# hyperplane-lab/ACL-GAN

Hardware: AMD Instinct MI355X
Metric: training images/sec at 256x256 (gen+dis step) (higher is better)
Workload: dtype fp32

## Files before the change

### acl-gan_amd/csrc/common.h

```cpp
#pragma once
#include <hip/hip_runtime.h>
#include <stdint.h>
#include <stddef.h>
#include <string>
#include <atomic>
#include "../../include/aclgan_hip.h"
#include "switches.h"

namespace aclgan {

void set_error(const char* fmt, ...);
int hip_fail(hipError_t e, const char* what);

extern std::atomic<long long> g_launches;
extern std::atomic<long long> g_enc_reuse_hits;

#define ACL_CHECK_LAUNCH(what)                                           \
    do {                                                                 \
        ++::aclgan::g_launches;                                          \
        hipError_t e__ = hipGetLastError();                              \
        if (e__ != hipSuccess) return ::aclgan::hip_fail(e__, what);     \
    } while (0)

#define ACL_REQUIRE(cond, ...)                                           \
    do {                                                                 \
        if (!(cond)) { ::aclgan::set_error(__VA_ARGS__); return ACLGAN_EINVAL; } \
    } while (0)

int reduce_slices_ordered(const float* part, int64_t n, int nslices, float* out, hipStream_t st);
size_t colsum_ordered_bytes(int64_t M, int C);
int colsum_ordered(const float* dy, float* db, int64_t M, int C, void* part, hipStream_t st);

static inline int cdiv(int a, int b) { return (a + b - 1) / b; }
static inline int64_t cdiv64(int64_t a, int64_t b) { return (a + b - 1) / b; }

struct ConvGeom {
    int B, Hi, Wi, Ci, Co, k, s, p, up, act;
    int Hu, Wu;
    int Hp, Wp;
    int Ho, Wo;
    int M;
    int K;
};
int make_geom(const aclgan_conv_desc* d, ConvGeom* g);

int conv_fold(const ConvGeom& g, const float* dxp, float* dx, int accumulate, hipStream_t st);
double conv_exec_flops(const ConvGeom& g, int which, bool f16);
bool conv_wgrad_fast_supported(const ConvGeom& g);
int conv_fwd(const ConvGeom& g, const float* x, const float* w, const float* bias, float* y, hipStream_t st, void* scratch = nullptr, float* stats = nullptr,
             float* keepV = nullptr);
size_t conv_fwd_keep_bytes(const ConvGeom& g);
int conv_fwd_stats_chunk(const ConvGeom& g);
size_t conv_fwd_scratch_bytes(const ConvGeom& g);
size_t conv_up5_scratch_bytes(const ConvGeom& g);
int conv_up5_fwd(const ConvGeom& g, const float* x, const float* w, const float* bias, float* y, void* scratch, hipStream_t st, float* keepV = nullptr);
int conv_fwd_naive(const ConvGeom& g, const float* x, const float* w, const float* bias, float* y, hipStream_t st);
size_t conv_dgrad_scratch_bytes(const ConvGeom& g);
int conv_dgrad(const ConvGeom& g, const float* dy, const float* w, float* dx, void* scratch, int accumulate, hipStream_t st);
int conv_wgrad(const ConvGeom& g, const float* x, const float* dy, float* dw, float* db, hipStream_t st, void* scratch = nullptr, const float* haveV = nullptr);
size_t conv_wgrad_scratch_bytes(const ConvGeom& g);
int conv_up5_dgrad(const ConvGeom& g, const float* dy, const float* w, float* dx, int accumulate, void* scratch, hipStream_t st);
int conv_up5_wgrad(const ConvGeom& g, const float* x, const float* dy, float* dw, float* db, void* scratch, hipStream_t st, const float* haveV = nullptr);

int conv_fwd_fast(const ConvGeom& g, const float* x, const float* w, const float* bias, float* y, hipStream_t st, void* scratch = nullptr, float* stats = nullptr,
                  float* keepV = nullptr);
size_t conv_fwd_fast_scratch_bytes(const ConvGeom& g);
int conv_dgrad_fast(const ConvGeom& g, const float* dy, const float* w, float* dxp, float* dx, int accumulate, bool* direct, hipStream_t st);
int conv_dgrad_ring(const ConvGeom& g, const float* dy, const float* w, float* dx, int band, hipStream_t st);
double conv_dgrad_ring_flops(const ConvGeom& g, int band);
int conv_wgrad_fast(const ConvGeom& g, const float* x, const float* dy, float* dw, float* db, hipStream_t st, void* scratch = nullptr, const float* haveV = nullptr);
size_t conv_wgrad_fast_scratch_bytes(const ConvGeom& g);

struct WinoUCache { void* user; float* (*lookup)(void* user, const float* w, int variant, size_t bytes, bool* fresh); };
void set_wino_ucache(const WinoUCache* c);
const WinoUCache* wino_ucache();
size_t conv_wino_u_bytes(const ConvGeom& g);
int conv_wino_u_variant(const ConvGeom& g, int dgrad, bool keepV);
int conv_up5_wino_u_variant(const ConvGeom& g, int dgrad, bool keepV);
int conv_wino_prefill(const ConvGeom& g, int uv, const float* w0, int64_t w_stride, float* U0, int64_t u_stride, int count, hipStream_t st);
int wino_fused_filter_batch(const float* w0, int64_t w_stride, float* Uf0, int64_t u_stride, int count, int Co, int Ci, int flip, hipStream_t st);

bool conv_wino_ok(const ConvGeom& g);
size_t conv_wino_scratch_bytes(const ConvGeom& g);
int conv_fwd_wino(const ConvGeom& g, const float* x, const float* w, const float* bias, float* y, void* scratch, hipStream_t st, float* stats = nullptr,
                  float* keepV = nullptr);
size_t conv_wino_keep_bytes(const ConvGeom& g);
size_t conv_up5_wino_keep_bytes(const ConvGeom& g);
int conv_dgrad_wino_interior(const ConvGeom& g, const float* dy, const float* w, float* dx, int accumulate, void* scratch, hipStream_t st);
size_t conv_wgrad_wino_scratch_bytes(const ConvGeom& g);
bool conv_up5_wino_ok(const ConvGeom& g);
size_t conv_up5_wino_fwd_scratch_bytes(const ConvGeom& g);
size_t conv_up5_wino_dgrad_scratch_bytes(const ConvGeom& g);
size_t conv_up5_wino_wgrad_scratch_bytes(const ConvGeom& g);
int conv_up5_wino_fwd_phases(const ConvGeom& g, const float* x, const float* wp, const float* bias, float* y, void* scratch, hipStream_t st, float* keepV = nullptr,
                             const float* wkey = nullptr);
int conv_up5_wino_dgrad_phases(const ConvGeom& g, const float* dy, const float* wp, float* dx, int accumulate, void* scratch, hipStream_t st,
                               const float* wkey = nullptr);
bool wino_u_cached(const float* wkey, int variant);
int conv_up5_wino_wgrad_phases(const ConvGeom& g, const float* x, const float* dy, float* dwp, float* db, void* scratch, hipStream_t st, const float* haveV = nullptr);
size_t conv_up5_dgrad_scratch_bytes(const ConvGeom& g);
int conv_wgrad_wino(const ConvGeom& g, const float* x, const float* dy, float* dw, float* db, void* scratch, hipStream_t st, const float* haveV = nullptr);

bool conv16_eligible(const ConvGeom& g, int which);
size_t conv_fwd16_scratch_bytes(const ConvGeom& g);
size_t conv_dgrad16_scratch_bytes(const ConvGeom& g);
size_t conv_wgrad16_scratch_bytes(const ConvGeom& g);
int conv_fwd16(const ConvGeom& g, int dtype, const float* x, const float* w, const void* w16, const float* bias, float* y, void* scratch, hipStream_t st,
               const void* x16 = nullptr, int y_storage = 0);
int conv_dgrad16(const ConvGeom& g, int dtype, const float* dy, const float* w, const void* w16t, float* dx, int accumulate, void* scratch, hipStream_t st);
int conv_wgrad16(const ConvGeom& g, int dtype, const float* x, const float* dy, float* dw, float* db, void* scratch, hipStream_t st, int x_storage = 0,
                 int dy_storage = 0);

bool conv16s_ok(const ConvGeom& g, int which);
int conv_fwd16s_stats_chunk(const ConvGeom& g);
int wino_fused_force(int on);
bool wino_fused_ok(int B, int H, int W, int Cin_, int Cout_, int act = ACLGAN_ACT_NONE, int gph = 1, int kph = 1);
int wino_fused_filter(const float* w, float* Uf, int Co, int Ci, int flip, hipStream_t st, int nph = 1);
int wino_fused_launch(int B, int H, int W, int Cin_, int Cout_, const float* in, const float* Uf, const float* bias, float* out, int act, int accumulate,
                      int reflect, float2* stats, hipStream_t st);
int wino_fused_up5_fwd(int B, int Hi, int Wi, int Cin_, int Cout_, const float* x, const float* Uf, const float* bias, float* y, int Hf, int Wf, int act,
                       hipStream_t st);
bool wino_wgrad_fused_ok(const ConvGeom& g);
size_t wino_wgrad_fused_scratch_bytes(const ConvGeom& g);
int wino_wgrad_fused(const ConvGeom& g, const float* x, const float* dy, float* dw, float* db, void* scratch, hipStream_t st);
int wino_fused_up5_dgrad(int B, int Hi, int Wi, int Cin_, int Cout_, const float* dy, const float* Uf, float* dx, int Hf, int Wf, int accumulate, hipStream_t st);
bool wino_fused_s2k4_ok(int B, int Hi, int Wi, int Ci, int Co, int act, int dgrad);
size_t wino_fused_s2k4_u_bytes(int Ci, int Co);
int wino_fused_filter_s2k4(const float* w, float* Uf, int Co, int Ci, int dgrad, hipStream_t st);
int wino_fused_s2k4_fwd(int B, int Hi, int Wi, int Ci, int Co, const float* x, const float* Uf, const float* bias, float* y, int act, float2* stats, hipStream_t st);
int wino_fused_s2k4_dgrad(int B, int Hi, int Wi, int Ci, int Co, const float* dy, const float* Uf, float* dx, int accumulate, hipStream_t st);
bool conv_s2k4_wino_ok(const ConvGeom& g, int which);
size_t conv_s2k4_wino_scratch_bytes(const ConvGeom& g);
int conv_fwd_s2k4_wino(const ConvGeom& g, const float* x, const float* w, const float* bias, float* y, void* scratch, hipStream_t st, float* stats = nullptr);
int conv_dgrad_s2k4_wino_interior(const ConvGeom& g, const float* dy, const float* w, float* dx, int accumulate, void* scratch, hipStream_t st);
bool gemm_x3_shape_ok(int T, int K, int N);
int gemm_slices_x3(const void* A3, size_t a_plane, const void* B3, size_t b_plane, float* C, int T, int K, int N, int nslices, int a_mod, hipStream_t st);
int split3_planes(const float* x, void* out, int64_t n, int64_t plane_elems, hipStream_t st);
int conv_fwd16s(const ConvGeom& g, int dtype, const void* x16, const void* w16, const float* bias, void* y, int yst, hipStream_t st, float* stats = nullptr);
size_t conv_dgrad16s_scratch_bytes(const ConvGeom& g);
bool conv_wgrad16s_ok(const ConvGeom& g);
size_t conv_wgrad16s_scratch_bytes(const ConvGeom& g);
int conv_wgrad16s(const ConvGeom& g, int dtype, const void* x16, const void* dy16, float* dw, float* db, void* scratch, hipStream_t st);
int conv_dgrad16s(const ConvGeom& g, int dtype, const void* dy16, const void* w16t, void* dx, int dxst, int accumulate, void* scratch, hipStream_t st);
int cast_flat16(const float* src, void* dst, int64_t n, int dtype, hipStream_t st);
int transpose_flat16(const float* base, void* base_t, const int64_t* offs, const int* co, const int* taps, const int* ci, int n, int dtype, hipStream_t st);

int conv_fwd_small(const ConvGeom& g, const float* x, const float* w, const float* bias, float* y, hipStream_t st);
int conv_wgrad_small(const ConvGeom& g, const float* x, const float* dy, float* dw, float* db, hipStream_t st, void* scratch = nullptr);
size_t conv_wgrad_small_scratch_bytes(const ConvGeom& g);
int conv_dgrad_small(const ConvGeom& g, const float* dy, const float* w, float* dxp, hipStream_t st);
bool conv_s2k4_thin_dgrad_ok(const ConvGeom& g);

size_t norm_scratch_bytes(int B, int HW, int C);
struct NormST { int x = 0, y = 0, res = 0, dy = 0, dx = 0, dres = 0; };
int norm_fwd(int kind, int act, int B, int HW, int C, const void* x, const float* w, const float* b, int w_stride,
             const void* residual, void* y, float* mean, float* rstd, void* scratch, hipStream_t st, const float* stats = nullptr,
             int stats_chunk = 0, const NormST* sto = nullptr, float* ss_out = nullptr);
int norm_bwd(int kind, int act, int B, int HW, int C, const void* x, const void* y, const void* dy,
             const float* w, int w_stride, const float* mean, const float* rstd, void* dx, float* dw, float* db,
             void* dres, int dres_accumulate, void* scratch, hipStream_t st, const NormST* sto = nullptr, float* sbc_out = nullptr,
             const float* ss = nullptr);
int norm_bwd_ln_params(const float* sbc, int B, int C, float* dgamma, float* dbeta, hipStream_t st);

int act_bwd_inplace(int act, const void* y, void* dy, int64_t n, hipStream_t st, int yst = 0, int gst = 0);
int cast_storage(const void* src, int src_st, void* dst, int dst_st, int64_t n, hipStream_t st);
int positive_mask(const void* y, int yst, unsigned char* dst, int64_t n, hipStream_t st);
int positive_mask_diff(const float* a, int ca, const float* b, int cb, unsigned char* dst, int64_t npix, hipStream_t st);
int avgpool3s2_fwd(int B, int H, int W, int C, const float* x, float* y, hipStream_t st);
int avgpool3s2_bwd(int B, int H, int W, int C, const float* dy, float* dx, int accumulate, hipStream_t st);
size_t diffaugment_scratch_bytes(int N, int H, int W, int C);
int diffaugment_fwd(int N, int H, int W, int C, int policy, const float* x, const float* params, float* y, void* scratch, hipStream_t st);
int diffaugment_bwd(int N, int H, int W, int C, int policy, const float* dy, const float* params, float* dx, int accumulate, void* scratch, hipStream_t st);
struct DisView {
    int cin = 0, dim = 0, n_layer = 0, num_scales = 0;
    const float* lscale = nullptr;
    const float* w[64]; const float* b[64]; float* dw[64];
};
const int DIS_VIEW_MAX = 64;
int dis_view(const aclgan_ctx* ctx, int net, DisView* v);
int adam_flat(float* p, const float* g, float* m, float* v, int64_t n, const aclgan_adam* o, int step, hipStream_t st);
int adam_flat_ema(float* p, const float* g, float* m, float* v, float* ema, int64_t n, const aclgan_adam* o, int step, float decay, int mode, hipStream_t st);
int nchw_to_nhwc(const float* src, float* dst, int B, int C, int H, int W, hipStream_t st);
int nhwc_to_nchw(const float* src, float* dst, int B, int C, int H, int W, hipStream_t st);
int fill_zero(float* p, int64_t n, hipStream_t st);
int zero_async(void* p, size_t bytes, hipStream_t st);

int linear_fwd(int B, int I, int O, const float* x, const float* w, const float* bias, int act, float* y, hipStream_t st);
bool mlp3_fwd_ok(int S, int M);
int mlp3_fwd(int B, int S, int M, int O, const float* s, const float* W0, const float* b0, const float* W1, const float* b1, const float* W2,
             const float* b2, float* m0, float* m1, float* ap, hipStream_t st);
int linear_bwd(int B, int I, int O, const float* x, const float* y, float* dy, const float* w, int act,
               float* dx, float* dw, float* db, hipStream_t st);
int linear_bwd_params(int B, int I, int O, const float* x, const float* dy, float* dw, float* db, hipStream_t st);
int gap_fwd(int B, int HW, int C, const void* x, float* y, hipStream_t st, int xst = 0);
int gap_bwd(int B, int HW, int C, const float* dy, void* dx, int accumulate, hipStream_t st, int xst = 0);

int focus_blend_fwd(int B, int HW, const float* dec4, const float* bg, float* out, const float* pair_first, float* pair, hipStream_t st);
int focus_blend_bwd(int B, int HW, const float* dec4, const float* bg, const float* d_out, const float* d_pair,
                    float* d_dec4, float* d_bg, int bg_accumulate, hipStream_t st);
int plain_pair_fwd(int B, int HW, const float* dec3, float* out, const float* pair_first, float* pair, hipStream_t st);
int plain_pair_bwd(int B, int HW, const float* d_out, const float* d_pair, float* d_dec3, hipStream_t st);
int focus_translation_nchw(const float* fg, int64_t fg_bstride, const float* bg, int64_t bg_bstride, const float* focus, int64_t focus_bstride,
                           float* out, int B, int HW, hipStream_t st);
int lsgan_loss(const float* o, int n, float target, float weight, float* loss_slot, float* d_o, float gscale, hipStream_t st, const float* lscale = nullptr);
struct LsganTerm { const float* o; float* d_o; float* slot; int n; float target, weight, gscale; };
const int LSGAN_MAX_TERMS = 12;
int lsgan_loss_batch(const LsganTerm* terms, int nterms, hipStream_t st, const float* lscale = nullptr);
struct LecamTerm { LsganTerm ls; const float* anchor; float* lecam; float* stats; };
int lsgan_lecam_batch(const LecamTerm* terms, int nterms, float lambda, int start, const int* count, hipStream_t st, const float* lscale = nullptr);
static inline size_t lecam_state_floats(int S) { return (size_t)18 * S + 4; }
int lecam_fold(float* state, int num_scales, float decay, bool whole, hipStream_t st);
struct AdaSignTerm { const float* o; int n; float weight; };
const int ADA_SIGN_MAX_TERMS = 12;
static inline size_t ada_state_floats() { return 12; }
int augment_gate(const float* rows, const float* u, const float* state, int n, int H, int W, int policy, float* rows_eff, hipStream_t st);
int ada_sign(const AdaSignTerm* terms, int nterms, float* acc, hipStream_t st);
int ada_fold(float* state, float target, int interval, float step, hipStream_t st);
const int L1_PART_FLOATS = 1024;
int l1_loss(const float* a, int a_stride, const float* b, int64_t npix, float* loss_slot, float* d_a, float gscale, int d_accumulate, hipStream_t st,
            const float* lscale = nullptr, float* part = nullptr);
int focus_sums_blocks(int64_t npix);
int focus_sums(const float* dec4, int64_t npix, float eps, float upper, float* part, hipStream_t st);
int focus_loss_finish(const float* dec4, int64_t npix, const float* part, float delta, float upper, float lower, float eps,
                      float scale, float* size_slot, float* digit_slot, float* d_dec4, hipStream_t st, const float* lscale = nullptr,
                      const float* totals = nullptr, int64_t npix_total = 0);
int focus_totals(const float* part, int64_t npix, int nmask, float* totals, hipStream_t st);
int adam_flat_scaled(float* p, const float* g, float* m, float* v, int64_t n, const aclgan_adam* o, int step, float* state, int group, hipStream_t st);
int adam_flat_scaled_ema(float* p, const float* g, float* m, float* v, float* ema, int64_t n, const aclgan_adam* o, int step, float decay, int mode,
                         float* state, int group, hipStream_t st);
size_t grad_clip_state_floats();
int gradnorm_launch(const float* g, int64_t n, float max_norm, float* clip, float* lscale, hipStream_t st);
int modeseek_chunks(int64_t n);
size_t modeseek_scratch_floats(int B, int64_t n);
int modeseek_part(const void* a, const void* b, int st, int B, int64_t n, float* part, hipStream_t s);
int modeseek_grad(const void* a, const void* b, int st, int B, int64_t n, const float* part, const float* u, const float* u2, int sd, float u_scale,
                  float weight, const float* lscale, float* out4, float* da, float* db, int accumulate, hipStream_t s);
int adam_flat_clipped(float* p, const float* g, float* m, float* v, float* ema, int64_t n, const aclgan_adam* o, int step, float decay, int mode,
                      float* state, int group, float max_norm, float* clip, hipStream_t st);

const int SN_MAX_LAYERS = 16;
struct SnLayerPtrs { const float* w; float* u; float* v; float* wn; float* uf; float* vf; float* G; int co, k; };
size_t sn_scratch_bytes(int n, const int* co, const int* k);
int sn_power_iteration(int n, const SnLayerPtrs* L, float* sigma, void* scratch, hipStream_t st);
struct SnFoldPtrs { const float* w; const float* G; const float* u; const float* v; float* grad; int co, k; };
size_t sn_fold_scratch_bytes(int n, const int* co, const int* k);
int sn_fold(int n, const SnFoldPtrs* L, const float* sigma, void* scratch, hipStream_t st);

}
```

### acl-gan_amd/csrc/engine.h

```cpp
#pragma once
#include "common.h"
#include <dlfcn.h>

#include <functional>
#include <map>
#include <vector>
#include <tuple>
#include <mutex>
#include <algorithm>
#include <cmath>
#include <cstring>
#include <cstdio>

namespace aclgan {

struct TensorInfo {
    std::string name;
    int64_t offset;
    int64_t numel;
    int shape[4];
    int ndim;
};

struct Group {
    std::vector<TensorInfo> tensors;
    std::map<std::string, int> index;
    int64_t numel = 0;
    float *param = nullptr, *grad = nullptr, *m = nullptr, *v = nullptr;
};

struct Act {
    float* d = nullptr;
    float* g = nullptr;
    int dt = 0, gdt = 0;
    int B = 0, H = 0, W = 0, C = 0;
    bool need_grad = false;
    bool gw = false;
    Act* parent = nullptr;
    struct Stamp { int lane, ck; };
    Stamp dst[4]; int ndst = 0;
    Stamp gst = {-1, 0};
    Act* root() { return parent ? parent : this; }
    int64_t numel() const { return (int64_t)B * H * W * C; }
    bool written() const { return gw || (parent && parent->gw); }
};

struct PW {
    const float* w = nullptr; const float* b = nullptr;
    float* dw = nullptr; float* db = nullptr;
    int64_t nw = 0, nb = 0;
    const unsigned short* w16 = nullptr;
    const unsigned short* w16t = nullptr;
};

struct TapeOp {
    std::function<int(aclgan_ctx&)> fn;
    int64_t goff[4] = {0, 0, 0, 0}, gnum[4] = {0, 0, 0, 0};
    int ng = 0;
    int lane = 0;
    int pass = -1;
};

struct Roctx {
    int (*push)(const char*) = nullptr;
    int (*pop)() = nullptr;
    bool on = false;
    Roctx() {
        if (!sw(SW_ROCTX)) return;
        for (const char* name : {"librocprofiler-sdk-roctx.so", "librocprofiler-sdk-roctx.so.1", "libroctx64.so", "libroctx64.so.4"}) {
            void* h = dlopen(name, RTLD_NOW | RTLD_GLOBAL);
            if (!h) continue;
            push = (int (*)(const char*))dlsym(h, "roctxRangePushA");
            pop = (int (*)())dlsym(h, "roctxRangePop");
            if (push && pop) { on = true; return; }
        }
    }
    static Roctx& get() { static Roctx r; return r; }
    void end_range() { pop(); push(("~end@" + std::to_string((long long)g_launches)).c_str()); pop(); }
};

struct StreamPool {
    static const int N = 4;
    hipStream_t s[N] = {nullptr, nullptr, nullptr, nullptr};
    static StreamPool& of_device() {
        static StreamPool pools[16];
        int dev = 0;
        (void)hipGetDevice(&dev);
        return pools[(dev >= 0 && dev < 16) ? dev : 0];
    }
    int get(int i, hipStream_t* out) {
        static std::mutex mu;
        std::lock_guard<std::mutex> lock(mu);
        if (!s[i]) {
            const hipError_t e = hipStreamCreateWithFlags(&s[i], hipStreamNonBlocking);
            if (e != hipSuccess) { s[i] = nullptr; return hip_fail(e, "stream pool"); }
        }
        *out = s[i];
        return ACLGAN_OK;
    }
};

inline const char* const NET_NAMES[5] = {"gen_AB", "gen_BA", "dis_A", "dis_B", "dis_2"};

}

using namespace aclgan;

struct aclgan_ctx {
    aclgan_arch arch;
    int dis_norm = ACLGAN_NORM_NONE;
    struct SnLayer { int co, k; std::string key; int64_t u_off, v_off; };
    std::vector<SnLayer> sn_layers[5];
    Group sn;
    std::vector<std::string> pass_names;
    std::vector<int> tape_pass;
    std::map<std::string, int> pass_count;
    int cur_pass = -1;
    int pass_begin(const char* net, const char* what);
    void pass_end(int prev);
    Group groups[2];
    char* ws = nullptr;
    size_t ws_bytes = 0;
    hipStream_t st = nullptr;
    bool dry = false;
    size_t top = 0, peak = 0;
    std::vector<Act*> acts;
    std::vector<TapeOp> tape;
    int dtype = ACLGAN_DTYPE_FP32;
    unsigned short* w16[2] = {nullptr, nullptr};
    unsigned short* w16t[2] = {nullptr, nullptr};
    float* lscale = nullptr;
    float* clip[2] = {nullptr, nullptr};
    float clip_max[2] = {0.f, 0.f};
    float* ema = nullptr;
    int fwd_weights = ACLGAN_WEIGHTS_LIVE;
    bool read_ema = false;
    const float* weights(int group) const { return group == ACLGAN_GROUP_GEN && read_ema ? ema : groups[group].param; }
    std::vector<int64_t> cv_off[2];
    std::vector<int> cv_co[2], cv_taps[2], cv_ci[2];
    int trained = -1;
    bool fire_dry = false;
    aclgan_sync_fn sync_fn = nullptr;
    void* sync_user = nullptr;
    int sync_world = 1;
    int64_t bucket_elems = 0;
    aclgan_bucket_fn bucket_fn = nullptr;
    void* bucket_user = nullptr;
    std::vector<int> bucket_order;
    struct NeedKey {
        int which, B, H, W, dtype; long long epoch; int determ, buckets;
        bool operator<(const NeedKey& o) const {
            return std::tie(which, B, H, W, dtype, epoch, determ, buckets) < std::tie(o.which, o.B, o.H, o.W, o.dtype, o.epoch, o.determ, o.buckets);
        }
    };
    std::map<NeedKey, size_t> need_cache;
    struct CarryBlock { float *in32, *co, *out, *mean, *rstd, *ss; int B, H, W, C, co_st, out_st; };
    struct CarryRec {
        bool valid = false;
        int B = 0, H = 0, W = 0, dtype = 0, determ = 0;
        const float* x_a = nullptr;
        long long gen_epoch = 0, tune_epoch = 0;
        char* ws = nullptr; size_t ws_bytes = 0, bytes = 0;
        std::vector<CarryBlock> blocks[2];
    };
    CarryRec carry;
    long long gen_epoch = 0;
    int aug_policy = 0;
    const float* aug_params = nullptr;
    int aug_rows = 0;
    float* lecam_state = nullptr;
    float lecam_lambda = 0.f, lecam_decay = 0.f;
    int lecam_start = 0;
    bool in_dis_update = false;
    float* ada_state = nullptr;
    float ada_target = 0.f, ada_step = 0.f;
    int ada_interval = 1;
    float ms_lambda = 0.f;
    const float* ms_z = nullptr;
    int ms_rows = 0;
    float* ms_out = nullptr;
    bool ms_on() const { return ms_lambda > 0.f && ms_z; }
    int carry_arm = ACLGAN_CARRY_OFF;
    int carry_call = ACLGAN_CARRY_OFF;
    int carry_mode = ACLGAN_CARRY_OFF;
    int carry_pass = 0; size_t carry_blk = 0;
    bool carry_fail = false;
    size_t carry_res = 0;
    int last_mode[2] = {ACLGAN_CARRY_OFF, ACLGAN_CARRY_OFF};
    void carry_drop() { carry.valid = false; ++gen_epoch; }
    size_t lim() const { return carry_res ? ((ws_bytes - carry_res) & ~(size_t)255) : ws_bytes; }
    void* alloc_carry(size_t bytes);
    void carry_pass_begin(int pass) { carry_mode = carry_call; carry_pass = pass; carry_blk = 0; }
    void carry_pass_end() { carry_mode = ACLGAN_CARRY_OFF; }
    double alg_bytes = 0.0;
    void count(double bytes) { alg_bytes += bytes; }
    double exec_flops = 0.0;
    size_t keep_total = 0;
    struct MaskEnt { int B, H, W, C, act; long long off; };
    unsigned char* mask_dst = nullptr; size_t mask_cap = 0, mask_top = 0;
    std::vector<MaskEnt> mask_log;
    int mask_push(int B, int H, int W, int C, int act, size_t n, unsigned char** dst) {
        if (mask_top + n > mask_cap) { set_error("aclgan_debug_capture_masks: buffer too small (%zu bytes)", mask_cap); return ACLGAN_ENOMEM; }
        *dst = mask_dst + mask_top;
        mask_log.push_back(MaskEnt{B, H, W, C, act, (long long)mask_top});
        mask_top += n;
        return ACLGAN_OK;
    }
    struct UEnt { float* u; bool filled; int layout; int lane, ck; };
    std::map<std::pair<const float*, int>, UEnt> ucache;
    WinoUCache ucache_hook;
    static float* ucache_lookup(void* user, const float* w, int variant, size_t bytes, bool* fresh);
    int ucache_reserve(const float* w, int variant, size_t bytes);
    bool act16() const { return dtype != ACLGAN_DTYPE_FP32 && sw(SW_ACT16); }

    hipStream_t st2 = nullptr;
    hipEvent_t ev_fork = nullptr, ev_join = nullptr;
    bool side_pending = false;
    size_t top2 = 0, peak2 = 0;
    void* alloc2(size_t bytes);
    int side_fork();
    int side_join();

    static const int MAXL = 4;
    hipStream_t st0 = nullptr;
    hipStream_t lane_st[MAXL] = {nullptr, nullptr, nullptr, nullptr};
    int nlanes = 1, cur_lane = 0;
    std::vector<hipEvent_t> ev_pool; size_t ev_next = 0;
    std::vector<hipEvent_t> lane_evs[MAXL];
    int seen[MAXL][MAXL] = {};
    size_t hw[MAXL] = {0, 0, 0, 0};
    bool lane_dirty[MAXL] = {false, false, false, false};
    int pass_seq = 0, cur_pass_id = -1;
    hipStream_t lane_stream(int l) const { return l == 0 ? st0 : lane_st[l]; }
    int nck(int l) const { return (int)lane_evs[l].size(); }
    hipStream_t st2_pool = nullptr;
    void lanes_clear();
    int lanes_begin(int want);
    int checkpoint(int l);
    int mark() { return nlanes > 1 ? checkpoint(cur_lane) : ACLGAN_OK; }
    int set_lane(int l);
    int wait_ck(int d, int s, int k);
    int need(Act* a);
    void wrote(Act* a);
    int acq(Act* a);
    int lanes_join();
    int lanes_barrier();
    void lanes_quiesce();
    ~aclgan_ctx();
    void reset_step();
    void* alloc(size_t bytes);
    float* allocf(int64_t n) { return (float*)alloc((size_t)n * sizeof(float)); }
    Act* new_act(int B, int H, int W, int C, bool need_grad, int st = 0, float* const* at = nullptr);
    Act* new_view(Act* joint, int b0, int nb);
    void push(std::function<int(aclgan_ctx&)> fn, std::initializer_list<std::pair<const float*, int64_t>> grads = {});
    PW pw(int group, int net, const std::string& key, bool with_bias = true) const;
    int64_t numel_of(int group, int net, const std::string& key) const;
    const float* param(int group, int net, const std::string& key) const;
    float* gradp(int group, int net, const std::string& key) const;
};

namespace aclgan {

#define RUN(expr)                                  \
    do {                                           \
        if (!c.dry) { int rc__ = (expr); if (rc__) return rc__; } \
    } while (0)
#define CHK(expr)                                  \
    do { int rc__ = (expr); if (rc__) return rc__; } while (0)
#define NEED(ptr)                                  \
    do { if (!(ptr)) { set_error("workspace too small (need > %zu bytes, bound %zu)", c.top, c.ws_bytes); return ACLGAN_ENOMEM; } } while (0)
#define NEED_ACT(a)                                \
    do { NEED((a)->d); if ((a)->need_grad) NEED((a)->g); } while (0)

struct PassScope {
    aclgan_ctx& c; int prev, prev_id;
    PassScope(aclgan_ctx& c_, int net, const char* what) : c(c_), prev(c_.pass_begin(NET_NAMES[net], what)), prev_id(c_.cur_pass_id) { c.cur_pass_id = c.pass_seq++; }
    ~PassScope() { c.pass_end(prev); c.cur_pass_id = prev_id; }
};

struct NormSpec {
    int kind = ACLGAN_NORM_NONE;
    const float* w = nullptr; const float* b = nullptr;
    float* dw = nullptr; float* db = nullptr;
    int w_stride = 0;
};

static inline void mark_written(Act* a) { a->gw = true; }

struct LsSeg { float target, weight, gscale; float* slot; };

int stream_capturing(hipStream_t s);
int run_tape(aclgan_ctx& c);
int prefill_on_side_lane(aclgan_ctx& c, int B, int H, int W, bool train);
int content_encode(aclgan_ctx& c, int net, bool train, Act* x, Act** out);
int style_encode(aclgan_ctx& c, int net, bool train, Act* x, Act** out);
int decode(aclgan_ctx& c, int net, bool train, Act* content, Act* style, Act** out);
int dis_forward(aclgan_ctx& c, int net, bool train, Act* x, std::vector<Act*>* outs, int lane_a = -1, int lane_b = -1);
int dis_lsgan(aclgan_ctx& c, int net, bool train, Act* x, int nb, int row0, const std::vector<LsSeg>& segs, int lane_a = -1, int lane_b = -1);
int blend(aclgan_ctx& c, Act* dec4, Act* bg, Act* pair_first, Act** out_p, Act** pair_p, Act* out_dst = nullptr, Act* pair_dst = nullptr);
int zero_grad_of(aclgan_ctx& c, Act* a);
int pack_params(aclgan_ctx& c);
int input_act(aclgan_ctx& c, const float* nchw, int B, int C, int H, int W, Act** out);
int wrap_vec(aclgan_ctx& c, const float* dev, int B, int n, float scale, Act** out);

}
```

### acl-gan_amd/csrc/engine.hip

```cpp
#include "engine.h"

int aclgan_ctx::pass_begin(const char* net, const char* what) {
    if (!Roctx::get().on || dry) return -1;
    const std::string base = std::string(net) + "." + what;
    const int n = ++pass_count[base];
    pass_names.push_back(base + "#" + std::to_string(n));
    const int prev = cur_pass;
    cur_pass = (int)pass_names.size() - 1;
    Roctx::get().push((pass_names.back() + "@" + std::to_string((long long)g_launches)).c_str());
    return prev;
}
void aclgan_ctx::pass_end(int prev) {
    if (!Roctx::get().on || dry) return;
    Roctx::get().end_range();
    cur_pass = prev;
}

void* aclgan_ctx::alloc2(size_t bytes) {
    const size_t need = top2 + ((bytes + 255) & ~(size_t)255);
    top2 = need;
    if (need > peak2) peak2 = need;
    if (dry) return (void*)(uintptr_t)4096;
    if (peak + need + 256 > lim()) return nullptr;
    return ws + ((lim() - need) & ~(size_t)255);
}
int aclgan_ctx::side_fork() {
    if (dry) return ACLGAN_OK;
    if (!st2) {
        CHK(aclgan::StreamPool::of_device().get(0, &st2_pool));
        st2 = st2_pool;
    }
    if (st2 == st) return ACLGAN_OK;
    if (!ev_fork) {
        hipError_t e = hipEventCreateWithFlags(&ev_fork, hipEventDisableTiming);
        if (e == hipSuccess) e = hipEventCreateWithFlags(&ev_join, hipEventDisableTiming);
        if (e != hipSuccess) return aclgan::hip_fail(e, "side stream events");
    }
    hipError_t e = hipEventRecord(ev_fork, st);
    if (e == hipSuccess) e = hipStreamWaitEvent(st2, ev_fork, 0);
    if (e != hipSuccess) return aclgan::hip_fail(e, "side stream fork");
    side_pending = true;
    return ACLGAN_OK;
}
int aclgan_ctx::side_join() {
    if (dry || !side_pending) return ACLGAN_OK;
    hipError_t e = hipEventRecord(ev_join, st2);
    if (e == hipSuccess) e = hipStreamWaitEvent(st0 ? st0 : st, ev_join, 0);
    if (e != hipSuccess) return aclgan::hip_fail(e, "side stream join");
    side_pending = false;
    return ACLGAN_OK;
}


int aclgan::stream_capturing(hipStream_t s) {
    hipStreamCaptureStatus cs = hipStreamCaptureStatusNone;
    if (hipStreamIsCapturing(s, &cs) != hipSuccess) { (void)hipGetLastError(); return -1; }
    return cs != hipStreamCaptureStatusNone;
}
void aclgan_ctx::lanes_clear() {
    for (int l = 0; l < MAXL; ++l) { lane_evs[l].clear(); hw[l] = 0; lane_dirty[l] = false; for (int m = 0; m < MAXL; ++m) seen[l][m] = 0; }
    ev_next = 0; cur_lane = 0;
}
int aclgan_ctx::lanes_begin(int want) {
    nlanes = std::max(1, std::min(want, (int)MAXL));
    if (!sw(SW_SIDE_STREAM)) nlanes = 1;
    const bool capturing = !dry && stream_capturing(st) > 0;
    if (!dry && !capturing) (void)hipGetLastError();
    if (capturing) nlanes = 1;
    st0 = st;
    lanes_clear();
    if (dry) return ACLGAN_OK;
    if (sw(SW_SIDE_STREAM) && !st2_pool) { int rc = aclgan::StreamPool::of_device().get(0, &st2_pool); if (rc) return rc; }
    st2 = capturing ? st : st2_pool;
    for (int l = 1; l < nlanes; ++l)
        if (!lane_st[l]) { int rc = aclgan::StreamPool::of_device().get(l, &lane_st[l]); if (rc) return rc; }
    return ACLGAN_OK;
}
int aclgan_ctx::checkpoint(int l) {
    hipEvent_t ev = nullptr;
    if (!dry) {
        if (ev_next == ev_pool.size()) {
            hipEvent_t e = nullptr;
            hipError_t rc = hipEventCreateWithFlags(&e, hipEventDisableTiming);
            if (rc != hipSuccess) return aclgan::hip_fail(rc, "lane event");
            ev_pool.push_back(e);
        }
        ev = ev_pool[ev_next++];
        hipError_t rc = hipEventRecord(ev, lane_stream(l));
        if (rc != hipSuccess) return aclgan::hip_fail(rc, "lane checkpoint");
    }
    lane_evs[l].push_back(ev);
    lane_dirty[l] = false;
    return ACLGAN_OK;
}
int aclgan_ctx::set_lane(int l) {
    if (nlanes <= 1) return ACLGAN_OK;
    l %= nlanes;
    if (l == cur_lane) return ACLGAN_OK;
    CHK(checkpoint(cur_lane));
    cur_lane = l;
    lane_dirty[l] = true;
    if (!dry) st = lane_stream(l);
    return ACLGAN_OK;
}
int aclgan_ctx::wait_ck(int d, int s, int k) {
    if (d == s || k < seen[d][s]) return ACLGAN_OK;
    if (k >= nck(s)) {
        CHK(checkpoint(s));
        k = nck(s) - 1;
    }
    if (!dry) {
        hipError_t e = hipStreamWaitEvent(lane_stream(d), lane_evs[s][k], 0);
        if (e != hipSuccess) return aclgan::hip_fail(e, "lane wait");
    }
    lane_dirty[d] = true;
    seen[d][s] = k + 1;
    return ACLGAN_OK;
}
int aclgan_ctx::need(Act* a) {
    if (nlanes <= 1 || !a) return ACLGAN_OK;
    Act* r = a->root();
    for (int i = 0; i < r->ndst; ++i)
        if (r->dst[i].lane != cur_lane) { int rc = wait_ck(cur_lane, r->dst[i].lane, r->dst[i].ck); if (rc) return rc; }
    return ACLGAN_OK;
}
void aclgan_ctx::wrote(Act* a) {
    if (!a) return;
    Act* r = a->root();
    for (int i = 0; i < r->ndst; ++i)
        if (r->dst[i].lane == cur_lane) { r->dst[i].ck = nck(cur_lane); return; }
    if (r->ndst < 4) r->dst[r->ndst++] = Act::Stamp{cur_lane, nck(cur_lane)};
}
int aclgan_ctx::acq(Act* a) {
    if (nlanes <= 1 || !a) return ACLGAN_OK;
    Act* r = a->root();
    if (r->gst.lane >= 0 && r->gst.lane != cur_lane) { int rc = wait_ck(cur_lane, r->gst.lane, r->gst.ck); if (rc) return rc; }
    r->gst = Act::Stamp{cur_lane, nck(cur_lane)};
    return ACLGAN_OK;
}
int aclgan_ctx::lanes_join() {
    if (nlanes > 1) {
        CHK(set_lane(0));
        for (int l = 1; l < nlanes; ++l) {
            if (lane_dirty[l]) CHK(checkpoint(l));
            if (nck(l) > 0) CHK(wait_ck(0, l, nck(l) - 1));
        }
    }
    return side_join();
}
int aclgan_ctx::lanes_barrier() {
    int rc = lanes_join();
    if (rc || nlanes <= 1) return rc;
    CHK(checkpoint(0));
    for (int l = 1; l < nlanes; ++l) CHK(wait_ck(l, 0, nck(0) - 1));
    for (int l = 0; l < MAXL; ++l) hw[l] = 0;
    return ACLGAN_OK;
}
void aclgan_ctx::lanes_quiesce() {
    if (dry) return;
    for (int l = 1; l < nlanes; ++l) if (lane_st[l]) (void)hipStreamSynchronize(lane_st[l]);
    if (st2) (void)hipStreamSynchronize(st2);
    side_pending = false;
    cur_lane = 0; if (st0) st = st0;
}
aclgan_ctx::~aclgan_ctx() {
    reset_step();
    if (ev_fork) (void)hipEventDestroy(ev_fork);
    if (ev_join) (void)hipEventDestroy(ev_join);
    for (hipEvent_t e : ev_pool) (void)hipEventDestroy(e);
}
void aclgan_ctx::reset_step() {
    for (Act* a : acts) delete a;
    acts.clear();
    tape.clear();
    tape_pass.clear(); pass_names.clear(); pass_count.clear(); cur_pass = -1;
    top = 0;
    top2 = 0;
    keep_total = 0;
    ucache.clear();
    read_ema = false;
    lanes_clear();
    nlanes = 1; pass_seq = 0; cur_pass_id = -1;
    if (st0) { st = st0; st0 = nullptr; }
}
void* aclgan_ctx::alloc(size_t bytes) {
    size_t a = (top + 255) & ~(size_t)255;
    if (nlanes > 1) for (int l = 0; l < nlanes; ++l) if (l != cur_lane && hw[l] > a) a = hw[l];
    top = a + bytes;
    if (nlanes > 1) { const size_t e = (top + 255) & ~(size_t)255; if (e > hw[cur_lane]) hw[cur_lane] = e; }
    if (top > peak) peak = top;
    if (dry) return (void*)(uintptr_t)(a + 4096);
    if (top + peak2 + 256 > lim()) return nullptr;
    return ws + a;
}
Act* aclgan_ctx::new_act(int B, int H, int W, int C, bool need_grad, int st, float* const* at) {
    Act* a = new Act();
    a->B = B; a->H = H; a->W = W; a->C = C; a->need_grad = need_grad; a->dt = st; a->gdt = st;
    a->d = at ? *at : (float*)alloc((size_t)a->numel() * (st ? 2 : 4));
    if (need_grad) a->g = allocf(a->numel());
    acts.push_back(a);
    wrote(a);
    return a;
}
Act* aclgan_ctx::new_view(Act* joint, int b0, int nb) {
    Act* a = new Act();
    a->B = nb; a->H = joint->H; a->W = joint->W; a->C = joint->C; a->need_grad = joint->need_grad;
    const int64_t off = (int64_t)b0 * joint->H * joint->W * joint->C;
    a->d = joint->d + off;
    a->g = joint->g ? joint->g + off : nullptr;
    a->parent = joint;
    acts.push_back(a);
    return a;
}
void aclgan_ctx::push(std::function<int(aclgan_ctx&)> fn, std::initializer_list<std::pair<const float*, int64_t>> grads) {
    TapeOp op;
    op.fn = std::move(fn);
    if (trained >= 0 && groups[trained].grad)
        for (const auto& g : grads)
            if (g.first && g.second > 0 && op.ng < 4 && g.first >= groups[trained].grad && g.first < groups[trained].grad + groups[trained].numel) {
                op.goff[op.ng] = g.first - groups[trained].grad; op.gnum[op.ng] = g.second; ++op.ng;
            }
    op.lane = cur_lane; op.pass = cur_pass_id;
    tape.push_back(std::move(op));
    tape_pass.push_back(cur_pass);
}
void* aclgan_ctx::alloc_carry(size_t bytes) {
    const size_t need = carry_res + ((bytes + 255) & ~(size_t)255);
    if (dry) { carry_res = need; return (void*)(uintptr_t)4096; }
    if (peak + peak2 + need + 512 > ws_bytes) return nullptr;
    carry_res = need;
    return ws + ((ws_bytes - need) & ~(size_t)255);
}
float* aclgan_ctx::ucache_lookup(void* user, const float* w, int variant, size_t bytes, bool* fresh) {
    aclgan_ctx* c = (aclgan_ctx*)user;
    const int layout = variant >> 4;
    auto it = c->ucache.find(std::make_pair(w, variant & 15));
    if (it == c->ucache.end()) return nullptr;
    UEnt& e = it->second;
    if (!e.filled) {
        *fresh = true;
        if (bytes) { e.filled = true; e.layout = layout; e.lane = c->cur_lane; e.ck = c->nck(c->cur_lane); }
        return e.u;
    }
    if (e.layout != layout) return nullptr;
    *fresh = false;
    if (bytes && c->nlanes > 1 && e.lane != c->cur_lane && c->wait_ck(c->cur_lane, e.lane, e.ck) != ACLGAN_OK) return nullptr;
    return e.u;
}
int aclgan_ctx::ucache_reserve(const float* w, int variant, size_t bytes) {
    if (sw(SW_NOUCACHE) || !bytes || ucache.count(std::make_pair(w, variant))) return ACLGAN_OK;
    float* u = (float*)alloc(bytes);
    if (!u) return ACLGAN_ENOMEM;
    ucache[std::make_pair(w, variant)] = UEnt{u, false, 0, 0, 0};
    return ACLGAN_OK;
}

static const TensorInfo* find_tensor(const Group& g, int net, const std::string& key) {
    auto it = g.index.find(std::string(NET_NAMES[net]) + "/" + key);
    return it == g.index.end() ? nullptr : &g.tensors[it->second];
}
const float* aclgan_ctx::param(int group, int net, const std::string& key) const {
    const TensorInfo* t = find_tensor(groups[group], net, key);
    return t && groups[group].param ? weights(group) + t->offset : nullptr;
}
float* aclgan_ctx::gradp(int group, int net, const std::string& key) const {
    const TensorInfo* t = find_tensor(groups[group], net, key);
    return t && groups[group].grad ? groups[group].grad + t->offset : nullptr;
}
int64_t aclgan_ctx::numel_of(int group, int net, const std::string& key) const {
    const TensorInfo* t = find_tensor(groups[group], net, key);
    return t ? t->numel : 0;
}
PW aclgan_ctx::pw(int group, int net, const std::string& key, bool with_bias) const {
    PW p;
    p.w = param(group, net, key + ".weight"); p.dw = gradp(group, net, key + ".weight"); p.nw = numel_of(group, net, key + ".weight");
    if (with_bias) { p.b = param(group, net, key + ".bias"); p.db = gradp(group, net, key + ".bias"); p.nb = numel_of(group, net, key + ".bias"); }
    if (dtype != ACLGAN_DTYPE_FP32 && p.w && w16[group] && w16t[group]) {
        const int64_t off = p.w - weights(group);
        p.w16 = w16[group] + off; p.w16t = w16t[group] + off;
    }
    return p;
}

namespace aclgan {

static void add_tensor(Group& g, const std::string& name, int ndim, int d0, int d1 = 1, int d2 = 1, int d3 = 1) {
    TensorInfo t;
    t.name = name; t.offset = g.numel; t.ndim = ndim;
    t.shape[0] = d0; t.shape[1] = d1; t.shape[2] = d2; t.shape[3] = d3;
    t.numel = (int64_t)d0 * d1 * d2 * d3;
    g.index[name] = (int)g.tensors.size();
    g.tensors.push_back(t);
    g.numel += (t.numel + 3) / 4 * 4;
}
static void add_conv(Group& g, const std::string& prefix, int co, int ci, int k) {
    add_tensor(g, prefix + ".weight", 4, co, ci, k, k);
    add_tensor(g, prefix + ".bias", 1, co);
}

static void build_gen(Group& g, const std::string& net, const aclgan_arch& a) {
    char buf[160];
    const int nd = a.gen_n_downsample, nr = a.gen_n_res, sd = a.gen_style_dim;
    int d = a.gen_dim;
    add_conv(g, net + "/enc_style.model.0.conv", d, a.input_dim_a, 7);
    for (int i = 0; i < 2; ++i) { snprintf(buf, sizeof buf, "/enc_style.model.%d.conv", 1 + i); add_conv(g, net + buf, 2 * d, d, 4); d *= 2; }
    for (int i = 0; i < 2; ++i) { snprintf(buf, sizeof buf, "/enc_style.model.%d.conv", 3 + i); add_conv(g, net + buf, d, d, 4); }
    add_conv(g, net + "/enc_style.model.6", sd, d, 1);
    d = a.gen_dim;
    add_conv(g, net + "/enc_content.model.0.conv", d, a.input_dim_a, 7);
    for (int i = 0; i < nd; ++i) { snprintf(buf, sizeof buf, "/enc_content.model.%d.conv", 1 + i); add_conv(g, net + buf, 2 * d, d, 4); d *= 2; }
    for (int r = 0; r < nr; ++r)
        for (int j = 0; j < 2; ++j) { snprintf(buf, sizeof buf, "/enc_content.model.%d.model.%d.model.%d.conv", 1 + nd, r, j); add_conv(g, net + buf, d, d, 3); }
    for (int r = 0; r < nr; ++r)
        for (int j = 0; j < 2; ++j) { snprintf(buf, sizeof buf, "/dec.model.0.model.%d.model.%d.conv", r, j); add_conv(g, net + buf, d, d, 3); }
    int idx = 2;
    for (int i = 0; i < nd; ++i) {
        snprintf(buf, sizeof buf, "/dec.model.%d.norm.gamma", idx); add_tensor(g, net + buf, 1, d / 2);
        snprintf(buf, sizeof buf, "/dec.model.%d.norm.beta", idx); add_tensor(g, net + buf, 1, d / 2);
        snprintf(buf, sizeof buf, "/dec.model.%d.conv", idx); add_conv(g, net + buf, d / 2, d, 5);
        d /= 2; idx += 2;
    }
    snprintf(buf, sizeof buf, "/dec.model.%d.conv", idx - 1); add_conv(g, net + buf, a.gen_output_dim, d, 7);
    const int C = a.gen_dim << nd, nad = 2 * C * 2 * nr, md = a.gen_mlp_dim;
    add_tensor(g, net + "/mlp.model.0.fc.weight", 2, md, sd); add_tensor(g, net + "/mlp.model.0.fc.bias", 1, md);
    add_tensor(g, net + "/mlp.model.1.fc.weight", 2, md, md); add_tensor(g, net + "/mlp.model.1.fc.bias", 1, md);
    add_tensor(g, net + "/mlp.model.2.fc.weight", 2, nad, md); add_tensor(g, net + "/mlp.model.2.fc.bias", 1, nad);
}

static void build_dis(Group& g, const std::string& net, int input_dim, const aclgan_arch& a, std::vector<aclgan_ctx::SnLayer>* sn = nullptr,
                      Group* st = nullptr) {
    char buf[160];
    for (int s = 0; s < a.dis_num_scales; ++s) {
        int d = a.dis_dim;
        snprintf(buf, sizeof buf, "/cnns.%d.0.conv", s); add_conv(g, net + buf, d, input_dim, 4);
        for (int i = 0; i < a.dis_n_layer - 1; ++i) {
            snprintf(buf, sizeof buf, "/cnns.%d.%d.conv", s, i + 1);
            if (sn) {
                const std::string pre = net + buf + ".module.";
                add_tensor(g, pre + "bias", 1, 2 * d);
                add_tensor(g, pre + "weight_bar", 4, 2 * d, d, 4, 4);
                aclgan_ctx::SnLayer L;
                L.co = 2 * d; L.k = 16 * d; L.key = std::string(buf + 1) + ".module.";
                L.u_off = st->numel; add_tensor(*st, pre + "weight_u", 1, L.co);
                L.v_off = st->numel; add_tensor(*st, pre + "weight_v", 1, L.k);
                sn->push_back(L);
            } else {
                add_conv(g, net + buf, 2 * d, d, 4);
            }
            d *= 2;
        }
        snprintf(buf, sizeof buf, "/cnns.%d.%d", s, a.dis_n_layer); add_conv(g, net + buf, 1, d, 1);
    }
}

static void fire_bucket(aclgan_ctx& c, int b) {
    c.bucket_order.push_back(b);
    if (!c.bucket_fn || (c.dry && !c.fire_dry)) return;
    const int64_t off = (int64_t)b * c.bucket_elems;
    const int64_t n = std::min<int64_t>(c.bucket_elems, c.groups[c.trained].numel - off);
    c.bucket_fn(c.bucket_user, c.trained, b, off, n);
}
static int run_tape_impl(aclgan_ctx& c) {
    const size_t n = c.tape.size();
    const bool buckets = c.trained >= 0 && c.bucket_elems > 0;
    std::vector<std::vector<int>> done_at;
    if (buckets) {
        const int nb = (int)cdiv64(c.groups[c.trained].numel, c.bucket_elems);
        std::vector<size_t> first(nb, n);
        for (size_t i = 0; i < n; ++i)
            for (int r = 0; r < c.tape[i].ng; ++r) {
                const int64_t b0 = c.tape[i].goff[r] / c.bucket_elems, b1 = (c.tape[i].goff[r] + c.tape[i].gnum[r] - 1) / c.bucket_elems;
                for (int64_t b = b0; b <= b1 && b < nb; ++b) first[b] = std::min(first[b], i);
            }
        done_at.resize(n);
        c.bucket_order.clear();
        for (int b = 0; b < nb; ++b) {
            if (first[b] == n) fire_bucket(c, b);
            else done_at[first[b]].push_back(b);
        }
    }
    CHK(c.lanes_barrier());
    const bool marks = Roctx::get().on && !c.dry && c.tape_pass.size() == n;
    int open = -1, last_pass = -2;
    for (size_t i = n; i-- > 0;) {
        if (marks && c.tape_pass[i] != open) {
            if (open >= 0) Roctx::get().end_range();
            open = c.tape_pass[i];
            if (open >= 0) Roctx::get().push(("bwd:" + c.pass_names[open] + "@" + std::to_string((long long)g_launches)).c_str());
        }
        if (c.tape[i].pass != last_pass) { if (last_pass != -2) CHK(c.mark()); last_pass = c.tape[i].pass; }
        CHK(c.set_lane(c.tape[i].lane));
        int rc_i = c.tape[i].fn(c);
        if (!rc_i && !c.dry && sw(SW_FAULT_AT) >= 0 && (int)(n - 1 - i) == sw(SW_FAULT_AT)) { set_error("injected fault after backward closure %d (tuning key fault_at)", sw(SW_FAULT_AT)); rc_i = ACLGAN_EHIP; }
        if (rc_i) { if (marks && open >= 0) Roctx::get().pop(); return rc_i; }
        if (buckets && !done_at[i].empty()) {
            const int lane = c.cur_lane;
            CHK(c.lanes_join());
            for (int b : done_at[i]) fire_bucket(c, b);
            CHK(c.set_lane(lane));
        }
    }
    if (marks && open >= 0) Roctx::get().end_range();
    return c.lanes_join();
}
int run_tape(aclgan_ctx& c) {
    const int rc = run_tape_impl(c);
    if (rc) c.lanes_quiesce();
    return rc;
}

}

extern "C" {

int aclgan_ctx_create(const aclgan_arch* arch, aclgan_ctx** out) {
    return aclgan_ctx_create_dis_norm(arch, ACLGAN_NORM_NONE, out);
}

int aclgan_ctx_create_dis_norm(const aclgan_arch* arch, int dis_norm, aclgan_ctx** out) {
    ACL_REQUIRE(arch && out, "null argument");
    ACL_REQUIRE(dis_norm == ACLGAN_NORM_NONE || dis_norm == ACLGAN_NORM_SN, "dis_norm %d: only none (%d) and sn (%d) are implemented", dis_norm,
                ACLGAN_NORM_NONE, ACLGAN_NORM_SN);
    ACL_REQUIRE(arch->input_dim_a == 3 && arch->input_dim_b == 6, "input_dim_a must be 3 and input_dim_b 6 (trainer.py:19-23,132-133)");
    ACL_REQUIRE(arch->gen_output_dim == 4 || arch->gen_output_dim == 3, "gen.output_dim must be 4 (image + focus mask, trainer.py:108) or 3 (non-focus configuration, trainer.py:117-121)");
    ACL_REQUIRE(arch->gen_dim >= 4 && (arch->gen_dim & (arch->gen_dim - 1)) == 0, "gen.dim must be a power of two >= 4");
    ACL_REQUIRE(arch->dis_dim >= 4 && arch->dis_dim % 4 == 0, "dis.dim must be a multiple of 4");
    ACL_REQUIRE(arch->gen_n_downsample >= 1 && arch->gen_n_res >= 1 && arch->dis_n_layer >= 1 && arch->dis_num_scales >= 1, "bad layer counts");
    ACL_REQUIRE(arch->gen_mlp_dim >= 1 && arch->gen_style_dim >= 1, "bad mlp/style dims");
    ACL_REQUIRE(dis_norm != ACLGAN_NORM_SN || arch->dis_num_scales * (arch->dis_n_layer - 1) <= SN_MAX_LAYERS,
                "spectral norm: at most %d normalised layers per discriminator", SN_MAX_LAYERS);
    aclgan_ctx* c = new aclgan_ctx();
    c->arch = *arch;
    const bool sn = dis_norm == ACLGAN_NORM_SN && arch->dis_n_layer > 1;
    c->dis_norm = sn ? ACLGAN_NORM_SN : ACLGAN_NORM_NONE;
    build_gen(c->groups[0], "gen_AB", *arch);
    build_gen(c->groups[0], "gen_BA", *arch);
    build_dis(c->groups[1], "dis_A", arch->input_dim_a, *arch, sn ? &c->sn_layers[ACLGAN_NET_DIS_A] : nullptr, &c->sn);
    build_dis(c->groups[1], "dis_B", arch->input_dim_a, *arch, sn ? &c->sn_layers[ACLGAN_NET_DIS_B] : nullptr, &c->sn);
    build_dis(c->groups[1], "dis_2", arch->input_dim_b, *arch, sn ? &c->sn_layers[ACLGAN_NET_DIS_2] : nullptr, &c->sn);
    for (int g = 0; g < 2; ++g)
        for (const TensorInfo& t : c->groups[g].tensors)
            if (t.ndim == 4) {
                c->cv_off[g].push_back(t.offset); c->cv_co[g].push_back(t.shape[0]);
                c->cv_taps[g].push_back(t.shape[2] * t.shape[3]); c->cv_ci[g].push_back(t.shape[1]);
            }
    *out = c;
    return ACLGAN_OK;
}

void aclgan_ctx_destroy(aclgan_ctx* ctx) { delete ctx; }

int aclgan_ctx_enable_capture(aclgan_ctx* ctx) {
    ACL_REQUIRE(ctx, "null ctx");
    return ACLGAN_OK;
}

int aclgan_warm_streams(int lanes) {
    int n = 0;
    if (hipGetDeviceCount(&n) != hipSuccess || n <= 0) { (void)hipGetLastError(); return ACLGAN_OK; }
    if (!sw(SW_SIDE_STREAM)) return ACLGAN_OK;
    lanes = std::max(1, std::min(lanes <= 0 ? sw(SW_LANES) : lanes, 3));
    hipStream_t s = nullptr;
    int rc = aclgan::StreamPool::of_device().get(0, &s);
    for (int l = 1; l < lanes && rc == ACLGAN_OK; ++l) rc = aclgan::StreamPool::of_device().get(l, &s);
    return rc;
}

int aclgan_debug_capture_masks(aclgan_ctx* ctx, unsigned char* dst, size_t cap_bytes) {
    ACL_REQUIRE(ctx, "null ctx");
    ctx->mask_dst = dst; ctx->mask_cap = dst ? cap_bytes : 0; ctx->mask_top = 0; ctx->mask_log.clear();
    return ACLGAN_OK;
}
int aclgan_debug_mask_count(const aclgan_ctx* ctx) { return ctx ? (int)ctx->mask_log.size() : 0; }
int aclgan_debug_mask_info(const aclgan_ctx* ctx, int index, int* dims4, long long* offset, int* act) {
    ACL_REQUIRE(ctx && index >= 0 && index < (int)ctx->mask_log.size(), "mask index out of range");
    const aclgan_ctx::MaskEnt& e = ctx->mask_log[index];
    if (dims4) { dims4[0] = e.B; dims4[1] = e.H; dims4[2] = e.W; dims4[3] = e.C; }
    if (offset) *offset = e.off;
    if (act) *act = e.act;
    return ACLGAN_OK;
}

int aclgan_set_compute_dtype(aclgan_ctx* ctx, int dtype) {
    ACL_REQUIRE(ctx && dtype >= ACLGAN_DTYPE_FP32 && dtype <= ACLGAN_DTYPE_FP16, "bad ctx / dtype %d", dtype);
    ctx->dtype = dtype;
    ctx->carry_drop();
    return ACLGAN_OK;
}
int aclgan_bind_params16(aclgan_ctx* ctx, int group, void* w16, void* w16t) {
    ACL_REQUIRE(ctx && group >= 0 && group <= 1, "bad ctx/group");
    ctx->w16[group] = (unsigned short*)w16; ctx->w16t[group] = (unsigned short*)w16t;
    ctx->carry_drop();
    return ACLGAN_OK;
}
int aclgan_bind_loss_scale(aclgan_ctx* ctx, float* state) {
    ACL_REQUIRE(ctx, "null ctx");
    ctx->lscale = state;
    return ACLGAN_OK;
}

int64_t aclgan_group_numel(const aclgan_ctx* ctx, int group) {
    if (!ctx || group < 0 || group > ACLGAN_GROUP_SN_STATE) return -1;
    return group == ACLGAN_GROUP_SN_STATE ? ctx->sn.numel : ctx->groups[group].numel;
}
int aclgan_tensor_count(const aclgan_ctx* ctx, int group) {
// ... 182 lines not shown
```

### acl-gan_amd/csrc/engine_graph.hip

```cpp
#include "engine.h"

namespace aclgan {

static int conv_block(aclgan_ctx& c, const PW& W, bool train_w, Act* in, int Co, int k, int stride, int pad, int up, int act,
                      const NormSpec& ns, Act* residual, Act** out_p, int out16 = 1) {
    aclgan_conv_desc d;
    d.B = in->B; d.Hi = in->H; d.Wi = in->W; d.Ci = in->C; d.Co = Co; d.k = k; d.stride = stride; d.pad = pad; d.upsample = up;
    d.act = ns.kind == ACLGAN_NORM_NONE ? act : ACLGAN_ACT_NONE;
    ConvGeom g;
    CHK(make_geom(&d, &g));
    if (!W.w) { set_error("conv_block: parameters not bound"); return ACLGAN_EINVAL; }
    CHK(c.need(in)); CHK(c.need(residual));
    Act* const gin = in;
    const bool want_grad = train_w || in->need_grad || ns.dw != nullptr;
    const bool has_norm = ns.kind != ACLGAN_NORM_NONE;
    const int dt = c.dtype;
    const bool h16 = dt != ACLGAN_DTYPE_FP32 && W.w16 != nullptr;
    const bool f16 = h16 && conv16_eligible(g, 0), d16 = h16 && conv16_eligible(g, 1), w16 = h16 && conv16_eligible(g, 2);
    const bool a16 = h16 && c.act16();
    const bool s_bwd = a16 && f16 && d16 && w16 && conv16s_ok(g, 1);
    const bool s_fwd = a16 && f16 && conv16s_ok(g, 0) && in->dt != 0;
    const bool keep = c.carry_mode == ACLGAN_CARRY_KEEP, adopt = c.carry_mode == ACLGAN_CARRY_ADOPT, carried = keep || adopt;
    const bool tw = train_w || keep;
    aclgan_ctx::CarryBlock cb_dry = {};
    aclgan_ctx::CarryBlock* cb = &cb_dry;
    if (carried && !c.dry) {
        std::vector<aclgan_ctx::CarryBlock>& blocks = c.carry.blocks[c.carry_pass];
        if (keep) { blocks.push_back(cb_dry); cb = &blocks.back(); }
        else {
            if (c.carry_blk >= blocks.size()) { set_error("conv_block: the kept encodings hold no block %zu", c.carry_blk); return ACLGAN_EINVAL; }
            cb = &blocks[c.carry_blk++];
        }
    }
    auto buf = [&](float* aclgan_ctx::CarryBlock::*slot, size_t bytes) -> float* {
        if (!carried) return (float*)c.alloc(bytes);
        if (adopt && !c.dry) return cb->*slot;
        float* p = (float*)c.alloc_carry(bytes);
        cb->*slot = p;
        return p;
    };
    auto act_in = [&](float* aclgan_ctx::CarryBlock::*slot, int B_, int H_, int W_, int C_, bool grad, int st) -> Act* {
        float* at = carried ? buf(slot, (size_t)B_ * H_ * W_ * C_ * (st ? 2 : 4)) : nullptr;
        return c.new_act(B_, H_, W_, C_, grad, st, carried ? &at : nullptr);
    };
    if (in->dt != 0 && !(f16 && (w16 || !tw))) {
        Act* in32 = act_in(&aclgan_ctx::CarryBlock::in32, in->B, in->H, in->W, in->C, false, 0);
        NEED_ACT(in32);
        if (!adopt) RUN(cast_storage(in->d, in->dt, in32->d, 0, in->numel(), c.st));
        in = in32;
    }
    const int out_st = (a16 && Co % 64 == 0 && out16) ? dt : 0;
    const int co_st = has_norm ? ((s_bwd && sw(SW_CO16)) ? dt : 0) : ((f16 || !out_st) ? out_st : 0);
    if (adopt && !c.dry && (cb->B != g.B || cb->H != g.Ho || cb->W != g.Wo || cb->C != Co || cb->co_st != co_st || cb->out_st != out_st)) {
        set_error("conv_block: the kept encodings do not match this layer (%d x %d x %d x %d)", g.B, g.Ho, g.Wo, Co);
        return ACLGAN_EINVAL;
    }
    if (keep) { cb->B = g.B; cb->H = g.Ho; cb->W = g.Wo; cb->C = Co; cb->co_st = co_st; cb->out_st = out_st; }
    Act* co = act_in(&aclgan_ctx::CarryBlock::co, g.B, g.Ho, g.Wo, Co, want_grad, co_st);
    NEED_ACT(co);
    Act* out = co;
    float *mean = nullptr, *rstd = nullptr, *ss = nullptr;
    const int HW = g.Ho * g.Wo;
    if (has_norm) {
        out = act_in(&aclgan_ctx::CarryBlock::out, g.B, g.Ho, g.Wo, Co, want_grad, out_st);
        NEED_ACT(out);
        const int nstat = ns.kind == ACLGAN_NORM_LN ? g.B : g.B * Co;
        mean = buf(&aclgan_ctx::CarryBlock::mean, (size_t)nstat * 4); rstd = buf(&aclgan_ctx::CarryBlock::rstd, (size_t)nstat * 4);
        NEED(mean); NEED(rstd);
        if ((want_grad || keep) && (act == ACLGAN_ACT_RELU || act == ACLGAN_ACT_LRELU) && sw(SW_NORM_MASK)) {
            ss = buf(&aclgan_ctx::CarryBlock::ss, (size_t)2 * g.B * Co * 4);
            NEED(ss);
        }
        co->gdt = s_bwd ? dt : 0;
    } else if (out_st && !co_st) {
        out = act_in(&aclgan_ctx::CarryBlock::out, g.B, g.Ho, g.Wo, Co, want_grad, out_st);
        NEED_ACT(out);
        out->gdt = 0;
    } else {
        out->gdt = s_bwd ? co_st : 0;
    }
    if (gin->need_grad && !s_bwd) gin->gdt = 0;
    float* keepV = nullptr;
    if (train_w && !adopt && !f16 && !w16) {
        const size_t kb = conv_fwd_keep_bytes(g);
        if (kb && c.keep_total + kb <= (size_t)(sw_real(SW_KEEPV_BUDGET_GB) * 1073741824.0) + 1) { keepV = (float*)c.alloc(kb); NEED(keepV); c.keep_total += kb; }
    }
    const size_t ubytes = f16 ? 0 : conv_wino_u_bytes(g);
    if (ubytes && !adopt && c.ucache_reserve(W.w, g.up ? 2 : 0, ubytes)) { set_error("workspace too small (filter-transform cache)"); return ACLGAN_ENOMEM; }
    const double es_in = in->dt ? 2.0 : 4.0, es_co = co->dt ? 2.0 : 4.0, es_out = out->dt ? 2.0 : 4.0, es_w = f16 ? 2.0 : 4.0;
    if (!adopt) c.count(es_in * (double)in->numel() + es_w * (double)Co * g.K + 4.0 * Co + es_co * (double)co->numel());
    if (!adopt) c.exec_flops += conv_exec_flops(g, 0, f16);
    if (out != co && !adopt) c.count((es_co + es_out) * (double)co->numel() + ((has_norm && residual) ? (residual->dt ? 2.0 : 4.0) * (double)co->numel() : 0.0));
    const size_t mark = c.top;
    if (!adopt) {
    const int schunk = !has_norm ? 0 : (s_fwd ? conv_fwd16s_stats_chunk(g) : (!f16 ? conv_fwd_stats_chunk(g) : 0));
    float* stats = nullptr;
    if (schunk) { stats = c.allocf((size_t)2 * g.B * (HW / schunk) * Co); NEED(stats); }
    {
        const size_t fmark = c.top;
        void* fscr = nullptr;
        const size_t fb = s_fwd ? 0 : (f16 ? conv_fwd16_scratch_bytes(g) : conv_fwd_scratch_bytes(g));
        if (fb) { fscr = c.alloc(fb); NEED(fscr); }
        if (s_fwd) RUN(conv_fwd16s(g, dt, in->d, W.w16, W.b, co->d, co->dt, c.st, stats));
        else if (f16) RUN(conv_fwd16(g, dt, in->dt ? nullptr : in->d, W.w, W.w16, W.b, co->d, fscr, c.st, in->dt ? in->d : nullptr, co->dt));
        else RUN(conv_fwd(g, in->d, W.w, W.b, co->d, c.st, fscr, stats, keepV));
        c.top = fmark;
    }
    NormST nst;
    nst.x = co->dt; nst.y = out->dt; nst.res = residual ? residual->dt : 0;
    if (has_norm) {
        void* scr = c.alloc(norm_scratch_bytes(g.B, HW, Co));
        NEED(scr);
        RUN(norm_fwd(ns.kind, act, g.B, HW, Co, co->d, ns.w, ns.b, ns.w_stride, residual ? residual->d : nullptr, out->d, mean, rstd, scr, c.st, stats, schunk, &nst, ss));
    } else if (out != co) {
        RUN(cast_storage(co->d, co->dt, out->d, out->dt, co->numel(), c.st));
    }
    }
    c.top = mark;
    *out_p = out;
    if (c.mask_dst && !c.dry && want_grad && (act == ACLGAN_ACT_RELU || act == ACLGAN_ACT_LRELU)) {
        unsigned char* dst = nullptr;
        CHK(c.mask_push(out->B, out->H, out->W, out->C, act, (size_t)out->numel(), &dst));
        RUN(positive_mask(out->d, out->dt, dst, out->numel(), c.st));
    }
    c.wrote(out); c.wrote(co);
    if (!want_grad) return ACLGAN_OK;
    const bool ln_train = ns.kind == ACLGAN_NORM_LN && ns.dw != nullptr;
    c.push([=](aclgan_ctx& c) -> int {
        if (!out->gw) return ACLGAN_OK;
        CHK(c.acq(out));
        if (residual && residual->need_grad) CHK(c.acq(residual));
        if (gin->need_grad) CHK(c.acq(gin));
        const double eg_out = out->gdt ? 2.0 : 4.0, eg_co = (has_norm ? co->gdt : (s_bwd ? dt : out->gdt)) ? 2.0 : 4.0, eg_in = gin->gdt ? 2.0 : 4.0;
        c.count((es_co + eg_out + eg_co) * (double)co->numel() + ((residual && residual->need_grad) ? (residual->gdt ? 2.0 : 4.0) * (double)co->numel() : 0.0));
        if (train_w) { c.count(es_in * (double)in->numel() + eg_co * (double)co->numel() + 4.0 * ((double)Co * g.K + Co)); c.exec_flops += conv_exec_flops(g, 2, w16); }
        if (gin->need_grad) { c.count(eg_co * (double)co->numel() + es_w * (double)Co * g.K + eg_in * (double)in->numel()); c.exec_flops += conv_exec_flops(g, 1, d16); }
        const bool side = train_w && sw(SW_SIDE_STREAM);
        if (ubytes && gin->need_grad && !d16 && c.ucache_reserve(W.w, g.up ? 3 : 1, ubytes)) { set_error("workspace too small (filter-transform cache)"); return ACLGAN_ENOMEM; }
        float* g16 = nullptr;
        const size_t mark_pre = c.top;
        if (!has_norm && s_bwd && out->gdt == 0) {
            g16 = (float*)c.alloc((size_t)out->numel() * 2);
            NEED(g16);
        }
        float* sbc = nullptr;
        if (ln_train && side) { sbc = c.allocf((int64_t)2 * g.B * Co); NEED(sbc); }
        const size_t mark0 = side ? c.top : mark_pre;
        const float* dyp = nullptr;
        int dy_st = 0;
        if (has_norm) {
            const size_t mark = c.top;
            void* scr = c.alloc(norm_scratch_bytes(g.B, HW, Co));
            NEED(scr);
            float* dres = nullptr; int dacc = 0;
            if (residual && residual->need_grad) { dres = residual->g; dacc = residual->gw ? 1 : 0; mark_written(residual); }
            NormST bst;
            bst.x = co->dt; bst.y = out->dt; bst.dy = out->gdt; bst.dx = co->gdt; bst.dres = residual ? residual->gdt : 0;
            RUN(norm_bwd(ns.kind, act, g.B, HW, Co, co->d, out->d, out->g, ns.w, ns.w_stride, mean, rstd, co->g, ns.dw, ns.db, dres, dacc, scr, c.st, &bst, sbc, ss));
            c.top = mark;
            dyp = co->g; dy_st = co->gdt;
        } else if (s_bwd && out->gdt == 0) {
            RUN(cast_storage(out->g, 0, g16, dt, out->numel(), c.st));
            RUN(act_bwd_inplace(act, out->d, g16, out->numel(), c.st, out->dt, dt));
            dyp = g16; dy_st = dt;
        } else {
            RUN(act_bwd_inplace(act, co->d, out->g, out->numel(), c.st, co->dt, out->gdt));
            dyp = out->g; dy_st = out->gdt;
        }
        if (train_w) {
            const size_t mark = c.top;
            void* wscr = nullptr;
            const size_t wb = w16 ? conv_wgrad16_scratch_bytes(g) : conv_wgrad_scratch_bytes(g);
            hipStream_t wst = c.st;
            if (side) {
                CHK(c.side_fork());
                if (!c.dry) wst = c.st2;
                c.top2 = 0;
                if (wb) { wscr = c.alloc2(wb); if (!wscr) { set_error("workspace too small for the side-stream scratch"); return ACLGAN_ENOMEM; } }
                if (sbc) RUN(norm_bwd_ln_params(sbc, g.B, Co, ns.dw, ns.db, wst));
            } else if (wb) { wscr = c.alloc(wb); NEED(wscr); }
            if (w16) RUN(conv_wgrad16(g, dt, in->d, dyp, W.dw, W.db, wscr, wst, in->dt, dy_st));
            else {
                if (in->dt || dy_st) { set_error("conv_block: fp32 weight-gradient kernel on 16-bit operands"); return ACLGAN_EINVAL; }
                RUN(conv_wgrad(g, in->d, dyp, W.dw, W.db, wst, wscr, keepV));
            }
            c.top = mark;
        }
        if (gin->need_grad) {
            const size_t mark = c.top;
            if (s_bwd) {
                if (!dy_st) { set_error("conv_block: 16-bit-storage dgrad on an fp32 gradient"); return ACLGAN_EINVAL; }
                void* scr = c.alloc(conv_dgrad16s_scratch_bytes(g));
                NEED(scr);
                RUN(conv_dgrad16s(g, dt, dyp, W.w16t, gin->g, gin->gdt, gin->gw ? 1 : 0, scr, c.st));
            } else {
                if (dy_st || gin->gdt) { set_error("conv_block: fp32-output dgrad kernel on 16-bit gradients"); return ACLGAN_EINVAL; }
                void* scr = c.alloc(d16 ? conv_dgrad16_scratch_bytes(g) + 256 : conv_dgrad_scratch_bytes(g));
                NEED(scr);
                if (d16) RUN(conv_dgrad16(g, dt, dyp, W.w, W.w16t, gin->g, gin->gw ? 1 : 0, scr, c.st));
                else RUN(conv_dgrad(g, dyp, W.w, gin->g, scr, gin->gw ? 1 : 0, c.st));
            }
            mark_written(gin);
            c.top = mark;
        }
        c.top = mark0;
        return ACLGAN_OK;
    }, {{train_w ? W.dw : nullptr, W.nw}, {train_w ? W.db : nullptr, W.nb}, {ln_train ? ns.dw : nullptr, Co}, {ln_train ? ns.db : nullptr, Co}});
    return ACLGAN_OK;
}

static int prefill_wino_u(aclgan_ctx& c, int net, int B, int H, int W, bool train) {
    if (sw(SW_NOUCACHE) || !sw(SW_U_BATCH)) return ACLGAN_OK;
    const aclgan_arch& a = c.arch;
    const int nd = a.gen_n_downsample, count = 2 * a.gen_n_res, C = a.gen_dim << nd;
    if (count < 2) return ACLGAN_OK;
    aclgan_conv_desc d;
    d.B = B; d.Hi = H >> nd; d.Wi = W >> nd; d.Ci = C; d.Co = C; d.k = 3; d.stride = 1; d.pad = 1; d.upsample = 0; d.act = ACLGAN_ACT_NONE;
    ConvGeom g;
    if (make_geom(&d, &g)) return ACLGAN_OK;
    const size_t ubytes = conv_wino_u_bytes(g);
    if (!ubytes) return ACLGAN_OK;
    if (c.dtype != ACLGAN_DTYPE_FP32 && c.w16[0] && conv16_eligible(g, 0)) return ACLGAN_OK;
    char buf[160];
    for (int part = 0; part < 2; ++part) {
        std::vector<const float*> ws;
        for (int r = 0; r < a.gen_n_res; ++r)
            for (int j = 0; j < 2; ++j) {
                if (part == 0) snprintf(buf, sizeof buf, "enc_content.model.%d.model.%d.model.%d.conv.weight", 1 + nd, r, j);
                else snprintf(buf, sizeof buf, "dec.model.0.model.%d.model.%d.conv.weight", r, j);
                ws.push_back(c.param(0, net, buf));
            }
        if (!ws[0]) continue;
        const int64_t wstride = ws[1] - ws[0];
        bool even = wstride > 0;
        for (int i = 1; i < count && even; ++i) even = ws[i] && ws[i] - ws[i - 1] == wstride;
        if (!even) continue;
        for (int dgrad = 0; dgrad <= (train ? 1 : 0); ++dgrad) {
            const bool keepV = train && !dgrad && conv_fwd_keep_bytes(g) > 0;
            const int uv = conv_wino_u_variant(g, dgrad, keepV);
            if (uv < 0 || c.ucache.count(std::make_pair(ws[0], uv & 15))) continue;
            float* u0 = nullptr;
            bool contiguous = true;
            const size_t ustride = (ubytes + 255) & ~(size_t)255;
            for (int i = 0; i < count; ++i) {
                float* u = (float*)c.alloc(ubytes);
                NEED(u);
                if (i == 0) u0 = u;
                else if ((char*)u != (char*)u0 + (size_t)i * ustride) contiguous = false;
                c.ucache[std::make_pair(ws[i], uv & 15)] = aclgan_ctx::UEnt{u, contiguous, uv >> 4, c.cur_lane, c.nck(c.cur_lane)};
            }
            if (!contiguous) {
                for (int i = 0; i < count; ++i) c.ucache[std::make_pair(ws[i], uv & 15)].filled = false;
                continue;
            }
            RUN(conv_wino_prefill(g, uv, ws[0], wstride, u0, (int64_t)(ustride / sizeof(float)), count, c.st));
        }
    }
    return ACLGAN_OK;
}

int prefill_on_side_lane(aclgan_ctx& c, int B, int H, int W, bool train) {
    const int AB = ACLGAN_NET_GEN_AB, BA = ACLGAN_NET_GEN_BA;
    if (c.nlanes <= 1) { CHK(prefill_wino_u(c, AB, B, H, W, train)); return prefill_wino_u(c, BA, B, H, W, train); }
    const int LP = c.nlanes - 1;
    CHK(c.mark());
    const int k0 = c.nck(0) - 1;
    CHK(c.set_lane(LP));
    CHK(c.wait_ck(LP, 0, k0));
    CHK(prefill_wino_u(c, AB, B, H, W, train)); CHK(prefill_wino_u(c, BA, B, H, W, train));
    CHK(c.mark());
    return c.set_lane(0);
}

int content_encode(aclgan_ctx& c, int net, bool train, Act* x, Act** out) {
    PassScope pass(c, net, c.carry_mode == ACLGAN_CARRY_ADOPT ? "encode(adopted)" : "encode");
    const aclgan_arch& a = c.arch;
    char buf[160];
    NormSpec in_; in_.kind = ACLGAN_NORM_IN;
    Act* h = nullptr;
    int d = a.gen_dim;
    CHK(conv_block(c, c.pw(0, net, "enc_content.model.0.conv"), train, x, d, 7, 1, 3, 0, ACLGAN_ACT_RELU, in_, nullptr, &h));
    for (int i = 0; i < a.gen_n_downsample; ++i) {
        snprintf(buf, sizeof buf, "enc_content.model.%d.conv", 1 + i);
        CHK(conv_block(c, c.pw(0, net, buf), train, h, 2 * d, 4, 2, 1, 0, ACLGAN_ACT_RELU, in_, nullptr, &h));
        d *= 2;
    }
    for (int r = 0; r < a.gen_n_res; ++r) {
        Act *t = nullptr, *o = nullptr;
        snprintf(buf, sizeof buf, "enc_content.model.%d.model.%d.model.0.conv", 1 + a.gen_n_downsample, r);
        CHK(conv_block(c, c.pw(0, net, buf), train, h, d, 3, 1, 1, 0, ACLGAN_ACT_RELU, in_, nullptr, &t));
        snprintf(buf, sizeof buf, "enc_content.model.%d.model.%d.model.1.conv", 1 + a.gen_n_downsample, r);
        CHK(conv_block(c, c.pw(0, net, buf), train, t, d, 3, 1, 1, 0, ACLGAN_ACT_NONE, in_, h, &o));
        h = o;
    }
    *out = h;
    return ACLGAN_OK;
}

static int dense(aclgan_ctx& c, const PW& W, bool train_w, Act* in, int O, int act, Act** out_p, bool launch = true) {
    const int B = in->B, I = in->H * in->W * in->C;
    const bool want = train_w || in->need_grad;
    CHK(c.need(in));
    Act* out = c.new_act(B, 1, 1, O, want);
    NEED_ACT(out);
    if (!W.w) { set_error("dense: parameters not bound"); return ACLGAN_EINVAL; }
    if (launch) RUN(linear_fwd(B, I, O, in->d, W.w, W.b, act, out->d, c.st));
    c.count(4.0 * ((double)B * I + (double)O * I + O + (double)B * O) * (want ? 3.0 : 1.0));
    c.wrote(out);
    *out_p = out;
    if (!want) return ACLGAN_OK;
    c.push([=](aclgan_ctx& c) -> int {
        if (!out->gw) return ACLGAN_OK;
        CHK(c.acq(out));
        if (in->need_grad) CHK(c.acq(in));
        float* dx = nullptr;
        float* tmp = nullptr;
        const size_t mark = c.top;
        if (in->need_grad) {
            if (in->gw) { tmp = c.allocf((int64_t)B * I); NEED(tmp); dx = tmp; } else dx = in->g;
        }
        const bool side = train_w && sw(SW_SIDE_STREAM);
        RUN(linear_bwd(B, I, O, in->d, out->d, out->g, W.w, act, dx, (train_w && !side) ? W.dw : nullptr, (train_w && !side) ? W.db : nullptr, c.st));
        if (side) {
            CHK(c.side_fork());
            RUN(linear_bwd_params(B, I, O, in->d, out->g, W.dw, W.db, c.st2));
        }
        if (in->need_grad) {
            if (tmp) {
                RUN(gap_bwd(B, 1, I, tmp, in->g, 1, c.st));
            }
            mark_written(in);
        }
        c.top = mark;
        return ACLGAN_OK;
    }, {{train_w ? W.dw : nullptr, W.nw}, {train_w ? W.db : nullptr, W.nb}});
    return ACLGAN_OK;
}

int style_encode(aclgan_ctx& c, int net, bool train, Act* x, Act** out) {
    PassScope pass(c, net, "style");
    const aclgan_arch& a = c.arch;
    char buf[160];
    NormSpec none;
    Act* h = nullptr;
    int d = a.gen_dim;
    CHK(conv_block(c, c.pw(0, net, "enc_style.model.0.conv"), train, x, d, 7, 1, 3, 0, ACLGAN_ACT_RELU, none, nullptr, &h));
    for (int i = 0; i < 2; ++i) {
        snprintf(buf, sizeof buf, "enc_style.model.%d.conv", 1 + i);
        CHK(conv_block(c, c.pw(0, net, buf), train, h, 2 * d, 4, 2, 1, 0, ACLGAN_ACT_RELU, none, nullptr, &h));
        d *= 2;
    }
    for (int i = 0; i < 2; ++i) {
        snprintf(buf, sizeof buf, "enc_style.model.%d.conv", 3 + i);
        CHK(conv_block(c, c.pw(0, net, buf), train, h, d, 4, 2, 1, 0, ACLGAN_ACT_RELU, none, nullptr, &h));
    }
    const bool want = h->need_grad;
    Act* p = c.new_act(h->B, 1, 1, d, want);
    NEED_ACT(p);
    RUN(gap_fwd(h->B, h->H * h->W, d, h->d, p->d, c.st, h->dt));
    c.wrote(p);
    c.count((h->dt ? 2.0 : 4.0) * (double)h->numel() * (want ? 2.0 : 1.0));
    if (want) {
        Act* hh = h;
        c.push([=](aclgan_ctx& c) -> int {
            if (!p->gw) return ACLGAN_OK;
            CHK(c.acq(p)); CHK(c.acq(hh));
            RUN(gap_bwd(hh->B, hh->H * hh->W, hh->C, p->g, hh->g, hh->gw ? 1 : 0, c.st, hh->gdt));
            mark_written(hh);
            return ACLGAN_OK;
        });
    }
    CHK(dense(c, c.pw(0, net, "enc_style.model.6"), train, p, a.gen_style_dim, ACLGAN_ACT_NONE, out));
    return ACLGAN_OK;
}

int decode(aclgan_ctx& c, int net, bool train, Act* content, Act* style, Act** out) {
    PassScope pass(c, net, "decode");
    const aclgan_arch& a = c.arch;
    char buf[160];
    const int C = content->C, nr = a.gen_n_res, nad = 2 * C * 2 * nr;
    Act *m0 = nullptr, *m1 = nullptr, *ap = nullptr;
    const int sdim = style->H * style->W * style->C;
    const bool fused = sw(SW_MLP_FUSED) && mlp3_fwd_ok(sdim, a.gen_mlp_dim);
    const PW W0 = c.pw(0, net, "mlp.model.0.fc"), W1 = c.pw(0, net, "mlp.model.1.fc"), W2 = c.pw(0, net, "mlp.model.2.fc");
    CHK(dense(c, W0, train, style, a.gen_mlp_dim, ACLGAN_ACT_RELU, &m0, !fused));
    CHK(dense(c, W1, train, m0, a.gen_mlp_dim, ACLGAN_ACT_RELU, &m1, !fused));
    CHK(dense(c, W2, train, m1, nad, ACLGAN_ACT_NONE, &ap, !fused));
    if (fused) RUN(mlp3_fwd(style->B, sdim, a.gen_mlp_dim, nad, style->d, W0.w, W0.b, W1.w, W1.b, W2.w, W2.b, m0->d, m1->d, ap->d, c.st));
    if (ap->need_grad) {
        RUN(fill_zero(ap->g, ap->numel(), c.st));
        mark_written(ap);
    }
    Act* h = content;
    int j = 0;
    for (int r = 0; r < nr; ++r) {
        Act *t = nullptr, *o = nullptr;
        for (int half = 0; half < 2; ++half) {
            NormSpec ns; ns.kind = ACLGAN_NORM_ADAIN; ns.w_stride = nad;
            ns.b = ap->d + 2 * C * j; ns.w = ap->d + 2 * C * j + C;
            if (ap->need_grad) { ns.db = ap->g + 2 * C * j; ns.dw = ap->g + 2 * C * j + C; }
            ++j;
            snprintf(buf, sizeof buf, "dec.model.0.model.%d.model.%d.conv", r, half);
            if (half == 0) CHK(conv_block(c, c.pw(0, net, buf), train, h, C, 3, 1, 1, 0, ACLGAN_ACT_RELU, ns, nullptr, &t));
            else CHK(conv_block(c, c.pw(0, net, buf), train, t, C, 3, 1, 1, 0, ACLGAN_ACT_NONE, ns, h, &o));
        }
        h = o;
    }
    int d = C, idx = 2;
    for (int i = 0; i < a.gen_n_downsample; ++i) {
        NormSpec ns; ns.kind = ACLGAN_NORM_LN;
        snprintf(buf, sizeof buf, "dec.model.%d.norm.gamma", idx); ns.w = c.param(0, net, buf); ns.dw = train ? c.gradp(0, net, buf) : nullptr;
        snprintf(buf, sizeof buf, "dec.model.%d.norm.beta", idx); ns.b = c.param(0, net, buf); ns.db = train ? c.gradp(0, net, buf) : nullptr;
        snprintf(buf, sizeof buf, "dec.model.%d.conv", idx);
        CHK(conv_block(c, c.pw(0, net, buf), train, h, d / 2, 5, 1, 2, 1, ACLGAN_ACT_RELU, ns, nullptr, &h, i + 1 < a.gen_n_downsample ? 1 : 0));
        d /= 2; idx += 2;
    }
    NormSpec none;
    snprintf(buf, sizeof buf, "dec.model.%d.conv", idx - 1);
    CHK(conv_block(c, c.pw(0, net, buf), train, h, a.gen_output_dim, 7, 1, 3, 0, ACLGAN_ACT_TANH, none, nullptr, out));
    return ACLGAN_OK;
}

struct SnCall {
    int n = 0;
    float *slot = nullptr, *G = nullptr, *sigma = nullptr;
    void* fscr = nullptr;
    unsigned short *s16 = nullptr, *s16t = nullptr;
    int64_t soff[SN_MAX_LAYERS] = {};
};

static int sn_begin_call(aclgan_ctx& c, int net, bool train, SnCall* sc) {
    const std::vector<aclgan_ctx::SnLayer>& Ls = c.sn_layers[net];
    const int n = (int)Ls.size();
    if (!c.dry && !c.sn.param) { set_error("spectral norm: aclgan_bind_sn_state was not called"); return ACLGAN_EINVAL; }
    int co[SN_MAX_LAYERS], kk[SN_MAX_LAYERS], taps[SN_MAX_LAYERS], ci[SN_MAX_LAYERS];
    int64_t tot = 0, tu = 0, tv = 0;
    sc->n = n;
    for (int l = 0; l < n; ++l) {
        co[l] = Ls[l].co; kk[l] = Ls[l].k; taps[l] = 16; ci[l] = Ls[l].k / 16;
        sc->soff[l] = tot;
        tot += (int64_t)co[l] * kk[l]; tu += co[l]; tv += kk[l];
    }
    const bool h16 = c.dtype != ACLGAN_DTYPE_FP32;
    sc->slot = c.allocf(tot); NEED(sc->slot);
    if (h16) {
        sc->s16 = (unsigned short*)c.alloc((size_t)tot * 2); NEED(sc->s16);
        sc->s16t = (unsigned short*)c.alloc((size_t)tot * 2); NEED(sc->s16t);
    }
    sc->sigma = c.allocf(n); NEED(sc->sigma);
    if (train) {
        sc->G = c.allocf(tot); NEED(sc->G);
        sc->fscr = c.alloc(sn_fold_scratch_bytes(n, co, kk)); NEED(sc->fscr);
    }
    const size_t mark = c.top;
    void* scr = c.alloc(sn_scratch_bytes(n, co, kk));
    NEED(scr);
    SnLayerPtrs P[SN_MAX_LAYERS];
    for (int l = 0; l < n; ++l) {
        float* st = c.sn.param;
        P[l] = SnLayerPtrs{c.param(1, net, Ls[l].key + "weight_bar"), st ? st + Ls[l].u_off : nullptr, st ? st + Ls[l].v_off : nullptr,
                           sc->slot + sc->soff[l], nullptr, nullptr, train ? sc->G + sc->soff[l] : nullptr, co[l], kk[l]};
    }
    RUN(sn_power_iteration(n, P, sc->sigma, scr, c.st));
    if (h16) {
        RUN(cast_flat16(sc->slot, sc->s16, tot, c.dtype, c.st));
        RUN(transpose_flat16(sc->slot, sc->s16t, sc->soff, co, taps, ci, n, c.dtype, c.st));
    }
    c.top = mark;
    c.count(4.0 * tot * (2.0 + 0.25 + 1.0 + (train ? 1.0 : 0.0)) + (h16 ? (8.0 + 4.0) * tot : 0.0) + 4.0 * 3.0 * (tu + tv));
    c.exec_flops += 4.0 * tot;
    if (!train) return ACLGAN_OK;
    const float* lo = nullptr; const float* hi = nullptr;
    for (int l = 0; l < n; ++l) {
        const float* g = c.gradp(1, net, Ls[l].key + "weight_bar");
        if (!g) continue;
        if (!lo || g < lo) lo = g;
        if (!hi || g + (int64_t)co[l] * kk[l] > hi) hi = g + (int64_t)co[l] * kk[l];
    }
    const SnCall s = *sc;
    c.push([=](aclgan_ctx& c) -> int {
        hipStream_t fst = c.st;
        if (sw(SW_SIDE_STREAM)) {
            CHK(c.side_fork());
            if (!c.dry) fst = c.st2;
        }
        SnFoldPtrs F[SN_MAX_LAYERS];
        const float* st = c.sn.param;
        for (int l = 0; l < s.n; ++l)
            F[l] = SnFoldPtrs{c.param(1, net, Ls[l].key + "weight_bar"), s.G + s.soff[l], st ? st + Ls[l].u_off : nullptr,
                              st ? st + Ls[l].v_off : nullptr, c.gradp(1, net, Ls[l].key + "weight_bar"), co[l], kk[l]};
        c.count(4.0 * tot * 5.0);
        c.exec_flops += 6.0 * tot;
        RUN(sn_fold(s.n, F, s.sigma, s.fscr, fst));
        return ACLGAN_OK;
    }, {{lo, (int64_t)(hi - lo)}});
    return ACLGAN_OK;
}

static PW sn_pw(aclgan_ctx& c, int net, const SnCall& sc, int l) {
    const aclgan_ctx::SnLayer& L = c.sn_layers[net][l];
    PW p;
    p.w = sc.slot + sc.soff[l];
    p.dw = sc.G ? sc.G + sc.soff[l] : nullptr;
    p.nw = (int64_t)L.co * L.k;
    p.b = c.param(1, net, L.key + "bias"); p.db = c.gradp(1, net, L.key + "bias"); p.nb = L.co;
    if (sc.s16) { p.w16 = sc.s16 + sc.soff[l]; p.w16t = sc.s16t + sc.soff[l]; }
    return p;
}

int dis_forward(aclgan_ctx& c, int net, bool train, Act* x, std::vector<Act*>* outs, int lane_a, int lane_b) {
    PassScope pass(c, net, "forward");
    const aclgan_arch& a = c.arch;
    char buf[160];
    NormSpec none;
    Act* xin = x;
    if (lane_a < 0) lane_a = lane_b = c.cur_lane;
    SnCall sc;
    const bool sn = !c.sn_layers[net].empty();
    int pi_lane = 0, pi_ck = 0;
    if (sn) {
        CHK(c.set_lane(lane_a));
        CHK(c.need(x));
        CHK(sn_begin_call(c, net, train, &sc));
        pi_lane = c.cur_lane; pi_ck = c.nck(pi_lane);
    }
    for (int s = 0; s < a.dis_num_scales; ++s) {
        CHK(c.set_lane(s == 0 ? lane_a : lane_b));
        if (sn) CHK(c.wait_ck(c.cur_lane, pi_lane, pi_ck));
        Act* h = xin;
        int d = a.dis_dim;
        for (int i = 0; i < a.dis_n_layer; ++i) {
            snprintf(buf, sizeof buf, "cnns.%d.%d.conv", s, i);
            const int co = i == 0 ? d : 2 * d;
            const PW p = (sn && i > 0) ? sn_pw(c, net, sc, s * (a.dis_n_layer - 1) + i - 1) : c.pw(1, net, buf);
            CHK(conv_block(c, p, train, h, co, 4, 2, 1, 0, ACLGAN_ACT_LRELU, none, nullptr, &h, i + 1 < a.dis_n_layer ? 1 : 0));
            if (i > 0) d *= 2;
        }
        snprintf(buf, sizeof buf, "cnns.%d.%d", s, a.dis_n_layer);
        Act* o = nullptr;
        CHK(conv_block(c, c.pw(1, net, buf), train, h, 1, 1, 1, 0, 0, ACLGAN_ACT_NONE, none, nullptr, &o));
        outs->push_back(o);
        if (s + 1 < a.dis_num_scales) {
            CHK(c.set_lane(lane_b));
            Act* src = xin;
            CHK(c.need(src));
            Act* p = c.new_act(src->B, (src->H - 1) / 2 + 1, (src->W - 1) / 2 + 1, src->C, src->need_grad);
            NEED_ACT(p);
            RUN(avgpool3s2_fwd(src->B, src->H, src->W, src->C, src->d, p->d, c.st));
            c.wrote(p);
            c.count(4.0 * ((double)src->numel() + (double)p->numel()) * (src->need_grad ? 2.0 : 1.0));
            if (src->need_grad) {
                c.push([=](aclgan_ctx& c) -> int {
                    if (!p->gw) return ACLGAN_OK;
                    CHK(c.acq(p)); CHK(c.acq(src));
                    RUN(avgpool3s2_bwd(src->B, src->H, src->W, src->C, p->g, src->g, src->gw ? 1 : 0, c.st));
                    mark_written(src);
                    return ACLGAN_OK;
                });
            }
            xin = p;
        }
    }
    return ACLGAN_OK;
}

static int augment(aclgan_ctx& c, int net, Act* x, int row0, Act** out) {
    PassScope pass(c, net, "augment");
    CHK(c.need(x));
    if (x->dt != 0) { set_error("augment: the discriminator inputs are fp32 tensors"); return ACLGAN_EINVAL; }
    Act* y = c.new_act(x->B, x->H, x->W, x->C, x->need_grad);
    NEED_ACT(y);
    const int policy = c.aug_policy;
    const size_t sb = (policy & ACLGAN_AUG_COLOR) ? diffaugment_scratch_bytes(x->B, x->H, x->W, x->C) : 0;
    const float* rows = c.aug_params ? c.aug_params + (size_t)row0 * 8 : nullptr;
    {
        const size_t mark = c.top;
        void* scr = nullptr;
        if (sb) { scr = c.alloc(sb); NEED(scr); }
        RUN(diffaugment_fwd(x->B, x->H, x->W, x->C, policy, x->d, rows, y->d, scr, c.st));
        c.top = mark;
    }
    c.wrote(y);
    c.count(4.0 * 2.0 * (double)x->numel() * (x->need_grad ? 2.0 : 1.0));
    *out = y;
    if (!x->need_grad) return ACLGAN_OK;
    c.push([=](aclgan_ctx& c) -> int {
        if (!y->gw) return ACLGAN_OK;
        CHK(c.acq(y)); CHK(c.acq(x));
        if (y->gdt != 0 || x->gdt != 0) { set_error("augment: the gradients of the discriminator inputs are fp32 tensors"); return ACLGAN_EINVAL; }
        const size_t mark = c.top;
        void* scr = nullptr;
        if (sb) { scr = c.alloc(sb); NEED(scr); }
        RUN(diffaugment_bwd(x->B, x->H, x->W, x->C, policy, y->g, rows, x->g, x->gw ? 1 : 0, scr, c.st));
        mark_written(x);
        c.top = mark;
        return ACLGAN_OK;
    });
    return ACLGAN_OK;
}

int dis_lsgan(aclgan_ctx& c, int net, bool train, Act* x, int nb, int row0, const std::vector<LsSeg>& segs, int lane_a, int lane_b) {
    std::vector<Act*> outs;
    if (c.aug_policy) {
        if (lane_a >= 0) CHK(c.set_lane(lane_a));
        CHK(augment(c, net, x, row0, &x));
        CHK(c.mark());
    }
    CHK(dis_forward(c, net, train, x, &outs, lane_a, lane_b));
    std::vector<LsganTerm> terms;
    for (Act* o : outs) {
        CHK(c.need(o));
        const int n = nb * o->H * o->W * o->C;
        for (size_t i = 0; i < segs.size(); ++i) {
            LsganTerm t;
            t.o = o->d + (size_t)i * n; t.d_o = o->need_grad ? o->g + (size_t)i * n : nullptr; t.slot = segs[i].slot;
            t.n = n; t.target = segs[i].target; t.weight = segs[i].weight; t.gscale = segs[i].gscale;
            terms.push_back(t);
        }
        if (o->need_grad) mark_written(o);
    }
    if (train && c.in_dis_update && c.lecam_state) {
        const int S = c.arch.dis_num_scales, D = net - ACLGAN_NET_DIS_A;
        float* st = c.lecam_state;
        std::vector<LecamTerm> lt(terms.size());
        for (size_t j = 0; j < terms.size(); ++j) {
            const int s = (int)(j / segs.size()), k = terms[j].target == 1.f ? 1 : 0;
            lt[j].ls = terms[j];
            lt[j].anchor = st + (D * S + s) * 2 + (1 - k);
            lt[j].lecam = st + 18 * S + D;
            lt[j].stats = st + 6 * S + ((D * S + s) * 2 + k) * 2;
        }
        RUN(lsgan_lecam_batch(lt.data(), (int)lt.size(), c.lecam_lambda, c.lecam_start, reinterpret_cast<const int*>(st + 18 * S + 3), c.st, c.lscale));
    } else RUN(lsgan_loss_batch(terms.data(), (int)terms.size(), c.st, c.lscale));
    if (train && c.in_dis_update && c.ada_state && net != ACLGAN_NET_DIS_2) {
        std::vector<AdaSignTerm> at;
        double bytes = 0.0;
        for (const LsganTerm& t : terms)
            if (t.target == 1.f) { at.push_back(AdaSignTerm{t.o, t.n, t.weight}); bytes += 4.0 * (double)t.n; }
        if (!at.empty()) {
            c.count(bytes + 2.0 * 4.0 * 2.0);
            RUN(ada_sign(at.data(), (int)at.size(), c.ada_state + 8 + 2 * (net - ACLGAN_NET_DIS_A), c.st));
        }
    }
    return ACLGAN_OK;
}

int blend(aclgan_ctx& c, Act* dec4, Act* bg, Act* pair_first, Act** out_p, Act** pair_p, Act* out_dst, Act* pair_dst) {
    const bool want = dec4->need_grad;
    CHK(c.need(dec4)); CHK(c.need(bg)); CHK(c.need(pair_first));
    Act* out = out_dst;
    if (!out) {
        out = c.new_act(dec4->B, dec4->H, dec4->W, 3, want);
        NEED_ACT(out);
    }
    Act* pair = nullptr;
    if (pair_first) {
        pair = pair_dst;
        if (!pair) {
            pair = c.new_act(dec4->B, dec4->H, dec4->W, 6, want);
            NEED_ACT(pair);
        }
    }
    const bool plain = dec4->C == 3;
    if (plain) RUN(plain_pair_fwd(dec4->B, dec4->H * dec4->W, dec4->d, out->d, pair_first ? pair_first->d : nullptr, pair ? pair->d : nullptr, c.st));
    else RUN(focus_blend_fwd(dec4->B, dec4->H * dec4->W, dec4->d, bg->d, out->d, pair_first ? pair_first->d : nullptr, pair ? pair->d : nullptr, c.st));
    c.count(4.0 * (double)dec4->B * dec4->H * dec4->W * ((plain ? 3 : 4 + 3) + 3 + (pair_first ? 9 : 0)) * (want ? 2.0 : 1.0));
    c.wrote(out); c.wrote(pair);
    *out_p = out;
    if (pair_p) *pair_p = pair;
    if (!want) return ACLGAN_OK;
    c.push([=](aclgan_ctx& c) -> int {
        const float* dout = out->written() ? out->g : nullptr;
        const float* dpair = (pair && pair->written()) ? pair->g : nullptr;
        if (!dout && !dpair) return ACLGAN_OK;
        if (dout) CHK(c.acq(out));
        if (dpair) CHK(c.acq(pair));
        CHK(c.acq(dec4));
        if (!plain && bg->need_grad) CHK(c.acq(bg));
        if (plain) { RUN(plain_pair_bwd(dec4->B, dec4->H * dec4->W, dout, dpair, dec4->g, c.st)); return ACLGAN_OK; }
        float* dbg = bg->need_grad ? bg->g : nullptr;
        RUN(focus_blend_bwd(dec4->B, dec4->H * dec4->W, dec4->d, bg->d, dout, dpair, dec4->g, dbg, bg->gw ? 1 : 0, c.st));
        if (dbg) mark_written(bg);
        return ACLGAN_OK;
    });
    return ACLGAN_OK;
}

int zero_grad_of(aclgan_ctx& c, Act* a) {
    if (a->need_grad) { RUN(fill_zero(a->g, a->numel(), c.st)); mark_written(a); }
    return ACLGAN_OK;
}

__global__ void scale_kernel(const float* s, float* d, float a, int n) {
    const int i = blockIdx.x * 256 + threadIdx.x;
    if (i < n) d[i] = a * s[i];
}

int pack_params(aclgan_ctx& c) {
    if (c.dtype == ACLGAN_DTYPE_FP32 || c.dry) return ACLGAN_OK;
    for (int g = 0; g < 2; ++g) {
        if (!c.w16[g] || !c.w16t[g]) { set_error("compute dtype is 16-bit but aclgan_bind_params16 was not called for group %d", g); return ACLGAN_EINVAL; }
        CHK(cast_flat16(c.weights(g), c.w16[g], c.groups[g].numel, c.dtype, c.st));
        CHK(transpose_flat16(c.weights(g), c.w16t[g], c.cv_off[g].data(), c.cv_co[g].data(), c.cv_taps[g].data(), c.cv_ci[g].data(),
                             (int)c.cv_off[g].size(), c.dtype, c.st));
    }
    return ACLGAN_OK;
// ... 23 lines not shown
```

### acl-gan_amd/csrc/engine_step.hip

```cpp
#include "engine.h"

namespace aclgan {

std::atomic<long long> g_enc_reuse_hits{0};

static int64_t dis_min_side(const aclgan_arch& a) {
    if (a.dis_n_layer + a.dis_num_scales > 30) return INT32_MAX;
    return (((int64_t)1 << a.dis_n_layer) - 1) * ((int64_t)1 << (a.dis_num_scales - 1)) + 1;
}
static int64_t content_min_side(const aclgan_arch& a) { return a.gen_n_downsample > 29 ? INT32_MAX : (int64_t)2 << a.gen_n_downsample; }
static const int STYLE_MIN_SIDE = 16;

static int check_shape(const aclgan_ctx& c, int B, int H, int W) {
    ACL_REQUIRE(B >= 1 && H >= 64 && W >= 64, "batch shape (%d,%d,%d): need B>=1 and H,W>=64 (third discriminator scale reflect-pads a >=2x2 map)", B, H, W);
    const aclgan_arch& a = c.arch;
    const int64_t dmin = dis_min_side(a), cmin = content_min_side(a);
    ACL_REQUIRE(H >= dmin && W >= dmin, "batch shape (%d,%d,%d): dis.n_layer %d at dis.num_scales %d needs H,W>=%lld (scale %d reflect-pads a >=2x2 map in each of its layers)",
                B, H, W, a.dis_n_layer, a.dis_num_scales, (long long)dmin, a.dis_num_scales - 1);
    ACL_REQUIRE(H >= cmin && W >= cmin, "batch shape (%d,%d,%d): gen.n_downsample %d needs H,W>=%lld (the ResBlocks reflect-pad a >=2x2 map)",
                B, H, W, a.gen_n_downsample, (long long)cmin);
    static_assert(STYLE_MIN_SIDE <= 64, "the style encoder's four stride-2 layers fit every admitted image");
    const int q = 1 << c.arch.gen_n_downsample;
    ACL_REQUIRE(H % q == 0 && W % q == 0, "H, W must be multiples of %d (2^n_downsample: decoder output must match the input size)", q);
    return ACLGAN_OK;
}

__global__ void gen_total_kernel(float* L, aclgan_hparams hp, float focus_scale) {
    float t = hp.gan_w * L[ACLGAN_L_GEN_ADV_A] + hp.gan_w * L[ACLGAN_L_GEN_ADV_B] + hp.gan_cw * L[ACLGAN_L_GEN_ADV_2];
    t += focus_scale * (L[ACLGAN_L_GEN_FOCUS_B_SIZE] + L[ACLGAN_L_GEN_FOCUS_B_DIGIT] + L[ACLGAN_L_GEN_FOCUS_A_SIZE] +
                        L[ACLGAN_L_GEN_FOCUS_A_DIGIT] + L[ACLGAN_L_GEN_FOCUS_A2_SIZE] + L[ACLGAN_L_GEN_FOCUS_A2_DIGIT]);
    t += hp.recon_x_w * L[ACLGAN_L_IDT_A] + hp.recon_x_w * L[ACLGAN_L_IDT_B];
    L[ACLGAN_L_GEN_TOTAL] = t;
}
__global__ void dis_total_kernel(float* L, aclgan_hparams hp) {
    L[ACLGAN_L_DIS_TOTAL] = hp.gan_w * L[ACLGAN_L_DIS_A] + hp.gan_w * L[ACLGAN_L_DIS_B] + hp.gan_cw * L[ACLGAN_L_DIS_2];
}

struct StepIn { Act *xa, *xb, *z1, *z2, *z3, *c1, *c2; };
static int step_inputs(aclgan_ctx& c, const float* x_a, const float* x_b, const float* z, int B, int H, int W, float alpha, bool train, StepIn* s) {
    const int sd = c.arch.gen_style_dim;
    CHK(c.lanes_begin(sw(SW_LANES)));
    CHK(pack_params(c));
    CHK(input_act(c, x_a, B, 3, H, W, &s->xa));
    CHK(input_act(c, x_b, B, 3, H, W, &s->xb));
    CHK(wrap_vec(c, z, B, sd, 1.f, &s->z1));
    CHK(wrap_vec(c, z + (size_t)B * sd, B, sd, alpha, &s->z2));
    CHK(wrap_vec(c, z + (size_t)2 * B * sd, B, sd, 1.f, &s->z3));
    CHK(prefill_on_side_lane(c, B, H, W, train));
    return ACLGAN_OK;
}
static int encode_x_a(aclgan_ctx& c, bool train, int L0, int L1, StepIn* s) {
    CHK(c.mark());
    CHK(c.set_lane(L0));
    c.carry_pass_begin(0);
    { const int rc = content_encode(c, ACLGAN_NET_GEN_AB, train, s->xa, &s->c1); c.carry_pass_end(); CHK(rc); } CHK(c.mark());
    CHK(c.set_lane(L1));
    c.carry_pass_begin(1);
    { const int rc = content_encode(c, ACLGAN_NET_GEN_BA, train, s->xa, &s->c2); c.carry_pass_end(); CHK(rc); } CHK(c.mark());
    return ACLGAN_OK;
}

static int modeseek_pair(aclgan_ctx& c, int net, Act* content, Act* zu, Act* zu2, Act* xa, Act* img, int dir) {
    Act *dec = nullptr, *img2 = nullptr;
    CHK(decode(c, net, true, content, zu2, &dec)); CHK(c.mark());
    CHK(zero_grad_of(c, dec));
    CHK(blend(c, dec, xa, nullptr, &img2, nullptr)); CHK(c.mark());
    const int B = img->B, sd = zu->H * zu->W * zu->C;
    const int64_t n = (int64_t)img->H * img->W * img->C;
    ACL_REQUIRE(img->need_grad && img2->need_grad && img->dt == img2->dt && img->gdt == 0 && img2->gdt == 0, "modeseek: the image pair takes fp32 gradients");
    float* part = c.allocf((int64_t)modeseek_scratch_floats(B, n));
    NEED(part);
    CHK(c.need(img));
    RUN(modeseek_part(img->d, img2->d, img->dt, B, n, part, c.st));
    c.count((img->dt ? 2.0 : 4.0) * 4.0 * (double)B * (double)n + 4.0 * 3.0 * (double)B * (double)n);
    c.push([=](aclgan_ctx& c) -> int {
        CHK(c.acq(img)); CHK(c.acq(img2));
        const int acc = (img->written() ? 1 : 0) | (img2->written() ? 2 : 0);
        RUN(modeseek_grad(img->d, img2->d, img->dt, B, n, part, zu->d, zu2->d, sd, 1.f, c.ms_lambda / (float)B, c.lscale, c.ms_out + 4 * dir, img->g, img2->g,
                          acc, c.st));
        mark_written(img); mark_written(img2);
        return ACLGAN_OK;
    });
    return ACLGAN_OK;
}

static int gen_update_impl(aclgan_ctx& c, const float* x_a, const float* x_b, const float* z, int B, int H, int W,
                           const aclgan_hparams& hp, float* L) {
    CHK(check_shape(c, B, H, W));
    const bool focus = hp.focus_loss > 0.f;
    ACL_REQUIRE(c.arch.gen_output_dim == (focus ? 4 : 3), "focus_loss %s 0 needs gen.output_dim %d (trainer.py:107-121), the context was built with %d",
                focus ? ">" : "<=", focus ? 4 : 3, c.arch.gen_output_dim);
    const int AB = ACLGAN_NET_GEN_AB, BA = ACLGAN_NET_GEN_BA;
    const int nfs = 2 * focus_sums_blocks((int64_t)B * H * W);
    float* sums = c.allocf((int64_t)3 * nfs);
    NEED(sums);
    if (!c.dry) {
        CHK(zero_async(L, sizeof(float) * (ACLGAN_L_GEN_TOTAL + 1), c.st));
    }
    StepIn in;
    auto& [xa, xb, z1, z2, z3, c1, c2] = in;
    CHK(step_inputs(c, x_a, x_b, z, B, H, W, hp.alpha, true, &in));
    const bool ms = c.ms_on();
    Act *z4 = nullptr, *z5 = nullptr;
    if (ms) {
        const int sd = c.arch.gen_style_dim;
        CHK(wrap_vec(c, c.ms_z, B, sd, 1.f, &z4));
        CHK(wrap_vec(c, c.ms_z + (size_t)B * sd, B, sd, hp.alpha, &z5));
    }
    Act *s2, *c4, *s4, *c3;
    Act *dB4, *dA4, *xB, *xA, *pA1, *rA4, *rB4, *dA24, *xA2, *pA2;
    Act* jA = c.new_act(2 * B, H, W, 3, true);
    Act* jP = c.new_act(2 * B, H, W, 6, true);
    NEED_ACT(jA); NEED_ACT(jP);
    const int L0 = 0, L1 = 1, L2 = c.nlanes > 2 ? 2 : 1, LS = c.nlanes > 2 ? 2 : 0;
#define PASS(expr) do { CHK(expr); CHK(c.mark()); } while (0)
    CHK(encode_x_a(c, true, L0, L1, &in));
    if (c.carry_call == ACLGAN_CARRY_ADOPT && !c.dry) { c.carry.valid = false; g_enc_reuse_hits += 2; }
    PASS(style_encode(c, BA, true, xa, &s2));
    CHK(c.set_lane(L0));
    PASS(decode(c, AB, true, c1, z1, &dB4)); CHK(zero_grad_of(c, dB4));
    PASS(blend(c, dB4, xa, nullptr, &xB, nullptr));
    if (ms) { CHK(c.set_lane(L2)); CHK(modeseek_pair(c, AB, c1, z1, z4, xa, xB, 0)); }
    CHK(c.set_lane(L1));
    PASS(decode(c, BA, true, c2, z2, &dA4)); CHK(zero_grad_of(c, dA4));
    Act *vA1 = c.new_view(jA, 0, B), *vP1 = c.new_view(jP, 0, B), *vA2 = c.new_view(jA, B, B), *vP2 = c.new_view(jP, B, B);
    PASS(blend(c, dA4, xa, xa, &xA, &pA1, vA1, vP1));
    if (ms) CHK(modeseek_pair(c, BA, c2, z2, z5, xa, xA, 1));
    CHK(c.set_lane(L0));
    PASS(content_encode(c, BA, true, xB, &c3));
    PASS(decode(c, BA, true, c3, z3, &dA24)); CHK(zero_grad_of(c, dA24));
    PASS(blend(c, dA24, xB, xa, &xA2, &pA2, vA2, vP2));
    CHK(c.set_lane(L1));
    PASS(decode(c, BA, true, c2, s2, &rA4)); CHK(zero_grad_of(c, rA4));
    CHK(c.set_lane(L2));
    PASS(content_encode(c, AB, true, xb, &c4));
    PASS(style_encode(c, AB, true, xb, &s4));
    PASS(decode(c, AB, true, c4, s4, &rB4)); CHK(zero_grad_of(c, rB4));
    PASS(dis_lsgan(c, ACLGAN_NET_DIS_B, false, xB, B, 2 * B, {{1.f, 1.f, hp.gan_w, L + ACLGAN_L_GEN_ADV_B}}, L1, LS));
    if (c.dis_norm != ACLGAN_NORM_SN) {
        PASS(dis_lsgan(c, ACLGAN_NET_DIS_A, false, jA, B, 0, {{1.f, 0.5f, hp.gan_w, L + ACLGAN_L_GEN_ADV_A}, {1.f, 0.5f, hp.gan_w, L + ACLGAN_L_GEN_ADV_A}}, L0, L2));
        PASS(dis_lsgan(c, ACLGAN_NET_DIS_2, false, jP, B, 3 * B, {{1.f, 1.f, hp.gan_cw, L + ACLGAN_L_GEN_ADV_2},
                                                            {0.f, 1.f, hp.gan_cw, L + ACLGAN_L_GEN_ADV_2}}, L1, LS));
    } else {
        PASS(dis_lsgan(c, ACLGAN_NET_DIS_A, false, vA1, B, 0, {{1.f, 0.5f, hp.gan_w, L + ACLGAN_L_GEN_ADV_A}}, L0, L2));
        PASS(dis_lsgan(c, ACLGAN_NET_DIS_A, false, vA2, B, B, {{1.f, 0.5f, hp.gan_w, L + ACLGAN_L_GEN_ADV_A}}, L0, L2));
        PASS(dis_lsgan(c, ACLGAN_NET_DIS_2, false, vP1, B, 3 * B, {{1.f, 1.f, hp.gan_cw, L + ACLGAN_L_GEN_ADV_2}}, L1, LS));
        PASS(dis_lsgan(c, ACLGAN_NET_DIS_2, false, vP2, B, 4 * B, {{0.f, 1.f, hp.gan_cw, L + ACLGAN_L_GEN_ADV_2}}, L1, LS));
    }
    CHK(c.lanes_join());
    const int64_t npix = (int64_t)B * H * W;
    const float fscale = hp.focus_loss / (float)H / (float)W / (float)B / 3.f;
    struct { Act* a; int size_slot; int digit_slot; } fl[3] = {
        {dB4, ACLGAN_L_GEN_FOCUS_B_SIZE, ACLGAN_L_GEN_FOCUS_B_DIGIT},
        {dA4, ACLGAN_L_GEN_FOCUS_A_SIZE, ACLGAN_L_GEN_FOCUS_A_DIGIT},
        {dA24, ACLGAN_L_GEN_FOCUS_A2_SIZE, ACLGAN_L_GEN_FOCUS_A2_DIGIT}};
    float* ftot = nullptr;
    if (c.sync_fn) { ftot = c.allocf(8); NEED(ftot); }
    for (int i = 0; i < 3 && focus; ++i) RUN(focus_sums(fl[i].a->d, npix, hp.focus_epsilon, hp.focus_upper, sums + (size_t)i * nfs, c.st));
    if (c.mask_dst && !c.dry) {
        unsigned char* dst = nullptr;
        for (int i = 0; i < 3 && focus; ++i) {
            CHK(c.mask_push(B, H, W, fl[i].a->C, 100, (size_t)fl[i].a->numel(), &dst));
            RUN(positive_mask(fl[i].a->d, fl[i].a->dt, dst, fl[i].a->numel(), c.st));
        }
        Act* rr[2] = {rA4, rB4}; Act* xx[2] = {xa, xb};
        for (int i = 0; i < 2; ++i) {
            CHK(c.mask_push(B, H, W, 3, 101, (size_t)npix * 3, &dst));
            RUN(positive_mask_diff(rr[i]->d, rr[i]->C, xx[i]->d, 3, dst, npix, c.st));
        }
    }
    c.count(4.0 * (double)npix * ((focus ? 3 * 2 : 0) + 2 * (4 + 3 + 4)));
    if (ftot && focus) {
        RUN(focus_totals(sums, npix, 3, ftot, c.st));
        if (!c.dry) c.sync_fn(c.sync_user, ftot, 6);
    }
    for (int i = 0; i < 3 && focus; ++i)
        RUN(focus_loss_finish(fl[i].a->d, npix, sums + (size_t)i * nfs, hp.focus_delta, hp.focus_upper, hp.focus_lower, hp.focus_epsilon, fscale,
                              L + fl[i].size_slot, L + fl[i].digit_slot, fl[i].a->g, c.st, c.lscale, ftot ? ftot + 2 * i : nullptr,
                              npix * (int64_t)c.sync_world));
    {
        const size_t mark = c.top;
        float* l1p = c.allocf(2 * L1_PART_FLOATS);
        NEED(l1p);
        RUN(l1_loss(rA4->d, rA4->C, xa->d, npix, L + ACLGAN_L_IDT_A, rA4->g, hp.recon_x_w, 1, c.st, c.lscale, l1p));
        RUN(l1_loss(rB4->d, rB4->C, xb->d, npix, L + ACLGAN_L_IDT_B, rB4->g, hp.recon_x_w, 1, c.st, c.lscale, l1p + L1_PART_FLOATS));
        c.top = mark;
    }
    if (!c.dry) {
        hipLaunchKernelGGL(gen_total_kernel, dim3(1), dim3(1), 0, c.st, L, hp, ftot ? fscale / (float)c.sync_world : fscale);
        ACL_CHECK_LAUNCH("gen_total_kernel");
    }
    return run_tape(c);
}

static int dis_update_impl(aclgan_ctx& c, const float* x_a, const float* x_b, const float* z, int B, int H, int W,
                           const aclgan_hparams& hp, float* L) {
    struct InDisUpdate {
        bool& f;
        explicit InDisUpdate(bool& flag) : f(flag) { f = true; }
        ~InDisUpdate() { f = false; }
    } in_dis_update(c.in_dis_update);
    CHK(check_shape(c, B, H, W));
    const bool focus = hp.focus_loss > 0.f;
    ACL_REQUIRE(c.arch.gen_output_dim == (focus ? 4 : 3), "focus_loss %s 0 needs gen.output_dim %d (trainer.py:266-276), the context was built with %d",
                focus ? ">" : "<=", focus ? 4 : 3, c.arch.gen_output_dim);
    const int AB = ACLGAN_NET_GEN_AB, BA = ACLGAN_NET_GEN_BA;
    if (!c.dry) {
        CHK(zero_async(L + ACLGAN_L_DIS_A, sizeof(float) * 4, c.st));
        if (c.lecam_state)
            CHK(zero_async(c.lecam_state + 18 * c.arch.dis_num_scales, sizeof(float) * 3, c.st));
    }
    StepIn in;
    auto& [xa, xb, z1, z2, z3, c1, c2] = in;
    CHK(step_inputs(c, x_a, x_b, z, B, H, W, hp.alpha, false, &in));
    Act *c3, *dB4, *dA4, *dA24, *xB, *xA, *xA2, *pA1, *pA2;
    Act* jA = c.new_act(3 * B, H, W, 3, false);
    Act* jB = c.new_act(2 * B, H, W, 3, false);
    Act* jP = c.new_act(2 * B, H, W, 6, false);
    NEED_ACT(jA); NEED_ACT(jB); NEED_ACT(jP);
    if (!c.dry) {
        hipError_t e = hipMemcpyAsync(jA->d + (size_t)2 * xa->numel(), xa->d, sizeof(float) * xa->numel(), hipMemcpyDeviceToDevice, c.st);
        if (e == hipSuccess) e = hipMemcpyAsync(jB->d + (size_t)xb->numel(), xb->d, sizeof(float) * xb->numel(), hipMemcpyDeviceToDevice, c.st);
        if (e != hipSuccess) return hip_fail(e, "copy real images into the joint discriminator batch");
    }
    const int L0 = 0, L1 = 1, L2 = c.nlanes > 2 ? 2 : 1, LS = c.nlanes > 2 ? 2 : 0;
    CHK(encode_x_a(c, false, L0, L1, &in));
    CHK(c.set_lane(L0));
    PASS(decode(c, AB, false, c1, z1, &dB4));
    PASS(blend(c, dB4, xa, nullptr, &xB, nullptr, c.new_view(jB, 0, B), nullptr));
    CHK(c.set_lane(L1));
    PASS(decode(c, BA, false, c2, z2, &dA4));
    PASS(blend(c, dA4, xa, xa, &xA, &pA1, c.new_view(jA, 0, B), c.new_view(jP, 0, B)));
    const bool sn = c.dis_norm == ACLGAN_NORM_SN;
    if (!sn) PASS(dis_lsgan(c, ACLGAN_NET_DIS_B, true, jB, B, 3 * B, {{0.f, 1.f, hp.gan_w, L + ACLGAN_L_DIS_B}, {1.f, 1.f, hp.gan_w, L + ACLGAN_L_DIS_B}}, L1, L2));
    else {
        PASS(dis_lsgan(c, ACLGAN_NET_DIS_B, true, c.new_view(jB, 0, B), B, 3 * B, {{0.f, 1.f, hp.gan_w, L + ACLGAN_L_DIS_B}}, L1, L2));
        PASS(dis_lsgan(c, ACLGAN_NET_DIS_B, true, c.new_view(jB, B, B), B, 4 * B, {{1.f, 1.f, hp.gan_w, L + ACLGAN_L_DIS_B}}, L1, L2));
    }
    CHK(c.set_lane(L0));
    PASS(content_encode(c, BA, false, xB, &c3));
    PASS(decode(c, BA, false, c3, z3, &dA24));
    PASS(blend(c, dA24, xB, xa, &xA2, &pA2, c.new_view(jA, B, B), c.new_view(jP, B, B)));
    if (!sn) {
        PASS(dis_lsgan(c, ACLGAN_NET_DIS_A, true, jA, B, 0, {{0.f, 0.5f, hp.gan_w, L + ACLGAN_L_DIS_A}, {0.f, 0.5f, hp.gan_w, L + ACLGAN_L_DIS_A},
                                                           {1.f, 1.0f, hp.gan_w, L + ACLGAN_L_DIS_A}}, L0, L2));
        PASS(dis_lsgan(c, ACLGAN_NET_DIS_2, true, jP, B, 5 * B, {{0.f, 1.f, hp.gan_cw, L + ACLGAN_L_DIS_2}, {1.f, 1.f, hp.gan_cw, L + ACLGAN_L_DIS_2}}, L1, LS));
    } else {
        Act* vx = c.new_view(jA, 2 * B, B);
        PASS(dis_lsgan(c, ACLGAN_NET_DIS_A, true, c.new_view(jA, 0, B), B, 0, {{0.f, 0.5f, hp.gan_w, L + ACLGAN_L_DIS_A}}, L0, L2));
        PASS(dis_lsgan(c, ACLGAN_NET_DIS_A, true, vx, B, 2 * B, {{1.f, 0.5f, hp.gan_w, L + ACLGAN_L_DIS_A}}, L0, L2));
        PASS(dis_lsgan(c, ACLGAN_NET_DIS_A, true, c.new_view(jA, B, B), B, B, {{0.f, 0.5f, hp.gan_w, L + ACLGAN_L_DIS_A}}, L0, L2));
        PASS(dis_lsgan(c, ACLGAN_NET_DIS_A, true, vx, B, 2 * B, {{1.f, 0.5f, hp.gan_w, L + ACLGAN_L_DIS_A}}, L0, L2));
        PASS(dis_lsgan(c, ACLGAN_NET_DIS_2, true, c.new_view(jP, 0, B), B, 5 * B, {{0.f, 1.f, hp.gan_cw, L + ACLGAN_L_DIS_2}}, L1, LS));
        PASS(dis_lsgan(c, ACLGAN_NET_DIS_2, true, c.new_view(jP, B, B), B, 6 * B, {{1.f, 1.f, hp.gan_cw, L + ACLGAN_L_DIS_2}}, L1, LS));
    }
    CHK(c.lanes_join());
    if (!c.dry) {
        hipLaunchKernelGGL(dis_total_kernel, dim3(1), dim3(1), 0, c.st, L, hp);
        ACL_CHECK_LAUNCH("dis_total_kernel");
    }
    if (c.lecam_state) {
        c.count(2.0 * 4.0 * (double)lecam_state_floats(c.arch.dis_num_scales));
        RUN(lecam_fold(c.lecam_state, c.arch.dis_num_scales, c.lecam_decay, true, c.st));
    }
    if (c.ada_state) {
        c.count(2.0 * 4.0 * (double)ada_state_floats());
        RUN(ada_fold(c.ada_state, c.ada_target, c.ada_interval, c.ada_step, c.st));
    }
    return run_tape(c);
}
#undef PASS

}

extern "C" {

struct DryRun {
    aclgan_ctx& c; const aclgan_bucket_fn keep;
    DryRun(aclgan_ctx& c_, int trained, int carry, bool fire_dry, bool park) : c(c_), keep(c_.bucket_fn) {
        c.reset_step();
        c.dry = true; c.peak = 0; c.peak2 = 0; c.trained = trained; c.fire_dry = fire_dry;
        c.carry_call = carry; c.carry_res = 0;
        if (park) c.bucket_fn = nullptr;
    }
    ~DryRun() {
        c.bucket_fn = keep;
        c.dry = false; c.fire_dry = false; c.trained = -1;
        c.carry_call = ACLGAN_CARRY_OFF; c.carry_res = 0;
        c.reset_step();
        c.peak = 0; c.peak2 = 0;
    }
};
static int dry_update(aclgan_ctx& c, int which, int B, int H, int W, int trained, int carry, bool fire_dry, bool park, size_t* need = nullptr) {
    aclgan_hparams hp;
    memset(&hp, 0, sizeof hp);
    hp.focus_loss = c.arch.gen_output_dim == 4 ? 1.f : 0.f; hp.alpha = 1.f;
    DryRun scope(c, trained, carry, fire_dry, park);
    const int rc = which == 0 ? gen_update_impl(c, nullptr, nullptr, nullptr, B, H, W, hp, nullptr)
                              : dis_update_impl(c, nullptr, nullptr, nullptr, B, H, W, hp, nullptr);
    if (need) *need = c.peak + c.peak2 + 512 + (c.carry_res ? c.carry_res + 256 : 0);
    return rc;
}
int aclgan_workspace_bytes(aclgan_ctx* ctx, int B, int H, int W, size_t* out) {
    ACL_REQUIRE(ctx && out, "null argument");
    aclgan_ctx& c = *ctx;
    ACL_REQUIRE(c.groups[0].param && c.groups[1].param, "bind parameters first");
    size_t best = 0;
    for (int which = 0; which < 2; ++which)
        for (int carry = 0; carry <= (sw(SW_ENC_REUSE) ? 1 : 0); ++carry) {
            size_t pk = 0;
            CHK(dry_update(c, which, B, H, W, -1, !carry ? ACLGAN_CARRY_OFF : which == 0 ? ACLGAN_CARRY_ADOPT : ACLGAN_CARRY_KEEP, false, true, &pk));
            if (pk > best) best = pk;
        }
    *out = best + 4096;
    return ACLGAN_OK;
}
int aclgan_check_workspace(aclgan_ctx* ctx, int B, int H, int W) {
    ACL_REQUIRE(ctx, "null ctx");
    ACL_REQUIRE(ctx->groups[0].param && ctx->groups[1].param, "bind parameters first");
    size_t need = 0;
    CHK(aclgan_workspace_bytes(ctx, B, H, W, &need));
    if (!ctx->ws || ctx->ws_bytes < need) {
        set_error("workspace too small: bound %zu bytes, aclgan_workspace_bytes(%d, %d, %d) = %zu", ctx->ws ? ctx->ws_bytes : (size_t)0, B, H, W, need);
        return ACLGAN_ENOMEM;
    }
    return ACLGAN_OK;
}
int aclgan_step_algorithmic_bytes(aclgan_ctx* ctx, int which, int B, int H, int W, double* out) {
    ACL_REQUIRE(ctx && out && (which == 0 || which == 1), "bad argument");
    aclgan_ctx& c = *ctx;
    ACL_REQUIRE(c.groups[0].param && c.groups[1].param, "bind parameters first");
    c.alg_bytes = 0.0; c.exec_flops = 0.0;
    CHK(dry_update(c, which, B, H, W, which, c.last_mode[which], false, true));
    *out = c.alg_bytes + (4.0 + 28.0) * (double)c.groups[which].numel;
    if (which == ACLGAN_GROUP_GEN && c.ema) *out += 8.0 * (double)c.groups[which].numel;
    if (c.clip[which] && !c.lscale) *out += 4.0 * (double)c.groups[which].numel;
    return ACLGAN_OK;
}
int aclgan_step_executed_flops(aclgan_ctx* ctx, int which, int B, int H, int W, double* out) {
    double bytes = 0.0;
    CHK(aclgan_step_algorithmic_bytes(ctx, which, B, H, W, &bytes));
    *out = ctx->exec_flops;
    return ACLGAN_OK;
}
int aclgan_forward_workspace_bytes(aclgan_ctx* ctx, int B, int H, int W, size_t* out) {
    ACL_REQUIRE(ctx && out, "null argument");
    aclgan_ctx& c = *ctx;
    ACL_REQUIRE(c.groups[0].param && c.groups[1].param, "bind parameters first");
    ACL_REQUIRE(B >= 1 && H >= 4 && W >= 4, "bad shape (%d,%d,%d)", B, H, W);
    const int q = 1 << c.arch.gen_n_downsample, C = c.arch.gen_dim << c.arch.gen_n_downsample;
    size_t best = 0;
    for (int which = 0; which < 3; ++which) {
        DryRun scope(c, -1, ACLGAN_CARRY_OFF, false, true);
        Act *x = nullptr, *o = nullptr, *s = nullptr;
        std::vector<Act*> outs;
        int rc = ACLGAN_OK;
        if (which == 0) {
            rc = input_act(c, nullptr, B, 3, H, W, &x);
            if (!rc) rc = content_encode(c, ACLGAN_NET_GEN_AB, false, x, &o);
            if (!rc && o && o->dt) c.allocf(o->numel());
            if (!rc) rc = style_encode(c, ACLGAN_NET_GEN_AB, false, x, &s);
        } else if (which == 1) {
            rc = input_act(c, nullptr, B, C, std::max(1, H / q), std::max(1, W / q), &x);
            if (!rc) rc = wrap_vec(c, nullptr, B, c.arch.gen_style_dim, 1.f, &s);
            if (!rc) rc = decode(c, ACLGAN_NET_GEN_AB, false, x, s, &o);
        } else if (std::min(H, W) >= std::max<int64_t>(64, dis_min_side(c.arch))) {
            rc = input_act(c, nullptr, B, c.arch.input_dim_b, H, W, &x);
            if (!rc) rc = dis_forward(c, ACLGAN_NET_DIS_2, false, x, &outs);
        }
        if (rc) return rc;
        if (c.peak > best) best = c.peak;
    }
    *out = best + 4096;
    return ACLGAN_OK;
}

static int step_common(aclgan_ctx* ctx, const float* x_a, const float* x_b, const float* z, const aclgan_hparams* hp, float* losses, void* stream, int group_trained,
                       int B, int H, int W) {
    ACL_REQUIRE(ctx && x_a && x_b && z && hp && losses, "null argument");
    ACL_REQUIRE(ctx->ws, "bind a workspace first (aclgan_workspace_bytes / aclgan_bind_workspace)");
    ACL_REQUIRE(ctx->groups[0].param && ctx->groups[1].param, "bind parameters first");
    ACL_REQUIRE(ctx->groups[group_trained].grad, "gradient buffer of the trained group is not bound");
    if (ctx->aug_policy) {
        const int want = (group_trained == 0 ? 5 : 7) * B;
        ACL_REQUIRE(ctx->aug_params, "%s with augmentation policy %d needs the parameter rows: aclgan_ctx_set_augment was given params = NULL",
                    group_trained == 0 ? "gen_update" : "dis_update", ctx->aug_policy);
        ACL_REQUIRE(ctx->aug_rows == want, "%s at B = %d reads %d augmentation rows (%d B), aclgan_ctx_set_augment was given %d",
                    group_trained == 0 ? "gen_update" : "dis_update", B, want, group_trained == 0 ? 5 : 7, ctx->aug_rows);
    }
    if (group_trained == 0 && ctx->ms_on())
        ACL_REQUIRE(ctx->ms_rows == 2 * B, "gen_update at B = %d reads %d mode-seeking noise rows (2 B: z_4, z_5), aclgan_ctx_set_modeseek was given %d", B, 2 * B, ctx->ms_rows);
    int carry = ctx->carry_arm;
    ctx->carry_arm = ACLGAN_CARRY_OFF;
    if (carry != (group_trained == 0 ? ACLGAN_CARRY_ADOPT : ACLGAN_CARRY_KEEP) || !sw(SW_ENC_REUSE) || ctx->mask_dst || sw(SW_FAULT_AT) >= 0) carry = ACLGAN_CARRY_OFF;
    if (carry && stream_capturing((hipStream_t)stream) != 0) carry = ACLGAN_CARRY_OFF;
    if (carry == ACLGAN_CARRY_ADOPT) {
        const aclgan_ctx::CarryRec& r = ctx->carry;
        if (!(r.valid && r.B == B && r.H == H && r.W == W && r.dtype == ctx->dtype && r.x_a == x_a && r.gen_epoch == ctx->gen_epoch &&
              r.tune_epoch == tuning_epoch() && r.determ == sw(SW_DETERMINISTIC) && r.ws == ctx->ws && r.ws_bytes == ctx->ws_bytes))
            carry = ACLGAN_CARRY_OFF;
    }
    if (carry != ACLGAN_CARRY_ADOPT) ctx->carry.valid = false;
    if (check_shape(*ctx, B, H, W) == ACLGAN_OK) {
        for (;;) {
            const aclgan_ctx::NeedKey key{group_trained, B, H, W, ctx->dtype, tuning_epoch(), sw(SW_DETERMINISTIC), (ctx->bucket_elems > 0 ? 1 : 0) | (carry << 1) | (ctx->aug_policy << 3) | ((group_trained == 0 && ctx->ms_on() ? 1 : 0) << 6)};
            auto it = ctx->need_cache.find(key);
            if (it == ctx->need_cache.end()) {
                size_t need = 0;
                CHK(dry_update(*ctx, group_trained, B, H, W, -1, carry, false, true, &need));
                it = ctx->need_cache.emplace(key, need).first;
            }
            if (it->second <= ctx->ws_bytes) break;
            if (carry) { carry = ACLGAN_CARRY_OFF; ctx->carry.valid = false; continue; }
            set_error("workspace too small: bound %zu bytes, this update needs %zu (aclgan_workspace_bytes)", ctx->ws_bytes, it->second);
            return ACLGAN_ENOMEM;
        }
    } else carry = ACLGAN_CARRY_OFF;
    ctx->reset_step();
    ctx->st = (hipStream_t)stream; ctx->dry = false; ctx->peak = 0; ctx->peak2 = 0; ctx->trained = group_trained;
    ctx->carry_call = carry; ctx->carry_mode = ACLGAN_CARRY_OFF; ctx->carry_fail = false;
    ctx->carry_res = carry == ACLGAN_CARRY_ADOPT ? ctx->carry.bytes : 0;
    if (carry == ACLGAN_CARRY_KEEP) { ctx->carry.blocks[0].clear(); ctx->carry.blocks[1].clear(); }
    ctx->last_mode[group_trained] = carry;
    ctx->ucache_hook = WinoUCache{ctx, &aclgan_ctx::ucache_lookup};
    set_wino_ucache(&ctx->ucache_hook);
    const int rc = (group_trained == 0 ? gen_update_impl : dis_update_impl)(*ctx, x_a, x_b, z, B, H, W, *hp, losses);
    set_wino_ucache(nullptr);
    if (rc) ctx->lanes_quiesce();
    if (group_trained == 0) ctx->carry.valid = false;
    else if (ctx->carry_call == ACLGAN_CARRY_KEEP) {
        aclgan_ctx::CarryRec& r = ctx->carry;
        r.valid = rc == ACLGAN_OK && !ctx->carry_fail && ctx->carry_res > 0;
        r.B = B; r.H = H; r.W = W; r.dtype = ctx->dtype; r.determ = sw(SW_DETERMINISTIC); r.x_a = x_a;
        r.gen_epoch = ctx->gen_epoch; r.tune_epoch = tuning_epoch(); r.ws = ctx->ws; r.ws_bytes = ctx->ws_bytes; r.bytes = ctx->carry_res;
    }
    ctx->carry_call = ACLGAN_CARRY_OFF; ctx->carry_res = 0;
    ctx->reset_step();
    return rc;
}
int aclgan_gen_update(aclgan_ctx* ctx, const float* x_a, const float* x_b, const float* z, int B, int H, int W,
                      const aclgan_hparams* hp, float* losses, void* stream) {
    return step_common(ctx, x_a, x_b, z, hp, losses, stream, 0, B, H, W);
}
int aclgan_dis_update(aclgan_ctx* ctx, const float* x_a, const float* x_b, const float* z, int B, int H, int W,
                      const aclgan_hparams* hp, float* losses, void* stream) {
    return step_common(ctx, x_a, x_b, z, hp, losses, stream, 1, B, H, W);
}

int aclgan_bucket_schedule(aclgan_ctx* ctx, int group, int B, int H, int W, int fire, int* order, int cap, int* count) {
    ACL_REQUIRE(ctx && count && group >= 0 && group <= 1, "bad argument");
    aclgan_ctx& c = *ctx;
    ACL_REQUIRE(c.groups[0].param && c.groups[1].param && c.groups[group].grad, "bind parameters (and the group's gradient buffer) first");
    ACL_REQUIRE(c.bucket_elems > 0, "aclgan_set_grad_buckets first");
    CHK(dry_update(c, group, B, H, W, group, ACLGAN_CARRY_OFF, fire != 0, false));
    *count = (int)c.bucket_order.size();
    for (int i = 0; i < *count && i < cap && order; ++i) order[i] = c.bucket_order[i];
    return ACLGAN_OK;
}

static int fwd_begin(aclgan_ctx* ctx, void* stream) {
    ACL_REQUIRE(ctx && ctx->ws, "bind a workspace first");
    ACL_REQUIRE(ctx->groups[0].param && ctx->groups[1].param, "bind parameters first");
    ctx->carry.valid = false; ctx->carry_arm = ACLGAN_CARRY_OFF; ctx->carry_res = 0;
    ctx->reset_step();
    ctx->st = (hipStream_t)stream; ctx->dry = false; ctx->peak = 0; ctx->peak2 = 0; ctx->trained = -1;
    ctx->read_ema = ctx->fwd_weights == ACLGAN_WEIGHTS_EMA;
    return ACLGAN_OK;
}

int aclgan_gen_encode(aclgan_ctx* ctx, int net, const float* x, int B, int H, int W, float* content, float* style, void* stream) {
    CHK(fwd_begin(ctx, stream));
    ACL_REQUIRE(net == ACLGAN_NET_GEN_AB || net == ACLGAN_NET_GEN_BA, "encode: net must be a generator");
    aclgan_ctx& c = *ctx;
    CHK(pack_params(c));
    Act *xa = nullptr, *cc = nullptr, *ss = nullptr;
    int rc = input_act(c, x, B, 3, H, W, &xa);
    if (!rc && content) {
        rc = content_encode(c, net, false, xa, &cc);
        const float* src = cc ? cc->d : nullptr;
        if (!rc && cc->dt) {
            float* tmp = c.allocf(cc->numel());
            if (!tmp) { set_error("workspace too small"); rc = ACLGAN_ENOMEM; }
            else { rc = cast_storage(cc->d, cc->dt, tmp, 0, cc->numel(), c.st); src = tmp; }
        }
        if (!rc) rc = nhwc_to_nchw(src, content, cc->B, cc->C, cc->H, cc->W, c.st);
    }
    if (!rc && style) {
        rc = style_encode(c, net, false, xa, &ss);
        if (!rc) { hipError_t e = hipMemcpyAsync(style, ss->d, sizeof(float) * ss->numel(), hipMemcpyDeviceToDevice, c.st); if (e != hipSuccess) rc = hip_fail(e, "copy style"); }
    }
    c.reset_step();
    return rc;
}

int aclgan_gen_decode(aclgan_ctx* ctx, int net, const float* content, const float* style, int B, int h, int w, float* out, void* stream) {
    CHK(fwd_begin(ctx, stream));
    ACL_REQUIRE(net == ACLGAN_NET_GEN_AB || net == ACLGAN_NET_GEN_BA, "decode: net must be a generator");
    aclgan_ctx& c = *ctx;
    CHK(pack_params(c));
    const int C = c.arch.gen_dim << c.arch.gen_n_downsample;
    Act *cc = nullptr, *ss = nullptr, *o = nullptr;
    int rc = input_act(c, content, B, C, h, w, &cc);
    if (!rc) rc = wrap_vec(c, style, B, c.arch.gen_style_dim, 1.f, &ss);
    if (!rc) rc = decode(c, net, false, cc, ss, &o);
    if (!rc) rc = nhwc_to_nchw(o->d, out, o->B, o->C, o->H, o->W, c.st);
    c.reset_step();
    return rc;
}

int aclgan_dis_forward(aclgan_ctx* ctx, int net, const float* x, int B, int H, int W, float* const* outs, void* stream) {
    CHK(fwd_begin(ctx, stream));
    ACL_REQUIRE(net >= ACLGAN_NET_DIS_A && net <= ACLGAN_NET_DIS_2, "dis_forward: net must be a discriminator");
    aclgan_ctx& c = *ctx;
    CHK(pack_params(c));
    const int Cin = net == ACLGAN_NET_DIS_2 ? c.arch.input_dim_b : c.arch.input_dim_a;
    Act* xa = nullptr;
    std::vector<Act*> o;
    int rc = input_act(c, x, B, Cin, H, W, &xa);
    if (!rc) rc = dis_forward(c, net, false, xa, &o);
    for (size_t s = 0; !rc && s < o.size(); ++s) {
        hipError_t e = hipMemcpyAsync(outs[s], o[s]->d, sizeof(float) * o[s]->numel(), hipMemcpyDeviceToDevice, c.st);
        if (e != hipSuccess) rc = hip_fail(e, "copy dis out");
    }
    c.reset_step();
    return rc;
}

}
```

### acl-gan_amd/csrc/misc.hip

```cpp
#include "common.h"
#include "st16.h"

namespace aclgan {

__device__ __forceinline__ float act_grad_m(float y, int act) {
    if (act == ACLGAN_ACT_RELU) return y > 0.f ? 1.f : 0.f;
    if (act == ACLGAN_ACT_LRELU) return y > 0.f ? 1.f : 0.2f;
    if (act == ACLGAN_ACT_TANH) return 1.f - y * y;
    return 1.f;
}
__device__ __forceinline__ float act_fwd_m(float v, int act) {
    if (act == ACLGAN_ACT_RELU) return v > 0.f ? v : 0.f;
    if (act == ACLGAN_ACT_LRELU) return v > 0.f ? v : 0.2f * v;
    if (act == ACLGAN_ACT_TANH) return tanhf(v);
    return v;
}
__device__ __forceinline__ float wave_sum_m(float v) {
#pragma unroll
    for (int o = 32; o > 0; o >>= 1) v += __shfl_xor(v, o);
    return v;
}
__device__ __forceinline__ float block_sum_t0(float v) {
    __shared__ float red[4];
    v = wave_sum_m(v);
    if ((threadIdx.x & 63) == 0) red[threadIdx.x >> 6] = v;
    __syncthreads();
    const float r = red[0] + red[1] + red[2] + red[3];
    __syncthreads();
    return r;
}

__global__ void act_bwd_kernel(const float* __restrict__ y, float* __restrict__ dy, int act, int64_t n) {
    for (int64_t i = (int64_t)blockIdx.x * 256 + threadIdx.x; i < n; i += (int64_t)gridDim.x * 256)
        dy[i] *= act_grad_m(y[i], act);
}
__global__ void act_bwd_st_kernel(const void* __restrict__ y, int yst, void* __restrict__ dy, int gst, int act, int64_t n4) {
    for (int64_t i = (int64_t)blockIdx.x * 256 + threadIdx.x; i < n4; i += (int64_t)gridDim.x * 256) {
        const st_f32x4 yv = st_ld4(y, i, yst);
        st_f32x4 g = st_ld4(dy, i, gst);
#pragma unroll
        for (int e = 0; e < 4; ++e) g[e] *= act_grad_m(yv[e], act);
        st_st4(dy, i, g, gst);
    }
}
__global__ void __launch_bounds__(256) act_bwd_v4_kernel(const st_f32x4* __restrict__ y, st_f32x4* __restrict__ dy, int act, int64_t n4) {
    const int64_t stride = (int64_t)gridDim.x * 256;
    int64_t i = (int64_t)blockIdx.x * 256 + threadIdx.x;
    for (; i + 3 * stride < n4; i += 4 * stride) {
        st_f32x4 yv[4], g[4];
#pragma unroll
        for (int u = 0; u < 4; ++u) { yv[u] = y[i + u * stride]; g[u] = dy[i + u * stride]; }
#pragma unroll
        for (int u = 0; u < 4; ++u) {
#pragma unroll
            for (int e = 0; e < 4; ++e) g[u][e] *= act_grad_m(yv[u][e], act);
            dy[i + u * stride] = g[u];
        }
    }
    for (; i < n4; i += stride) {
        const st_f32x4 yv = y[i];
        st_f32x4 g = dy[i];
#pragma unroll
        for (int e = 0; e < 4; ++e) g[e] *= act_grad_m(yv[e], act);
        dy[i] = g;
    }
}
int act_bwd_inplace(int act, const void* y, void* dy, int64_t n, hipStream_t st, int yst, int gst) {
    if (act == ACLGAN_ACT_NONE || n == 0) return ACLGAN_OK;
    if (yst == ST_F32 && gst == ST_F32 && n % 4 == 0 && (((uintptr_t)y | (uintptr_t)dy) & 15) == 0) {
        const int grid = (int)std::min<int64_t>(cdiv64(n / 4, 256 * 4), 8192);
        hipLaunchKernelGGL(act_bwd_v4_kernel, dim3(std::max(grid, 1)), dim3(256), 0, st, (const st_f32x4*)y, (st_f32x4*)dy, act, n / 4);
        ACL_CHECK_LAUNCH("act_bwd_v4_kernel");
        return ACLGAN_OK;
    }
    if (yst == ST_F32 && gst == ST_F32) {
        const int grid = (int)std::min<int64_t>(cdiv64(n, 256), 8192);
        hipLaunchKernelGGL(act_bwd_kernel, dim3(grid), dim3(256), 0, st, (const float*)y, (float*)dy, act, n);
        ACL_CHECK_LAUNCH("act_bwd_kernel");
        return ACLGAN_OK;
    }
    ACL_REQUIRE(n % 4 == 0, "act_bwd: %lld elements of a 16-bit tensor (must be a multiple of 4)", (long long)n);
    hipLaunchKernelGGL(act_bwd_st_kernel, dim3((int)std::min<int64_t>(cdiv64(n / 4, 256), 8192)), dim3(256), 0, st, y, yst, dy, gst, act, n / 4);
    ACL_CHECK_LAUNCH("act_bwd_st_kernel");
    return ACLGAN_OK;
}

__global__ void positive_mask_kernel(const void* __restrict__ y, int yst, unsigned char* __restrict__ dst, int64_t n4) {
    for (int64_t i = (int64_t)blockIdx.x * 256 + threadIdx.x; i < n4; i += (int64_t)gridDim.x * 256) {
        const st_f32x4 v = st_ld4(y, i, yst);
        uchar4 m;
        m.x = v[0] > 0.f; m.y = v[1] > 0.f; m.z = v[2] > 0.f; m.w = v[3] > 0.f;
        reinterpret_cast<uchar4*>(dst)[i] = m;
    }
}
int positive_mask(const void* y, int yst, unsigned char* dst, int64_t n, hipStream_t st) {
    ACL_REQUIRE(n % 4 == 0, "positive_mask: %lld elements (must be a multiple of 4)", (long long)n);
    if (n == 0) return ACLGAN_OK;
    hipLaunchKernelGGL(positive_mask_kernel, dim3((int)std::min<int64_t>(cdiv64(n / 4, 256), 8192)), dim3(256), 0, st, y, yst, dst, n / 4);
    ACL_CHECK_LAUNCH("positive_mask_kernel");
    return ACLGAN_OK;
}

__global__ void positive_mask_diff_kernel(const float* __restrict__ a, int ca, const float* __restrict__ b, int cb, unsigned char* __restrict__ dst, int64_t n) {
    for (int64_t i = (int64_t)blockIdx.x * 256 + threadIdx.x; i < n; i += (int64_t)gridDim.x * 256) {
        const int64_t pix = i / cb; const int ch = (int)(i - pix * cb);
        dst[i] = a[pix * ca + ch] > b[pix * cb + ch];
    }
}
int positive_mask_diff(const float* a, int ca, const float* b, int cb, unsigned char* dst, int64_t npix, hipStream_t st) {
    const int64_t n = npix * cb;
    if (n == 0) return ACLGAN_OK;
    hipLaunchKernelGGL(positive_mask_diff_kernel, dim3((int)std::min<int64_t>(cdiv64(n, 256), 8192)), dim3(256), 0, st, a, ca, b, cb, dst, n);
    ACL_CHECK_LAUNCH("positive_mask_diff_kernel");
    return ACLGAN_OK;
}

__global__ void cast_storage_kernel(const void* __restrict__ src, int sst, void* __restrict__ dst, int dst_st, int64_t n4) {
    for (int64_t i = (int64_t)blockIdx.x * 256 + threadIdx.x; i < n4; i += (int64_t)gridDim.x * 256) st_st4(dst, i, st_ld4(src, i, sst), dst_st);
}
int cast_storage(const void* src, int src_st, void* dst, int dst_st, int64_t n, hipStream_t st) {
    ACL_REQUIRE(n % 4 == 0, "cast_storage: n %% 4 != 0");
    if (n == 0) return ACLGAN_OK;
    hipLaunchKernelGGL(cast_storage_kernel, dim3((int)std::min<int64_t>(cdiv64(n / 4, 256), 8192)), dim3(256), 0, st, src, src_st, dst, dst_st, n / 4);
    ACL_CHECK_LAUNCH("cast_storage_kernel");
    return ACLGAN_OK;
}

__global__ void fill_zero_kernel(float* p, int64_t n) {
    for (int64_t i = (int64_t)blockIdx.x * 256 + threadIdx.x; i < n; i += (int64_t)gridDim.x * 256) p[i] = 0.f;
}
int zero_async(void* p, size_t bytes, hipStream_t st) {
    if (bytes == 0) return ACLGAN_OK;
    hipStreamCaptureStatus cs = hipStreamCaptureStatusNone;
    if (hipStreamIsCapturing(st, &cs) != hipSuccess) { (void)hipGetLastError(); cs = hipStreamCaptureStatusNone; }
    if (cs != hipStreamCaptureStatusNone && bytes % sizeof(float) == 0 && (uintptr_t)p % sizeof(float) == 0) {
        const int64_t n = (int64_t)(bytes / sizeof(float));
        hipLaunchKernelGGL(fill_zero_kernel, dim3((int)std::min<int64_t>(cdiv64(n, 256), 4096)), dim3(256), 0, st, (float*)p, n);
        ACL_CHECK_LAUNCH("fill_zero_kernel");
        return ACLGAN_OK;
    }
    hipError_t e = hipMemsetAsync(p, 0, bytes, st);
    if (e != hipSuccess) return hip_fail(e, "hipMemsetAsync");
    return ACLGAN_OK;
}
int fill_zero(float* p, int64_t n, hipStream_t st) { return zero_async(p, (size_t)n * sizeof(float), st); }

__global__ void avgpool_fwd_kernel(const float* __restrict__ x, float* __restrict__ y, int B, int H, int W, int C, int Ho, int Wo) {
    const int64_t n = (int64_t)B * Ho * Wo * C;
    for (int64_t i = (int64_t)blockIdx.x * 256 + threadIdx.x; i < n; i += (int64_t)gridDim.x * 256) {
        const int c = (int)(i % C);
        int64_t t = i / C;
        const int ox = (int)(t % Wo); t /= Wo;
        const int oy = (int)(t % Ho);
        const int b = (int)(t / Ho);
        float s = 0.f; int cnt = 0;
        for (int dy = -1; dy <= 1; ++dy) {
            const int iy = 2 * oy + dy;
            if (iy < 0 || iy >= H) continue;
            for (int dx = -1; dx <= 1; ++dx) {
                const int ix = 2 * ox + dx;
                if (ix < 0 || ix >= W) continue;
                s += x[((size_t)(b * H + iy) * W + ix) * C + c]; ++cnt;
            }
        }
        y[i] = s / (float)cnt;
    }
}
__device__ __forceinline__ int pool_cnt(int o, int n) {
    int c = 0;
    for (int d = -1; d <= 1; ++d) { const int i = 2 * o + d; c += (i >= 0 && i < n); }
    return c;
}
__global__ void avgpool_bwd_kernel(const float* __restrict__ dy, float* __restrict__ dx, int B, int H, int W, int C, int Ho, int Wo, int acc) {
    const int64_t n = (int64_t)B * H * W * C;
    for (int64_t i = (int64_t)blockIdx.x * 256 + threadIdx.x; i < n; i += (int64_t)gridDim.x * 256) {
        const int c = (int)(i % C);
        int64_t t = i / C;
        const int ix = (int)(t % W); t /= W;
        const int iy = (int)(t % H);
        const int b = (int)(t / H);
        float s = 0.f;
        for (int oy = (iy) / 2; oy <= (iy + 1) / 2; ++oy) {
            if (oy < 0 || oy >= Ho || 2 * oy - 1 > iy) continue;
            const int cy = pool_cnt(oy, H);
            for (int ox = (ix) / 2; ox <= (ix + 1) / 2; ++ox) {
                if (ox < 0 || ox >= Wo || 2 * ox - 1 > ix) continue;
                s += dy[((size_t)(b * Ho + oy) * Wo + ox) * C + c] / (float)(cy * pool_cnt(ox, W));
            }
        }
        dx[i] = acc ? dx[i] + s : s;
    }
}
int avgpool3s2_fwd(int B, int H, int W, int C, const float* x, float* y, hipStream_t st) {
    const int Ho = (H - 1) / 2 + 1, Wo = (W - 1) / 2 + 1;
    const int64_t n = (int64_t)B * Ho * Wo * C;
    hipLaunchKernelGGL(avgpool_fwd_kernel, dim3((int)std::min<int64_t>(cdiv64(n, 256), 4096)), dim3(256), 0, st, x, y, B, H, W, C, Ho, Wo);
    ACL_CHECK_LAUNCH("avgpool_fwd_kernel");
    return ACLGAN_OK;
}
int avgpool3s2_bwd(int B, int H, int W, int C, const float* dy, float* dx, int accumulate, hipStream_t st) {
    const int Ho = (H - 1) / 2 + 1, Wo = (W - 1) / 2 + 1;
    const int64_t n = (int64_t)B * H * W * C;
    hipLaunchKernelGGL(avgpool_bwd_kernel, dim3((int)std::min<int64_t>(cdiv64(n, 256), 4096)), dim3(256), 0, st, dy, dx, B, H, W, C, Ho, Wo, accumulate);
    ACL_CHECK_LAUNCH("avgpool_bwd_kernel");
    return ACLGAN_OK;
}

template <bool SCALED, bool EMA>
__device__ __forceinline__ void adam_pass(float* __restrict__ p, const float* __restrict__ g, float* __restrict__ m, float* __restrict__ v, int64_t n,
                                          float b1, float b2, float eps, float wd, float step_size, float inv_sqrt_bc2, float inv,
                                          float* __restrict__ ema, float d, int blend) {
    for (int64_t i = (int64_t)blockIdx.x * 256 + threadIdx.x; i < n; i += (int64_t)gridDim.x * 256) {
        const float pv = p[i];
        const float gv = fmaf(wd, pv, SCALED ? g[i] * inv : g[i]);
        const float mv = fmaf(b1, m[i], (1.f - b1) * gv);
        const float vv = fmaf(b2, v[i], (1.f - b2) * gv * gv);
        m[i] = mv; v[i] = vv;
        const float pn = pv - step_size * mv / (sqrtf(vv) * inv_sqrt_bc2 + eps);
        p[i] = pn;
        if (EMA) ema[i] = blend ? fmaf(d, ema[i], (1.f - d) * pn) : pn;
    }
}
__global__ void adam_kernel(float* __restrict__ p, const float* __restrict__ g, float* __restrict__ m, float* __restrict__ v,
                            int64_t n, float b1, float b2, float eps, float wd, float step_size, float inv_sqrt_bc2) {
    adam_pass<false, false>(p, g, m, v, n, b1, b2, eps, wd, step_size, inv_sqrt_bc2, 1.f, nullptr, 0.f, 0);
}
__global__ void adam_ema_kernel(float* __restrict__ p, const float* __restrict__ g, float* __restrict__ m, float* __restrict__ v,
                                int64_t n, float b1, float b2, float eps, float wd, float step_size, float inv_sqrt_bc2,
                                float* __restrict__ ema, float d, int blend) {
    adam_pass<false, true>(p, g, m, v, n, b1, b2, eps, wd, step_size, inv_sqrt_bc2, 1.f, ema, d, blend);
}
static int ema_args_ok(const float* ema, float decay, int mode) {
    ACL_REQUIRE(ema, "adam (EMA): the average's buffer is null");
    ACL_REQUIRE(mode == ACLGAN_EMA_COPY || mode == ACLGAN_EMA_BLEND, "adam (EMA): mode %d is neither ACLGAN_EMA_COPY nor ACLGAN_EMA_BLEND", mode);
    ACL_REQUIRE(mode == ACLGAN_EMA_COPY || (decay >= 0.f && decay < 1.f), "adam (EMA): decay %g outside [0, 1)", (double)decay);
    return ACLGAN_OK;
}
static int adam_launch(float* p, const float* g, float* m, float* v, float* ema, int64_t n, const aclgan_adam* o, int step, float decay, int mode, hipStream_t st) {
    ACL_REQUIRE(step >= 1, "adam: step must be >= 1");
    const double bc1 = 1.0 - pow((double)o->beta1, step), bc2 = 1.0 - pow((double)o->beta2, step);
    const int grid = (int)std::min<int64_t>(cdiv64(n, 256), 16384);
    const float step_size = (float)(o->lr / bc1), inv_sqrt_bc2 = (float)(1.0 / sqrt(bc2));
    if (ema) {
        hipLaunchKernelGGL(adam_ema_kernel, dim3(grid), dim3(256), 0, st, p, g, m, v, n, o->beta1, o->beta2, o->eps, o->weight_decay,
                           step_size, inv_sqrt_bc2, ema, decay, mode == ACLGAN_EMA_BLEND ? 1 : 0);
        ACL_CHECK_LAUNCH("adam_ema_kernel");
        return ACLGAN_OK;
    }
    hipLaunchKernelGGL(adam_kernel, dim3(grid), dim3(256), 0, st, p, g, m, v, n, o->beta1, o->beta2, o->eps, o->weight_decay,
                       step_size, inv_sqrt_bc2);
    ACL_CHECK_LAUNCH("adam_kernel");
    return ACLGAN_OK;
}
int adam_flat(float* p, const float* g, float* m, float* v, int64_t n, const aclgan_adam* o, int step, hipStream_t st) {
    return adam_launch(p, g, m, v, nullptr, n, o, step, 0.f, ACLGAN_EMA_COPY, st);
}
int adam_flat_ema(float* p, const float* g, float* m, float* v, float* ema, int64_t n, const aclgan_adam* o, int step, float decay, int mode, hipStream_t st) {
    const int rc = ema_args_ok(ema, decay, mode);
    return rc ? rc : adam_launch(p, g, m, v, ema, n, o, step, decay, mode, st);
}

__global__ void grad_check_kernel(const float* __restrict__ g, int64_t n, float* state) {
    bool bad = false;
    for (int64_t i = (int64_t)blockIdx.x * 256 + threadIdx.x; i < n; i += (int64_t)gridDim.x * 256) bad |= !isfinite(g[i]);
    if (bad) state[3] = 1.f;
}
template <bool EMA, bool CLIP = false>
__device__ __forceinline__ void adam_scaled_pass(float* __restrict__ p, const float* __restrict__ g, float* __restrict__ m, float* __restrict__ v, int64_t n,
                                                 float b1, float b2, float eps, float wd, float lr, int step_host, const float* __restrict__ state, int group,
                                                 float* __restrict__ ema, float d, int blend, const float* __restrict__ clip = nullptr) {
    if (state[3] != 0.f) return;
    if (CLIP && !isfinite(clip[0])) return;
    const int step = step_host - (int)state[4 + group] - (CLIP ? (int)clip[3] : 0);
    const double bc1 = 1.0 - pow((double)b1, (double)step), bc2 = 1.0 - pow((double)b2, (double)step);
    const float step_size = (float)((double)lr / bc1), inv_sqrt_bc2 = (float)(1.0 / sqrt(bc2)), inv = CLIP ? state[1] * clip[1] : state[1];
    adam_pass<true, EMA>(p, g, m, v, n, b1, b2, eps, wd, step_size, inv_sqrt_bc2, inv, ema, d, blend);
}
__global__ void adam_scaled_kernel(float* __restrict__ p, const float* __restrict__ g, float* __restrict__ m, float* __restrict__ v,
                                   int64_t n, float b1, float b2, float eps, float wd, float lr, int step_host, const float* __restrict__ state, int group) {
    adam_scaled_pass<false>(p, g, m, v, n, b1, b2, eps, wd, lr, step_host, state, group, nullptr, 0.f, 0);
}
__global__ void adam_scaled_ema_kernel(float* __restrict__ p, const float* __restrict__ g, float* __restrict__ m, float* __restrict__ v,
                                       int64_t n, float b1, float b2, float eps, float wd, float lr, int step_host, const float* __restrict__ state, int group,
                                       float* __restrict__ ema, float d, int blend) {
    adam_scaled_pass<true>(p, g, m, v, n, b1, b2, eps, wd, lr, step_host, state, group, ema, d, blend);
}
__global__ void adam_scaled_clip_kernel(float* __restrict__ p, const float* __restrict__ g, float* __restrict__ m, float* __restrict__ v,
                                        int64_t n, float b1, float b2, float eps, float wd, float lr, int step_host, const float* __restrict__ state, int group,
                                        const float* __restrict__ clip) {
    adam_scaled_pass<false, true>(p, g, m, v, n, b1, b2, eps, wd, lr, step_host, state, group, nullptr, 0.f, 0, clip);
}
__global__ void adam_scaled_clip_ema_kernel(float* __restrict__ p, const float* __restrict__ g, float* __restrict__ m, float* __restrict__ v,
                                            int64_t n, float b1, float b2, float eps, float wd, float lr, int step_host, const float* __restrict__ state, int group,
                                            const float* __restrict__ clip, float* __restrict__ ema, float d, int blend) {
    adam_scaled_pass<true, true>(p, g, m, v, n, b1, b2, eps, wd, lr, step_host, state, group, ema, d, blend, clip);
}
template <bool EMA>
__device__ __forceinline__ void adam_clip_pass(float* __restrict__ p, const float* __restrict__ g, float* __restrict__ m, float* __restrict__ v, int64_t n,
                                               float b1, float b2, float eps, float wd, float lr, int step_host, float step_size, float inv_sqrt_bc2,
                                               const float* __restrict__ clip, float* __restrict__ ema, float d, int blend) {
    if (!isfinite(clip[0])) return;
    const int skipped = (int)clip[3];
    if (skipped != 0) {
        const int step = max(step_host - skipped, 1);
        const double bc1 = 1.0 - pow((double)b1, (double)step), bc2 = 1.0 - pow((double)b2, (double)step);
        step_size = (float)((double)lr / bc1); inv_sqrt_bc2 = (float)(1.0 / sqrt(bc2));
    }
    adam_pass<true, EMA>(p, g, m, v, n, b1, b2, eps, wd, step_size, inv_sqrt_bc2, clip[1], ema, d, blend);
}
__global__ void adam_clip_kernel(float* __restrict__ p, const float* __restrict__ g, float* __restrict__ m, float* __restrict__ v,
                                 int64_t n, float b1, float b2, float eps, float wd, float lr, int step_host, float step_size, float inv_sqrt_bc2,
                                 const float* __restrict__ clip) {
    adam_clip_pass<false>(p, g, m, v, n, b1, b2, eps, wd, lr, step_host, step_size, inv_sqrt_bc2, clip, nullptr, 0.f, 0);
}
__global__ void adam_clip_ema_kernel(float* __restrict__ p, const float* __restrict__ g, float* __restrict__ m, float* __restrict__ v,
                                     int64_t n, float b1, float b2, float eps, float wd, float lr, int step_host, float step_size, float inv_sqrt_bc2,
                                     const float* __restrict__ clip, float* __restrict__ ema, float d, int blend) {
    adam_clip_pass<true>(p, g, m, v, n, b1, b2, eps, wd, lr, step_host, step_size, inv_sqrt_bc2, clip, ema, d, blend);
}
__global__ void scale_update_kernel(float* state, int group) {
    state[7] = state[0];
    if (state[3] != 0.f) {
        state[0] = fmaxf(state[0] * 0.5f, 1.f); state[2] = 0.f; state[4 + group] += 1.f;
    } else {
        state[2] += 1.f;
        const float interval = state[6] > 0.f ? state[6] : 2000.f;
        if (state[2] >= interval) { state[0] = fminf(state[0] * 2.f, 16777216.f); state[2] = 0.f; }
    }
    state[1] = 1.f / state[0];
    state[3] = 0.f;
}
static int adam_scaled_launch(float* p, const float* g, float* m, float* v, float* ema, int64_t n, const aclgan_adam* o, int step, float decay, int mode,
                         float* state, int group, hipStream_t st) {
    ACL_REQUIRE(step >= 1 && state && (group == 0 || group == 1), "adam (loss-scaled): bad arguments");
    const int grid = (int)std::min<int64_t>(cdiv64(n, 256), 16384);
    hipLaunchKernelGGL(grad_check_kernel, dim3(grid), dim3(256), 0, st, g, n, state);
    ACL_CHECK_LAUNCH("grad_check_kernel");
    if (ema) {
        hipLaunchKernelGGL(adam_scaled_ema_kernel, dim3(grid), dim3(256), 0, st, p, g, m, v, n, o->beta1, o->beta2, o->eps, o->weight_decay, o->lr, step, state, group,
                           ema, decay, mode == ACLGAN_EMA_BLEND ? 1 : 0);
        ACL_CHECK_LAUNCH("adam_scaled_ema_kernel");
    } else {
        hipLaunchKernelGGL(adam_scaled_kernel, dim3(grid), dim3(256), 0, st, p, g, m, v, n, o->beta1, o->beta2, o->eps, o->weight_decay, o->lr, step, state, group);
        ACL_CHECK_LAUNCH("adam_scaled_kernel");
    }
    hipLaunchKernelGGL(scale_update_kernel, dim3(1), dim3(1), 0, st, state, group);
    ACL_CHECK_LAUNCH("scale_update_kernel");
    return ACLGAN_OK;
}
int adam_flat_clipped(float* p, const float* g, float* m, float* v, float* ema, int64_t n, const aclgan_adam* o, int step, float decay, int mode,
                      float* state, int group, float max_norm, float* clip, hipStream_t st) {
    ACL_REQUIRE(step >= 1 && clip && (group == 0 || group == 1), "adam (clipped): bad arguments");
    if (ema) { const int rc = ema_args_ok(ema, decay, mode); if (rc) return rc; }
    const int rc = gradnorm_launch(g, n, max_norm, clip, state, st);
    if (rc) return rc;
    const int grid = (int)std::min<int64_t>(cdiv64(n, 256), 16384);
    const int blend = mode == ACLGAN_EMA_BLEND ? 1 : 0;
    if (state) {
        if (ema) {
            hipLaunchKernelGGL(adam_scaled_clip_ema_kernel, dim3(grid), dim3(256), 0, st, p, g, m, v, n, o->beta1, o->beta2, o->eps, o->weight_decay, o->lr, step,
                               (const float*)state, group, (const float*)clip, ema, decay, blend);
            ACL_CHECK_LAUNCH("adam_scaled_clip_ema_kernel");
        } else {
            hipLaunchKernelGGL(adam_scaled_clip_kernel, dim3(grid), dim3(256), 0, st, p, g, m, v, n, o->beta1, o->beta2, o->eps, o->weight_decay, o->lr, step,
                               (const float*)state, group, (const float*)clip);
            ACL_CHECK_LAUNCH("adam_scaled_clip_kernel");
        }
        hipLaunchKernelGGL(scale_update_kernel, dim3(1), dim3(1), 0, st, state, group);
        ACL_CHECK_LAUNCH("scale_update_kernel");
        return ACLGAN_OK;
    }
    const double bc1 = 1.0 - pow((double)o->beta1, step), bc2 = 1.0 - pow((double)o->beta2, step);
    const float step_size = (float)(o->lr / bc1), inv_sqrt_bc2 = (float)(1.0 / sqrt(bc2));
    if (ema) {
        hipLaunchKernelGGL(adam_clip_ema_kernel, dim3(grid), dim3(256), 0, st, p, g, m, v, n, o->beta1, o->beta2, o->eps, o->weight_decay, o->lr, step,
                           step_size, inv_sqrt_bc2, (const float*)clip, ema, decay, blend);
        ACL_CHECK_LAUNCH("adam_clip_ema_kernel");
    } else {
        hipLaunchKernelGGL(adam_clip_kernel, dim3(grid), dim3(256), 0, st, p, g, m, v, n, o->beta1, o->beta2, o->eps, o->weight_decay, o->lr, step,
                           step_size, inv_sqrt_bc2, (const float*)clip);
        ACL_CHECK_LAUNCH("adam_clip_kernel");
    }
    return ACLGAN_OK;
}
int adam_flat_scaled(float* p, const float* g, float* m, float* v, int64_t n, const aclgan_adam* o, int step, float* state, int group, hipStream_t st) {
    return adam_scaled_launch(p, g, m, v, nullptr, n, o, step, 0.f, ACLGAN_EMA_COPY, state, group, st);
}
int adam_flat_scaled_ema(float* p, const float* g, float* m, float* v, float* ema, int64_t n, const aclgan_adam* o, int step, float decay, int mode,
                              float* state, int group, hipStream_t st) {
    const int rc = ema_args_ok(ema, decay, mode);
    return rc ? rc : adam_scaled_launch(p, g, m, v, ema, n, o, step, decay, mode, state, group, st);
}

__global__ void nchw2nhwc_kernel(const float* __restrict__ s, float* __restrict__ d, int C, int HW, int64_t n) {
    for (int64_t i = (int64_t)blockIdx.x * 256 + threadIdx.x; i < n; i += (int64_t)gridDim.x * 256) {
        const int c = (int)(i % C);
        const int64_t t = i / C;
        const int p = (int)(t % HW);
        const int64_t b = t / HW;
        d[i] = s[(b * C + c) * HW + p];
    }
}
__global__ void nhwc2nchw_kernel(const float* __restrict__ s, float* __restrict__ d, int C, int HW, int64_t n) {
    for (int64_t i = (int64_t)blockIdx.x * 256 + threadIdx.x; i < n; i += (int64_t)gridDim.x * 256) {
        const int p = (int)(i % HW);
        const int64_t t = i / HW;
        const int c = (int)(t % C);
        const int64_t b = t / C;
        d[i] = s[(b * HW + p) * C + c];
    }
}
int nchw_to_nhwc(const float* src, float* dst, int B, int C, int H, int W, hipStream_t st) {
    const int64_t n = (int64_t)B * C * H * W;
    hipLaunchKernelGGL(nchw2nhwc_kernel, dim3((int)std::min<int64_t>(cdiv64(n, 256), 8192)), dim3(256), 0, st, src, dst, C, H * W, n);
    ACL_CHECK_LAUNCH("nchw2nhwc_kernel");
    return ACLGAN_OK;
}
int nhwc_to_nchw(const float* src, float* dst, int B, int C, int H, int W, hipStream_t st) {
    const int64_t n = (int64_t)B * C * H * W;
    hipLaunchKernelGGL(nhwc2nchw_kernel, dim3((int)std::min<int64_t>(cdiv64(n, 256), 8192)), dim3(256), 0, st, src, dst, C, H * W, n);
    ACL_CHECK_LAUNCH("nhwc2nchw_kernel");
    return ACLGAN_OK;
}

__global__ void __launch_bounds__(64) linear_fwd_kernel(const float* __restrict__ x, const float* __restrict__ w,
                                                        const float* __restrict__ bias, float* __restrict__ y, int B, int I, int O, int act) {
    const int o = blockIdx.x, b0 = blockIdx.y * 8, lane = threadIdx.x;
// ... 609 lines not shown
```

### acl-gan_amd/csrc/switches.h

```cpp
#pragma once
#include <atomic>

namespace aclgan {

enum SwitchId {
    SW_LANES, SW_U_BATCH, SW_NORM_MASK, SW_MLP_FUSED, SW_FAULT_AT, SW_ENC_REUSE, SW_DGRAD_RING,
    SW_GLDS_TILE, SW_WINO_X3, SW_WINO_FUSED, SW_WINO_WGRAD_FUSED, SW_WINO_S2K4, SW_DGRAD16S_DIRECT, SW_FWD16_PATCH,
    SW_DETERMINISTIC,
    SW_NOFAST, SW_NOUP5, SW_SPLIT_NWG,
    SW_NOWGKC, SW_NOUP5DGRAD,
    SW_NOSTATFUSE, SW_NOKEEPV, SW_NODIRECT,
    SW_NOWGRAD16S, SW_WGRAD16S_MINPIX, SW_NOGLDS16,
    SW_NOSMALL, SW_NOTHIN,
    SW_NOWINO, SW_NOWINOUP5, SW_WINO_VEC, SW_WINO_VEC3,
    SW_ROCTX, SW_NOUCACHE, SW_ACT16, SW_CO16, SW_SIDE_STREAM, SW_KEEPV_BUDGET_GB,
    SW_COUNT
};

const long long SW_BIAS = 1ll << 32;
extern std::atomic<long long> g_switches[SW_COUNT];
int sw_latch(SwitchId id);
inline int sw(SwitchId id) {
    const long long e = g_switches[id].load(std::memory_order_relaxed);
    return e ? (int)(e - SW_BIAS) : sw_latch(id);
}
double sw_real(SwitchId id);
int sw_set(SwitchId id, int v);

long long tuning_epoch();

}
```

### acl-gan_amd/csrc/switches.hip

```cpp
#include <string.h>
#include "common.h"

#include <climits>
#include <cmath>
#include <cstdlib>

namespace aclgan {

namespace {

enum Rule {
    R_INT,
    R_BOOL,
    R_NOT,
    R_CLAMP,
    R_RANGE,
    R_LOW4,
    R_ONEOF,
};
enum { SETTABLE = 1,
       EMPTY_UNSET = 2 };

struct Switch {
    const char* key;
    const char* env;
    int dflt;
    Rule rule;
    int lo, hi;
    int flags;
    double (*parse)(const char*);
};

double parse_real(const char* s) { return atof(s); }
const int VEC_124 = (1 << 1) | (1 << 2) | (1 << 4);

const Switch kSwitches[SW_COUNT] = {
    {"lanes",             "ACLGAN_LANES",             3,  R_CLAMP, 1, 3,       SETTABLE | EMPTY_UNSET, nullptr},
    {"u_batch",           "ACLGAN_U_BATCH",           1,  R_BOOL,  0, 0,       SETTABLE | EMPTY_UNSET, nullptr},
    {"norm_mask",         "ACLGAN_NORM_MASK",         1,  R_BOOL,  0, 0,       SETTABLE | EMPTY_UNSET, nullptr},
    {"mlp_fused",         "ACLGAN_MLP_FUSED",         1,  R_BOOL,  0, 0,       SETTABLE | EMPTY_UNSET, nullptr},
    {"fault_at",          nullptr,                    -1, R_INT,   0, 0,       SETTABLE, nullptr},
    {"enc_reuse",         nullptr,                    1,  R_BOOL,  0, 0,       SETTABLE, nullptr},
    {"dgrad_ring",        nullptr,                    1,  R_BOOL,  0, 0,       SETTABLE, nullptr},
    {"glds_tile",         "ACLGAN_GLDS_TILE",         0,  R_CLAMP, 0, INT_MAX, SETTABLE, nullptr},
    {"wino_x3",           "ACLGAN_WINO_X3",           0,  R_BOOL,  0, 0,       SETTABLE, nullptr},
    {"wino_fused",        "ACLGAN_WINO_FUSED",        1,  R_LOW4,  0, 2,       SETTABLE, nullptr},
    {"wino_wgrad_fused",  "ACLGAN_WINO_WGRAD_FUSED",  1,  R_RANGE, 0, 2,       SETTABLE, nullptr},
    {"wino_s2k4",         "ACLGAN_NOWINOS2",          1,  R_NOT,   0, 0,       SETTABLE, nullptr},
    {"dgrad16s_direct",   "ACLGAN_DGRAD16S_DIRECT",   0,  R_BOOL,  0, 0,       SETTABLE, nullptr},
    {"fwd16_patch",       "ACLGAN_FWD16_PATCH",       1,  R_LOW4,  0, 2,       SETTABLE, nullptr},
    {"deterministic",     "ACLGAN_DETERMINISTIC",     0,  R_BOOL,  0, 0,       0, nullptr},
    {"nofast",            "ACLGAN_NOFAST",            0,  R_BOOL,  0, 0,       0, nullptr},
    {"noup5",             "ACLGAN_NOUP5",             0,  R_BOOL,  0, 0,       0, nullptr},
    {"split_nwg",         "ACLGAN_SPLIT_NWG",         256, R_INT,  0, 0,       0, nullptr},
    {"nowgkc",            "ACLGAN_NOWGKC",            0,  R_BOOL,  0, 0,       0, nullptr},
    {"noup5dgrad",        "ACLGAN_NOUP5DGRAD",        0,  R_BOOL,  0, 0,       0, nullptr},
    {"nostatfuse",        "ACLGAN_NOSTATFUSE",        0,  R_BOOL,  0, 0,       0, nullptr},
    {"nokeepv",           "ACLGAN_NOKEEPV",           0,  R_BOOL,  0, 0,       0, nullptr},
    {"nodirect",          "ACLGAN_NODIRECT",          0,  R_BOOL,  0, 0,       0, nullptr},
    {"nowgrad16s",        "ACLGAN_NOWGRAD16S",        0,  R_BOOL,  0, 0,       0, nullptr},
    {"wgrad16s_minpix",   "ACLGAN_WGRAD16S_MINPIX",   64, R_INT,   0, 0,       0, nullptr},
    {"noglds16",          "ACLGAN_NOGLDS16",          0,  R_BOOL,  0, 0,       0, nullptr},
    {"nosmall",           "ACLGAN_NOSMALL",           0,  R_BOOL,  0, 0,       0, nullptr},
    {"nothin",            "ACLGAN_NOTHIN",            0,  R_BOOL,  0, 0,       0, nullptr},
    {"nowino",            "ACLGAN_NOWINO",            0,  R_BOOL,  0, 0,       0, nullptr},
    {"nowinoup5",         "ACLGAN_NOWINOUP5",         0,  R_BOOL,  0, 0,       0, nullptr},
    {"wino_vec",          "ACLGAN_WINO_VEC",          2,  R_ONEOF, VEC_124, 0, 0, nullptr},
    {"wino_vec3",         "ACLGAN_WINO_VEC3",         2,  R_ONEOF, VEC_124, 0, 0, nullptr},
    {"roctx",             "ACLGAN_ROCTX",             0,  R_BOOL,  0, 0,       0, nullptr},
    {"noucache",          "ACLGAN_NOUCACHE",          0,  R_BOOL,  0, 0,       0, nullptr},
    {"act16",             "ACLGAN_ACT16",             1,  R_BOOL,  0, 0,       0, nullptr},
    {"co16",              "ACLGAN_CO16",              1,  R_BOOL,  0, 0,       0, nullptr},
    {"side_stream",       "ACLGAN_SIDE_STREAM",       1,  R_BOOL,  0, 0,       0, nullptr},
    {"keepv_budget_gb",   "ACLGAN_KEEPV_BUDGET_GB",   64, R_INT,   0, 0,       0, parse_real},
};

int normalise(const Switch& s, int v, bool from_env) {
    switch (s.rule) {
    case R_INT: return v;
    case R_BOOL: return v ? 1 : 0;
    case R_NOT: return (v ? 1 : 0) ^ (from_env ? 1 : 0);
    case R_CLAMP: return v < s.lo ? s.lo : v > s.hi ? s.hi : v;
    case R_RANGE: return (v < s.lo || v > s.hi) ? s.dflt : v;
    case R_LOW4: return (v < 0 || (v & 15) < s.lo || (v & 15) > s.hi) ? s.dflt : v;
    case R_ONEOF: return (v >= 0 && v < 31 && ((s.lo >> v) & 1)) ? v : s.dflt;
    }
    return v;
}

std::atomic<double> g_real[SW_COUNT];
std::atomic<long long> g_tuning_epoch{0};

int find(const char* key) {
    for (int i = 0; i < SW_COUNT; ++i)
        if (!strcmp(key, kSwitches[i].key)) return i;
    return -1;
}

}

std::atomic<long long> g_switches[SW_COUNT];

int sw_latch(SwitchId id) {
    const Switch& s = kSwitches[id];
    const char* e = s.env ? getenv(s.env) : nullptr;
    if (e && !*e && (s.flags & EMPTY_UNSET)) e = nullptr;
    int v = s.dflt;
    if (e && s.parse) {
        const double r = s.parse(e);
        g_real[id].store(r, std::memory_order_relaxed);
        v = std::isfinite(r) && std::fabs(r) < 2e9 ? (int)r : 0;
    } else if (e) {
        v = normalise(s, atoi(e), true);
    } else if (s.parse) {
        g_real[id].store(s.dflt, std::memory_order_relaxed);
    }
    long long expected = 0;
    return g_switches[id].compare_exchange_strong(expected, v + SW_BIAS, std::memory_order_release, std::memory_order_acquire) ? v : (int)(expected - SW_BIAS);
}

double sw_real(SwitchId id) {
    if (!g_switches[id].load(std::memory_order_acquire)) sw_latch(id);
    return g_real[id].load(std::memory_order_relaxed);
}

int sw_set(SwitchId id, int v) {
    sw(id);
    return (int)(g_switches[id].exchange(normalise(kSwitches[id], v, false) + SW_BIAS) - SW_BIAS);
}

long long tuning_epoch() { return g_tuning_epoch.load(); }

}

using namespace aclgan;

extern "C" {

int aclgan_set_deterministic(int on) { sw_set(SW_DETERMINISTIC, on); return ACLGAN_OK; }
int aclgan_get_deterministic(void) { return sw(SW_DETERMINISTIC); }

int aclgan_tuning(const char* key, int value, int* previous) {
    ACL_REQUIRE(key, "aclgan_tuning: null key");
    const int i = find(key);
    if (i < 0) { set_error("aclgan_tuning: unknown key '%s'", key); return ACLGAN_EINVAL; }
    if (!(kSwitches[i].flags & SETTABLE)) { set_error("aclgan_tuning: key '%s' is read-only (set %s before the first use instead)", key, kSwitches[i].env); return ACLGAN_EINVAL; }
    const int old = sw_set((SwitchId)i, value);
    ++g_tuning_epoch;
    if (previous) *previous = old;
    return ACLGAN_OK;
}
int aclgan_tuning_get(const char* key, long long* value) {
    ACL_REQUIRE(key && value, "aclgan_tuning_get: null argument");
    if (!strcmp(key, "epoch")) { *value = tuning_epoch(); return ACLGAN_OK; }
    if (!strcmp(key, "enc_reuse_hits")) { *value = g_enc_reuse_hits.load(); return ACLGAN_OK; }
    const int i = find(key);
    if (i < 0) { set_error("aclgan_tuning_get: unknown key '%s'", key); return ACLGAN_EINVAL; }
    *value = sw((SwitchId)i);
    return ACLGAN_OK;
}
int aclgan_set_tuning(const char* key, int value) {
    int old = 0;
    return aclgan_tuning(key, value, &old) == ACLGAN_OK ? old : -1;
}

}
```

Baseline: 104.1.

## Share first decoder convolution across decodes of the same content code

Result: no change. 105.0 (median of 6 runs) (+0.9%).

```diff
diff --git a/acl-gan_amd/csrc/common.h b/acl-gan_amd/csrc/common.h
--- a/acl-gan_amd/csrc/common.h
+++ b/acl-gan_amd/csrc/common.h
@@ -14,6 +14,7 @@
 
 extern std::atomic<long long> g_launches;
 extern std::atomic<long long> g_enc_reuse_hits;
+extern std::atomic<long long> g_dec_share_hits;
 
 #define ACL_CHECK_LAUNCH(what)                                           \
     do {                                                                 \
@@ -164,6 +165,7 @@
 
 int act_bwd_inplace(int act, const void* y, void* dy, int64_t n, hipStream_t st, int yst = 0, int gst = 0);
 int cast_storage(const void* src, int src_st, void* dst, int dst_st, int64_t n, hipStream_t st);
+int add_storage(const void* src, void* dst, int st_, int64_t n, hipStream_t st);
 int positive_mask(const void* y, int yst, unsigned char* dst, int64_t n, hipStream_t st);
 int positive_mask_diff(const float* a, int ca, const float* b, int cb, unsigned char* dst, int64_t npix, hipStream_t st);
 int avgpool3s2_fwd(int B, int H, int W, int C, const float* x, float* y, hipStream_t st);
diff --git a/acl-gan_amd/csrc/engine.h b/acl-gan_amd/csrc/engine.h
--- a/acl-gan_amd/csrc/engine.h
+++ b/acl-gan_amd/csrc/engine.h
@@ -43,6 +43,18 @@
     Act* root() { return parent ? parent : this; }
     int64_t numel() const { return (int64_t)B * H * W * C; }
     bool written() const { return gw || (parent && parent->gw); }
+};
+
+struct aclgan_ctx_carry_slot { float *co = nullptr, *stats = nullptr; int B = 0, H = 0, W = 0, C = 0, co_st = 0, schunk = 0; bool set = false; };
+
+struct ConvShare {
+    bool merge = false;
+    Act* co = nullptr;
+    Act* in = nullptr;
+    float* stats = nullptr;
+    float* keepV = nullptr;
+    int schunk = 0;
+    aclgan_ctx_carry_slot* kept = nullptr;
 };
 
 struct PW {
@@ -125,6 +137,9 @@
     bool dry = false;
     size_t top = 0, peak = 0;
     std::vector<Act*> acts;
+    std::vector<ConvShare*> shares;
+    ConvShare* new_share(aclgan_ctx_carry_slot* kept = nullptr);
+    bool size_unshared = false;
     std::vector<TapeOp> tape;
     int dtype = ACLGAN_DTYPE_FP32;
     unsigned short* w16[2] = {nullptr, nullptr};
@@ -162,6 +177,9 @@
         long long gen_epoch = 0, tune_epoch = 0;
         char* ws = nullptr; size_t ws_bytes = 0, bytes = 0;
         std::vector<CarryBlock> blocks[2];
+        aclgan_ctx_carry_slot dec[2];
+        struct KeptU { bool set = false; const float* w0 = nullptr; int uv = 0, count = 0; size_t ubytes = 0; float* u0 = nullptr; };
+        KeptU u[2][2];
     };
     CarryRec carry;
     long long gen_epoch = 0;
@@ -294,7 +312,7 @@
 int prefill_on_side_lane(aclgan_ctx& c, int B, int H, int W, bool train);
 int content_encode(aclgan_ctx& c, int net, bool train, Act* x, Act** out);
 int style_encode(aclgan_ctx& c, int net, bool train, Act* x, Act** out);
-int decode(aclgan_ctx& c, int net, bool train, Act* content, Act* style, Act** out);
+int decode(aclgan_ctx& c, int net, bool train, Act* content, Act* style, Act** out, ConvShare* sh = nullptr);
 int dis_forward(aclgan_ctx& c, int net, bool train, Act* x, std::vector<Act*>* outs, int lane_a = -1, int lane_b = -1);
 int dis_lsgan(aclgan_ctx& c, int net, bool train, Act* x, int nb, int row0, const std::vector<LsSeg>& segs, int lane_a = -1, int lane_b = -1);
 int blend(aclgan_ctx& c, Act* dec4, Act* bg, Act* pair_first, Act** out_p, Act** pair_p, Act* out_dst = nullptr, Act* pair_dst = nullptr);
diff --git a/acl-gan_amd/csrc/engine.hip b/acl-gan_amd/csrc/engine.hip
--- a/acl-gan_amd/csrc/engine.hip
+++ b/acl-gan_amd/csrc/engine.hip
@@ -172,6 +172,8 @@
 void aclgan_ctx::reset_step() {
     for (Act* a : acts) delete a;
     acts.clear();
+    for (ConvShare* s : shares) delete s;
+    shares.clear();
     tape.clear();
     tape_pass.clear(); pass_names.clear(); pass_count.clear(); cur_pass = -1;
     top = 0;
@@ -201,6 +203,13 @@
     acts.push_back(a);
     wrote(a);
     return a;
+}
+ConvShare* aclgan_ctx::new_share(aclgan_ctx_carry_slot* kept) {
+    ConvShare* s = new ConvShare();
+    s->merge = !sw(SW_DETERMINISTIC);
+    s->kept = kept;
+    shares.push_back(s);
+    return s;
 }
 Act* aclgan_ctx::new_view(Act* joint, int b0, int nb) {
     Act* a = new Act();
diff --git a/acl-gan_amd/csrc/engine_graph.hip b/acl-gan_amd/csrc/engine_graph.hip
--- a/acl-gan_amd/csrc/engine_graph.hip
+++ b/acl-gan_amd/csrc/engine_graph.hip
@@ -3,7 +3,7 @@
 namespace aclgan {
 
 static int conv_block(aclgan_ctx& c, const PW& W, bool train_w, Act* in, int Co, int k, int stride, int pad, int up, int act,
-                      const NormSpec& ns, Act* residual, Act** out_p, int out16 = 1) {
+                      const NormSpec& ns, Act* residual, Act** out_p, int out16 = 1, ConvShare* sh = nullptr) {
     aclgan_conv_desc d;
     d.B = in->B; d.Hi = in->H; d.Wi = in->W; d.Ci = in->C; d.Co = Co; d.k = k; d.stride = stride; d.pad = pad; d.upsample = up;
     d.act = ns.kind == ACLGAN_NORM_NONE ? act : ACLGAN_ACT_NONE;
@@ -22,6 +22,11 @@
     const bool s_fwd = a16 && f16 && conv16s_ok(g, 0) && in->dt != 0;
     const bool keep = c.carry_mode == ACLGAN_CARRY_KEEP, adopt = c.carry_mode == ACLGAN_CARRY_ADOPT, carried = keep || adopt;
     const bool tw = train_w || keep;
+    const bool reuse = sh && sh->co;
+    const bool sh_keep = sh && !reuse && sh->kept && c.carry_call == ACLGAN_CARRY_KEEP, sh_adopt = sh && !reuse && sh->kept && c.carry_call == ACLGAN_CARRY_ADOPT;
+    const bool have_co = reuse || sh_adopt;
+    const bool merge = sh && sh->merge;
+    if (sh && (!has_norm || carried || residual)) { set_error("conv_block: a shared convolution feeds a normalisation layer outside the carried passes"); return ACLGAN_EINVAL; }
     aclgan_ctx::CarryBlock cb_dry = {};
     aclgan_ctx::CarryBlock* cb = &cb_dry;
     if (carried && !c.dry) {
@@ -43,7 +48,8 @@
         float* at = carried ? buf(slot, (size_t)B_ * H_ * W_ * C_ * (st ? 2 : 4)) : nullptr;
         return c.new_act(B_, H_, W_, C_, grad, st, carried ? &at : nullptr);
     };
-    if (in->dt != 0 && !(f16 && (w16 || !tw))) {
+    if (reuse) in = sh->in;
+    else if (in->dt != 0 && !(f16 && (w16 || !tw))) {
         Act* in32 = act_in(&aclgan_ctx::CarryBlock::in32, in->B, in->H, in->W, in->C, false, 0);
         NEED_ACT(in32);
         if (!adopt) RUN(cast_storage(in->d, in->dt, in32->d, 0, in->numel(), c.st));
@@ -56,11 +62,44 @@
         return ACLGAN_EINVAL;
     }
     if (keep) { cb->B = g.B; cb->H = g.Ho; cb->W = g.Wo; cb->C = Co; cb->co_st = co_st; cb->out_st = out_st; }
-    Act* co = act_in(&aclgan_ctx::CarryBlock::co, g.B, g.Ho, g.Wo, Co, want_grad, co_st);
+    int schunk = !has_norm ? 0 : (s_fwd ? conv_fwd16s_stats_chunk(g) : (!f16 ? conv_fwd_stats_chunk(g) : 0));
+    const int HW = g.Ho * g.Wo;
+    float* stats = nullptr;
+    Act* co = nullptr;
+    if (reuse) {
+        const Act* s = sh->co;
+        if (s->B != g.B || s->H != g.Ho || s->W != g.Wo || s->C != Co || s->dt != co_st || (want_grad && !s->need_grad)) {
+            set_error("conv_block: the shared convolution does not match this layer (%d x %d x %d x %d)", g.B, g.Ho, g.Wo, Co);
+            return ACLGAN_EINVAL;
+        }
+        CHK(c.need(sh->co));
+        co = merge ? sh->co : c.new_act(g.B, g.Ho, g.Wo, Co, want_grad, co_st, &sh->co->d);
+        stats = sh->stats; schunk = sh->schunk;
+    } else if (sh_keep || sh_adopt) {
+        aclgan_ctx_carry_slot& k = *sh->kept;
+        const size_t sbytes = schunk ? (size_t)2 * g.B * (HW / schunk) * Co * 4 : 0;
+        if (sh_adopt && !c.dry) {
+            if (!k.set || k.B != g.B || k.H != g.Ho || k.W != g.Wo || k.C != Co || k.co_st != co_st || k.schunk != schunk) {
+                set_error("conv_block: the kept decoder convolution does not match this layer (%d x %d x %d x %d)", g.B, g.Ho, g.Wo, Co);
+                return ACLGAN_EINVAL;
+            }
+            co = c.new_act(g.B, g.Ho, g.Wo, Co, want_grad, co_st, &k.co);
+            stats = k.stats;
+        } else {
+            float* at = (float*)c.alloc_carry((size_t)g.B * HW * Co * (co_st ? 2 : 4));
+            co = c.new_act(g.B, g.Ho, g.Wo, Co, want_grad, co_st, &at);
+            if (sbytes) { stats = (float*)c.alloc_carry(sbytes); NEED(stats); }
+            if (sh_keep && !c.dry) { k.co = at; k.stats = stats; k.B = g.B; k.H = g.Ho; k.W = g.Wo; k.C = Co; k.co_st = co_st; k.schunk = schunk; k.set = at != nullptr; }
+        }
+    } else {
+        co = act_in(&aclgan_ctx::CarryBlock::co, g.B, g.Ho, g.Wo, Co, want_grad, co_st);
+        if (sh && schunk) { stats = c.allocf((size_t)2 * g.B * (HW / schunk) * Co); NEED(stats); }
+    }
     NEED_ACT(co);
+    if (sh && !reuse) { sh->co = co; sh->in = in; sh->stats = stats; sh->schunk = schunk; }
+    if (have_co && !c.dry) ++g_dec_share_hits;
     Act* out = co;
     float *mean = nullptr, *rstd = nullptr, *ss = nullptr;
-    const int HW = g.Ho * g.Wo;
     if (has_norm) {
         out = act_in(&aclgan_ctx::CarryBlock::out, g.B, g.Ho, g.Wo, Co, want_grad, out_st);
         NEED_ACT(out);
@@ -81,22 +120,22 @@
     }
     if (gin->need_grad && !s_bwd) gin->gdt = 0;
     float* keepV = nullptr;
-    if (train_w && !adopt && !f16 && !w16) {
+    if (train_w && !adopt && !have_co && !f16 && !w16) {
         const size_t kb = conv_fwd_keep_bytes(g);
         if (kb && c.keep_total + kb <= (size_t)(sw_real(SW_KEEPV_BUDGET_GB) * 1073741824.0) + 1) { keepV = (float*)c.alloc(kb); NEED(keepV); c.keep_total += kb; }
-    }
+        if (sh) sh->keepV = keepV;
+    } else if (reuse && train_w) keepV = sh->keepV;
     const size_t ubytes = f16 ? 0 : conv_wino_u_bytes(g);
-    if (ubytes && !adopt && c.ucache_reserve(W.w, g.up ? 2 : 0, ubytes)) { set_error("workspace too small (filter-transform cache)"); return ACLGAN_ENOMEM; }
+    if (ubytes && !adopt && !have_co && c.ucache_reserve(W.w, g.up ? 2 : 0, ubytes)) { set_error("workspace too small (filter-transform cache)"); return ACLGAN_ENOMEM; }
     const double es_in = in->dt ? 2.0 : 4.0, es_co = co->dt ? 2.0 : 4.0, es_out = out->dt ? 2.0 : 4.0, es_w = f16 ? 2.0 : 4.0;
-    if (!adopt) c.count(es_in * (double)in->numel() + es_w * (double)Co * g.K + 4.0 * Co + es_co * (double)co->numel());
-    if (!adopt) c.exec_flops += conv_exec_flops(g, 0, f16);
+    const bool no_conv = adopt || have_co;
+    if (!no_conv) c.count(es_in * (double)in->numel() + es_w * (double)Co * g.K + 4.0 * Co + es_co * (double)co->numel());
+    if (!no_conv) c.exec_flops += conv_exec_flops(g, 0, f16);
     if (out != co && !adopt) c.count((es_co + es_out) * (double)co->numel() + ((has_norm && residual) ? (residual->dt ? 2.0 : 4.0) * (double)co->numel() : 0.0));
     const size_t mark = c.top;
     if (!adopt) {
-    const int schunk = !has_norm ? 0 : (s_fwd ? conv_fwd16s_stats_chunk(g) : (!f16 ? conv_fwd_stats_chunk(g) : 0));
-    float* stats = nullptr;
-    if (schunk) { stats = c.allocf((size_t)2 * g.B * (HW / schunk) * Co); NEED(stats); }
-    {
+    if (schunk && !stats) { stats = c.allocf((size_t)2 * g.B * (HW / schunk) * Co); NEED(stats); }
+    if (!have_co) {
         const size_t fmark = c.top;
         void* fscr = nullptr;
         const size_t fb = s_fwd ? 0 : (f16 ? conv_fwd16_scratch_bytes(g) : conv_fwd_scratch_bytes(g));
@@ -123,50 +162,14 @@
         CHK(c.mask_push(out->B, out->H, out->W, out->C, act, (size_t)out->numel(), &dst));
         RUN(positive_mask(out->d, out->dt, dst, out->numel(), c.st));
     }
-    c.wrote(out); c.wrote(co);
+    c.wrote(out);
+    if (!have_co) c.wrote(co);
     if (!want_grad) return ACLGAN_OK;
     const bool ln_train = ns.kind == ACLGAN_NORM_LN && ns.dw != nullptr;
-    c.push([=](aclgan_ctx& c) -> int {
-        if (!out->gw) return ACLGAN_OK;
-        CHK(c.acq(out));
-        if (residual && residual->need_grad) CHK(c.acq(residual));
-        if (gin->need_grad) CHK(c.acq(gin));
-        const double eg_out = out->gdt ? 2.0 : 4.0, eg_co = (has_norm ? co->gdt : (s_bwd ? dt : out->gdt)) ? 2.0 : 4.0, eg_in = gin->gdt ? 2.0 : 4.0;
-        c.count((es_co + eg_out + eg_co) * (double)co->numel() + ((residual && residual->need_grad) ? (residual->gdt ? 2.0 : 4.0) * (double)co->numel() : 0.0));
+    auto conv_bwd = [=](aclgan_ctx& c, const float* dyp, int dy_st, bool side, float* sbc) -> int {
+        const double eg_co = (has_norm ? co->gdt : (s_bwd ? dt : out->gdt)) ? 2.0 : 4.0, eg_in = gin->gdt ? 2.0 : 4.0;
         if (train_w) { c.count(es_in * (double)in->numel() + eg_co * (double)co->numel() + 4.0 * ((double)Co * g.K + Co)); c.exec_flops += conv_exec_flops(g, 2, w16); }
         if (gin->need_grad) { c.count(eg_co * (double)co->numel() + es_w * (double)Co * g.K + eg_in * (double)in->numel()); c.exec_flops += conv_exec_flops(g, 1, d16); }
-        const bool side = train_w && sw(SW_SIDE_STREAM);
-        if (ubytes && gin->need_grad && !d16 && c.ucache_reserve(W.w, g.up ? 3 : 1, ubytes)) { set_error("workspace too small (filter-transform cache)"); return ACLGAN_ENOMEM; }
-        float* g16 = nullptr;
-        const size_t mark_pre = c.top;
-        if (!has_norm && s_bwd && out->gdt == 0) {
-            g16 = (float*)c.alloc((size_t)out->numel() * 2);
-            NEED(g16);
-        }
-        float* sbc = nullptr;
-        if (ln_train && side) { sbc = c.allocf((int64_t)2 * g.B * Co); NEED(sbc); }
-        const size_t mark0 = side ? c.top : mark_pre;
-        const float* dyp = nullptr;
-        int dy_st = 0;
-        if (has_norm) {
-            const size_t mark = c.top;
-            void* scr = c.alloc(norm_scratch_bytes(g.B, HW, Co));
-            NEED(scr);
-            float* dres = nullptr; int dacc = 0;
-            if (residual && residual->need_grad) { dres = residual->g; dacc = residual->gw ? 1 : 0; mark_written(residual); }
-            NormST bst;
-            bst.x = co->dt; bst.y = out->dt; bst.dy = out->gdt; bst.dx = co->gdt; bst.dres = residual ? residual->gdt : 0;
-            RUN(norm_bwd(ns.kind, act, g.B, HW, Co, co->d, out->d, out->g, ns.w, ns.w_stride, mean, rstd, co->g, ns.dw, ns.db, dres, dacc, scr, c.st, &bst, sbc, ss));
-            c.top = mark;
-            dyp = co->g; dy_st = co->gdt;
-        } else if (s_bwd && out->gdt == 0) {
-            RUN(cast_storage(out->g, 0, g16, dt, out->numel(), c.st));
-            RUN(act_bwd_inplace(act, out->d, g16, out->numel(), c.st, out->dt, dt));
-            dyp = g16; dy_st = dt;
-        } else {
-            RUN(act_bwd_inplace(act, co->d, out->g, out->numel(), c.st, co->dt, out->gdt));
-            dyp = out->g; dy_st = out->gdt;
-        }
         if (train_w) {
             const size_t mark = c.top;
             void* wscr = nullptr;
@@ -203,9 +206,66 @@
             mark_written(gin);
             c.top = mark;
         }
+        return ACLGAN_OK;
+    };
+    if (merge && !reuse) {
+        c.push([=](aclgan_ctx& c) -> int {
+            if (!co->gw) return ACLGAN_OK;
+            CHK(c.acq(co));
+            if (gin->need_grad) CHK(c.acq(gin));
+            const bool side = train_w && sw(SW_SIDE_STREAM);
+            if (ubytes && gin->need_grad && !d16 && c.ucache_reserve(W.w, g.up ? 3 : 1, ubytes)) { set_error("workspace too small (filter-transform cache)"); return ACLGAN_ENOMEM; }
+            return conv_bwd(c, co->g, co->gdt, side, nullptr);
+        }, {{train_w ? W.dw : nullptr, W.nw}, {train_w ? W.db : nullptr, W.nb}});
+    }
+    c.push([=](aclgan_ctx& c) -> int {
+        if (!out->gw) return ACLGAN_OK;
+        CHK(c.acq(out));
+        if (residual && residual->need_grad) CHK(c.acq(residual));
+        if (merge) CHK(c.acq(co));
+        else if (gin->need_grad) CHK(c.acq(gin));
+        const double eg_out = out->gdt ? 2.0 : 4.0, eg_co = (has_norm ? co->gdt : (s_bwd ? dt : out->gdt)) ? 2.0 : 4.0;
+        c.count((es_co + eg_out + eg_co) * (double)co->numel() + ((residual && residual->need_grad) ? (residual->gdt ? 2.0 : 4.0) * (double)co->numel() : 0.0));
+        const bool side = !merge && train_w && sw(SW_SIDE_STREAM);
+        if (!merge && ubytes && gin->need_grad && !d16 && c.ucache_reserve(W.w, g.up ? 3 : 1, ubytes)) { set_error("workspace too small (filter-transform cache)"); return ACLGAN_ENOMEM; }
+        float* g16 = nullptr;
+        const size_t mark_pre = c.top;
+        if (!has_norm && s_bwd && out->gdt == 0) {
+            g16 = (float*)c.alloc((size_t)out->numel() * 2);
+            NEED(g16);
+        }
+        float* sbc = nullptr;
+        if (ln_train && side) { sbc = c.allocf((int64_t)2 * g.B * Co); NEED(sbc); }
+        const size_t mark0 = side ? c.top : mark_pre;
+        const float* dyp = nullptr;
+        int dy_st = 0;
+        if (has_norm) {
+            const size_t mark = c.top;
+            void* scr = c.alloc(norm_scratch_bytes(g.B, HW, Co));
+            NEED(scr);
+            float* dres = nullptr; int dacc = 0;
+            if (residual && residual->need_grad) { dres = residual->g; dacc = residual->gw ? 1 : 0; mark_written(residual); }
+            NormST bst;
+            bst.x = co->dt; bst.y = out->dt; bst.dy = out->gdt; bst.dx = co->gdt; bst.dres = residual ? residual->gdt : 0;
+            float* dx = co->g;
+            if (merge && co->gw) { dx = (float*)c.alloc((size_t)co->numel() * (co->gdt ? 2 : 4)); NEED(dx); }
+            RUN(norm_bwd(ns.kind, act, g.B, HW, Co, co->d, out->d, out->g, ns.w, ns.w_stride, mean, rstd, dx, ns.dw, ns.db, dres, dacc, scr, c.st, &bst, sbc, ss));
+            if (dx != co->g) { RUN(add_storage(dx, co->g, co->gdt, co->numel(), c.st)); c.count(3.0 * eg_co * (double)co->numel()); }
+            if (merge) mark_written(co);
+            c.top = mark;
+            dyp = co->g; dy_st = co->gdt;
+        } else if (s_bwd && out->gdt == 0) {
+            RUN(cast_storage(out->g, 0, g16, dt, out->numel(), c.st));
+            RUN(act_bwd_inplace(act, out->d, g16, out->numel(), c.st, out->dt, dt));
+            dyp = g16; dy_st = dt;
+        } else {
+            RUN(act_bwd_inplace(act, co->d, out->g, out->numel(), c.st, co->dt, out->gdt));
+            dyp = out->g; dy_st = out->gdt;
+        }
+        if (!merge) CHK(conv_bwd(c, dyp, dy_st, side, sbc));
         c.top = mark0;
         return ACLGAN_OK;
-    }, {{train_w ? W.dw : nullptr, W.nw}, {train_w ? W.db : nullptr, W.nb}, {ln_train ? ns.dw : nullptr, Co}, {ln_train ? ns.db : nullptr, Co}});
+    }, {{train_w && !merge ? W.dw : nullptr, W.nw}, {train_w && !merge ? W.db : nullptr, W.nb}, {ln_train ? ns.dw : nullptr, Co}, {ln_train ? ns.db : nullptr, Co}});
     return ACLGAN_OK;
 }
 
@@ -242,8 +302,16 @@
             float* u0 = nullptr;
             bool contiguous = true;
             const size_t ustride = (ubytes + 255) & ~(size_t)255;
+            aclgan_ctx::CarryRec::KeptU* ku = (!dgrad && c.carry_call != ACLGAN_CARRY_OFF && (net == ACLGAN_NET_GEN_AB || net == ACLGAN_NET_GEN_BA))
+                                                  ? &c.carry.u[net == ACLGAN_NET_GEN_BA][part] : nullptr;
+            const bool adoptU = ku && c.carry_call == ACLGAN_CARRY_ADOPT;
+            const bool haveU = adoptU && !c.dry && ku->set && ku->w0 == ws[0] && ku->uv == uv && ku->count == count && ku->ubytes == ubytes;
+            if (adoptU && !c.dry && !haveU) ku = nullptr;
+            char* cbase = nullptr;
+            if (haveU) cbase = (char*)ku->u0;
+            else if (ku) { cbase = (char*)c.alloc_carry((size_t)count * ustride); NEED(cbase); }
             for (int i = 0; i < count; ++i) {
-                float* u = (float*)c.alloc(ubytes);
+                float* u = cbase ? (float*)(cbase + (size_t)i * ustride) : (float*)c.alloc(ubytes);
                 NEED(u);
                 if (i == 0) u0 = u;
                 else if ((char*)u != (char*)u0 + (size_t)i * ustride) contiguous = false;
@@ -253,7 +321,9 @@
                 for (int i = 0; i < count; ++i) c.ucache[std::make_pair(ws[i], uv & 15)].filled = false;
                 continue;
             }
+            if (haveU) continue;
             RUN(conv_wino_prefill(g, uv, ws[0], wstride, u0, (int64_t)(ustride / sizeof(float)), count, c.st));
+            if (ku && !c.dry && c.carry_call == ACLGAN_CARRY_KEEP) { ku->set = true; ku->w0 = ws[0]; ku->uv = uv; ku->count = count; ku->ubytes = ubytes; ku->u0 = u0; }
         }
     }
     return ACLGAN_OK;
@@ -374,7 +444,7 @@
     return ACLGAN_OK;
 }
 
-int decode(aclgan_ctx& c, int net, bool train, Act* content, Act* style, Act** out) {
+int decode(aclgan_ctx& c, int net, bool train, Act* content, Act* style, Act** out, ConvShare* sh) {
     PassScope pass(c, net, "decode");
     const aclgan_arch& a = c.arch;
     char buf[160];
@@ -401,7 +471,7 @@
             if (ap->need_grad) { ns.db = ap->g + 2 * C * j; ns.dw = ap->g + 2 * C * j + C; }
             ++j;
             snprintf(buf, sizeof buf, "dec.model.0.model.%d.model.%d.conv", r, half);
-            if (half == 0) CHK(conv_block(c, c.pw(0, net, buf), train, h, C, 3, 1, 1, 0, ACLGAN_ACT_RELU, ns, nullptr, &t));
+            if (half == 0) CHK(conv_block(c, c.pw(0, net, buf), train, h, C, 3, 1, 1, 0, ACLGAN_ACT_RELU, ns, nullptr, &t, 1, r == 0 ? sh : nullptr));
             else CHK(conv_block(c, c.pw(0, net, buf), train, t, C, 3, 1, 1, 0, ACLGAN_ACT_NONE, ns, h, &o));
         }
         h = o;
diff --git a/acl-gan_amd/csrc/engine_step.hip b/acl-gan_amd/csrc/engine_step.hip
--- a/acl-gan_amd/csrc/engine_step.hip
+++ b/acl-gan_amd/csrc/engine_step.hip
@@ -3,6 +3,14 @@
 namespace aclgan {
 
 std::atomic<long long> g_enc_reuse_hits{0};
+std::atomic<long long> g_dec_share_hits{0};
+
+static ConvShare* decoder_share(aclgan_ctx& c, int i) {
+    if (!sw(SW_ENC_REUSE) || !sw(SW_DEC_SHARE) || sw(SW_FAULT_AT) >= 0 || c.size_unshared) return nullptr;
+    aclgan_ctx_carry_slot* slot = c.carry_call != ACLGAN_CARRY_OFF ? &c.carry.dec[i] : nullptr;
+    if (slot && c.carry_call == ACLGAN_CARRY_ADOPT && !c.dry && !slot->set) slot = nullptr;
+    return c.new_share(slot);
+}
 
 static int64_t dis_min_side(const aclgan_arch& a) {
     if (a.dis_n_layer + a.dis_num_scales > 30) return INT32_MAX;
@@ -60,9 +68,9 @@
     return ACLGAN_OK;
 }
 
-static int modeseek_pair(aclgan_ctx& c, int net, Act* content, Act* zu, Act* zu2, Act* xa, Act* img, int dir) {
+static int modeseek_pair(aclgan_ctx& c, int net, Act* content, Act* zu, Act* zu2, Act* xa, Act* img, int dir, ConvShare* sh) {
     Act *dec = nullptr, *img2 = nullptr;
-    CHK(decode(c, net, true, content, zu2, &dec)); CHK(c.mark());
+    CHK(decode(c, net, true, content, zu2, &dec, sh)); CHK(c.mark());
     CHK(zero_grad_of(c, dec));
     CHK(blend(c, dec, xa, nullptr, &img2, nullptr)); CHK(c.mark());
     const int B = img->B, sd = zu->H * zu->W * zu->C;
@@ -118,20 +126,21 @@
     if (c.carry_call == ACLGAN_CARRY_ADOPT && !c.dry) { c.carry.valid = false; g_enc_reuse_hits += 2; }
     PASS(style_encode(c, BA, true, xa, &s2));
     CHK(c.set_lane(L0));
-    PASS(decode(c, AB, true, c1, z1, &dB4)); CHK(zero_grad_of(c, dB4));
+    ConvShare *shAB = decoder_share(c, 0), *shBA = decoder_share(c, 1);
+    PASS(decode(c, AB, true, c1, z1, &dB4, shAB)); CHK(zero_grad_of(c, dB4));
     PASS(blend(c, dB4, xa, nullptr, &xB, nullptr));
-    if (ms) { CHK(c.set_lane(L2)); CHK(modeseek_pair(c, AB, c1, z1, z4, xa, xB, 0)); }
+    if (ms) { CHK(c.set_lane(L2)); CHK(modeseek_pair(c, AB, c1, z1, z4, xa, xB, 0, shAB)); }
     CHK(c.set_lane(L1));
-    PASS(decode(c, BA, true, c2, z2, &dA4)); CHK(zero_grad_of(c, dA4));
+    PASS(decode(c, BA, true, c2, z2, &dA4, shBA)); CHK(zero_grad_of(c, dA4));
     Act *vA1 = c.new_view(jA, 0, B), *vP1 = c.new_view(jP, 0, B), *vA2 = c.new_view(jA, B, B), *vP2 = c.new_view(jP, B, B);
     PASS(blend(c, dA4, xa, xa, &xA, &pA1, vA1, vP1));
-    if (ms) CHK(modeseek_pair(c, BA, c2, z2, z5, xa, xA, 1));
+    if (ms) CHK(modeseek_pair(c, BA, c2, z2, z5, xa, xA, 1, shBA));
     CHK(c.set_lane(L0));
     PASS(content_encode(c, BA, true, xB, &c3));
     PASS(decode(c, BA, true, c3, z3, &dA24)); CHK(zero_grad_of(c, dA24));
     PASS(blend(c, dA24, xB, xa, &xA2, &pA2, vA2, vP2));
     CHK(c.set_lane(L1));
-    PASS(decode(c, BA, true, c2, s2, &rA4)); CHK(zero_grad_of(c, rA4));
+    PASS(decode(c, BA, true, c2, s2, &rA4, shBA)); CHK(zero_grad_of(c, rA4));
     CHK(c.set_lane(L2));
     PASS(content_encode(c, AB, true, xb, &c4));
     PASS(style_encode(c, AB, true, xb, &s4));
@@ -226,10 +235,10 @@
     const int L0 = 0, L1 = 1, L2 = c.nlanes > 2 ? 2 : 1, LS = c.nlanes > 2 ? 2 : 0;
     CHK(encode_x_a(c, false, L0, L1, &in));
     CHK(c.set_lane(L0));
-    PASS(decode(c, AB, false, c1, z1, &dB4));
+    PASS(decode(c, AB, false, c1, z1, &dB4, c.carry_call == ACLGAN_CARRY_KEEP ? decoder_share(c, 0) : nullptr));
     PASS(blend(c, dB4, xa, nullptr, &xB, nullptr, c.new_view(jB, 0, B), nullptr));
     CHK(c.set_lane(L1));
-    PASS(decode(c, BA, false, c2, z2, &dA4));
+    PASS(decode(c, BA, false, c2, z2, &dA4, c.carry_call == ACLGAN_CARRY_KEEP ? decoder_share(c, 1) : nullptr));
     PASS(blend(c, dA4, xa, xa, &xA, &pA1, c.new_view(jA, 0, B), c.new_view(jP, 0, B)));
     const bool sn = c.dis_norm == ACLGAN_NORM_SN;
     if (!sn) PASS(dis_lsgan(c, ACLGAN_NET_DIS_B, true, jB, B, 3 * B, {{0.f, 1.f, hp.gan_w, L + ACLGAN_L_DIS_B}, {1.f, 1.f, hp.gan_w, L + ACLGAN_L_DIS_B}}, L1, L2));
@@ -307,9 +316,12 @@
     ACL_REQUIRE(c.groups[0].param && c.groups[1].param, "bind parameters first");
     size_t best = 0;
     for (int which = 0; which < 2; ++which)
-        for (int carry = 0; carry <= (sw(SW_ENC_REUSE) ? 1 : 0); ++carry) {
+        for (int carry = 0; carry <= (sw(SW_ENC_REUSE) ? 2 : 0); ++carry) {
             size_t pk = 0;
-            CHK(dry_update(c, which, B, H, W, -1, !carry ? ACLGAN_CARRY_OFF : which == 0 ? ACLGAN_CARRY_ADOPT : ACLGAN_CARRY_KEEP, false, true, &pk));
+            c.size_unshared = carry == 2;
+            const int rc = dry_update(c, which, B, H, W, -1, carry != 1 ? ACLGAN_CARRY_OFF : which == 0 ? ACLGAN_CARRY_ADOPT : ACLGAN_CARRY_KEEP, false, true, &pk);
+            c.size_unshared = false;
+            CHK(rc);
             if (pk > best) best = pk;
         }
     *out = best + 4096;
@@ -420,7 +432,8 @@
     ctx->st = (hipStream_t)stream; ctx->dry = false; ctx->peak = 0; ctx->peak2 = 0; ctx->trained = group_trained;
     ctx->carry_call = carry; ctx->carry_mode = ACLGAN_CARRY_OFF; ctx->carry_fail = false;
     ctx->carry_res = carry == ACLGAN_CARRY_ADOPT ? ctx->carry.bytes : 0;
-    if (carry == ACLGAN_CARRY_KEEP) { ctx->carry.blocks[0].clear(); ctx->carry.blocks[1].clear(); }
+    if (carry == ACLGAN_CARRY_KEEP) { ctx->carry.blocks[0].clear(); ctx->carry.blocks[1].clear(); ctx->carry.dec[0] = ctx->carry.dec[1] = aclgan_ctx_carry_slot();
+                                      for (auto& pair : ctx->carry.u) for (auto& ku : pair) ku = aclgan_ctx::CarryRec::KeptU(); }
     ctx->last_mode[group_trained] = carry;
     ctx->ucache_hook = WinoUCache{ctx, &aclgan_ctx::ucache_lookup};
     set_wino_ucache(&ctx->ucache_hook);
diff --git a/acl-gan_amd/csrc/misc.hip b/acl-gan_amd/csrc/misc.hip
--- a/acl-gan_amd/csrc/misc.hip
+++ b/acl-gan_amd/csrc/misc.hip
@@ -123,6 +123,22 @@
     if (n == 0) return ACLGAN_OK;
     hipLaunchKernelGGL(cast_storage_kernel, dim3((int)std::min<int64_t>(cdiv64(n / 4, 256), 8192)), dim3(256), 0, st, src, src_st, dst, dst_st, n / 4);
     ACL_CHECK_LAUNCH("cast_storage_kernel");
+    return ACLGAN_OK;
+}
+
+__global__ void add_storage_kernel(const void* __restrict__ src, void* __restrict__ dst, int st_, int64_t n4) {
+    for (int64_t i = (int64_t)blockIdx.x * 256 + threadIdx.x; i < n4; i += (int64_t)gridDim.x * 256) {
+        const st_f32x4 a = st_ld4(src, i, st_);
+        st_f32x4 b = st_ld4(dst, i, st_);
+        b[0] += a[0]; b[1] += a[1]; b[2] += a[2]; b[3] += a[3];
+        st_st4(dst, i, b, st_);
+    }
+}
+int add_storage(const void* src, void* dst, int st_, int64_t n, hipStream_t st) {
+    ACL_REQUIRE(n % 4 == 0, "add_storage: n %% 4 != 0");
+    if (n == 0) return ACLGAN_OK;
+    hipLaunchKernelGGL(add_storage_kernel, dim3((int)std::min<int64_t>(cdiv64(n / 4, 256), 8192)), dim3(256), 0, st, src, dst, st_, n / 4);
+    ACL_CHECK_LAUNCH("add_storage_kernel");
     return ACLGAN_OK;
 }
 
diff --git a/acl-gan_amd/csrc/switches.h b/acl-gan_amd/csrc/switches.h
--- a/acl-gan_amd/csrc/switches.h
+++ b/acl-gan_amd/csrc/switches.h
@@ -4,7 +4,7 @@
 namespace aclgan {
 
 enum SwitchId {
-    SW_LANES, SW_U_BATCH, SW_NORM_MASK, SW_MLP_FUSED, SW_FAULT_AT, SW_ENC_REUSE, SW_DGRAD_RING,
+    SW_LANES, SW_U_BATCH, SW_NORM_MASK, SW_MLP_FUSED, SW_FAULT_AT, SW_ENC_REUSE, SW_DEC_SHARE, SW_DGRAD_RING,
     SW_GLDS_TILE, SW_WINO_X3, SW_WINO_FUSED, SW_WINO_WGRAD_FUSED, SW_WINO_S2K4, SW_DGRAD16S_DIRECT, SW_FWD16_PATCH,
     SW_DETERMINISTIC,
     SW_NOFAST, SW_NOUP5, SW_SPLIT_NWG,
diff --git a/acl-gan_amd/csrc/switches.hip b/acl-gan_amd/csrc/switches.hip
--- a/acl-gan_amd/csrc/switches.hip
+++ b/acl-gan_amd/csrc/switches.hip
@@ -41,6 +41,7 @@
     {"mlp_fused",         "ACLGAN_MLP_FUSED",         1,  R_BOOL,  0, 0,       SETTABLE | EMPTY_UNSET, nullptr},
     {"fault_at",          nullptr,                    -1, R_INT,   0, 0,       SETTABLE, nullptr},
     {"enc_reuse",         nullptr,                    1,  R_BOOL,  0, 0,       SETTABLE, nullptr},
+    {"dec_share",         nullptr,                    1,  R_BOOL,  0, 0,       SETTABLE, nullptr},
     {"dgrad_ring",        nullptr,                    1,  R_BOOL,  0, 0,       SETTABLE, nullptr},
     {"glds_tile",         "ACLGAN_GLDS_TILE",         0,  R_CLAMP, 0, INT_MAX, SETTABLE, nullptr},
     {"wino_x3",           "ACLGAN_WINO_X3",           0,  R_BOOL,  0, 0,       SETTABLE, nullptr},
@@ -154,6 +155,7 @@
     ACL_REQUIRE(key && value, "aclgan_tuning_get: null argument");
     if (!strcmp(key, "epoch")) { *value = tuning_epoch(); return ACLGAN_OK; }
     if (!strcmp(key, "enc_reuse_hits")) { *value = g_enc_reuse_hits.load(); return ACLGAN_OK; }
+    if (!strcmp(key, "dec_share_hits")) { *value = g_dec_share_hits.load(); return ACLGAN_OK; }
     const int i = find(key);
     if (i < 0) { set_error("aclgan_tuning_get: unknown key '%s'", key); return ACLGAN_EINVAL; }
     *value = sw((SwitchId)i);
```
